# hvkwak/my-raytracer

Measured on AMD Instinct MI355X. Metric: Mrays/sec (primary+shadow+reflect), Office 1920x1080 1spp, higher is better.
Workload: dtype f64; 1 GPU; office_proxy 1920x1080 spp=1 depth=5 lights=2; triangles=59670, rays_per_frame=7073857, parallelism=single GPU, animation=camera orbit, 0.12 rad over each launch's 128 frames (distinct views), launches_in_flight=1, analytic_prims=False, production_frames_rendered=2595

## Files before the change

include/rt_hip.h:

```cpp
#ifndef RT_HIP_H
#define RT_HIP_H

#include <stddef.h>
#include "rt_scene.h"

#ifdef __cplusplus
extern "C" {
#endif

#define RT_OK 0
#define RT_ERR_INVALID (-1)
#define RT_ERR_HIP (-2)
#define RT_ERR_UNSUPPORTED (-3)

#define RT_MAX_LIGHTS 16
#define RT_LIGHTS_LIMIT (1 << 20)

typedef struct rt_scene_soa {
  int n_meshes;
  int n_vertices;
  int n_vertex_idx;
  int n_tex_coords;
  long long n_texels;
  const int* vertex_mesh_id;
// ... 23 lines not shown
  const double* bb_max;
  const int* left_child;
  const int* first_tri;
  const int* tri_count;
} rt_bvh_soa;

enum {
  RT_OUT_RGB_F32 = 0,
  RT_OUT_RGB_F64 = 1
};

enum {
  RT_FLAG_TRAVERSAL_STATS = 1,
  RT_FLAG_WIDE_STATS = 2,
  RT_FLAG_TIMELINE = 4,
  RT_FLAG_TILE_COST = 8,
  RT_FLAG_TILE_COST_TIME = 16,
  RT_FLAG_COST_ORDER = 32,
  RT_FLAG_NATURAL_ORDER = 64,
  RT_FLAG_GLOBAL_ROWS = 128
};

typedef struct rt_render_params {
  rt_camera camera;
  int n_lights;
  int max_depth;
  rt_light lights[RT_MAX_LIGHTS];
  double background[3];
  double ambience[3];
  int spp_n;
  int row_begin;
  int row_end;
  int stripe_height;
  int stripe_count;
  int stripe_index;
  int out_format;
  int flags;
  const rt_light* lights_ext;
} rt_render_params;

static inline const rt_light* rt_params_light(const rt_render_params* p, int i) {
  return p->lights_ext ? &p->lights_ext[i] : &p->lights[i];
}

typedef struct rt_stats {
  long long primary_rays;
  long long shadow_rays;
  long long reflection_rays;
  long long node_visits;
  long long tri_tests;
  long long closest_hits;
  long long pixels;
  long long reserved_;
} rt_stats;

typedef struct rt_scene rt_scene;

#define RT_MAX_COORDINATE 2305843009213693952.0

int rt_scene_upload(const rt_scene_soa* soa, const rt_bvh_soa* bvh, int device, rt_scene** out);

enum { RT_TREE_SAH = 0, RT_TREE_REFERENCE = 1, RT_TREE_SBVH = 2 };
enum { RT_COLLAPSE_GREEDY = 0, RT_COLLAPSE_SAH = 1, RT_COLLAPSE_BY_SIZE = 2 };

typedef struct rt_upload_options {
  int device_tree;
  int build_threads;
  int stack_ring;
  int lds_treelet;
  int collapse;
  int sbvh_leaf_max;
  int sbvh_bins;
  int blocks_per_cu;
  int grid_spare;
  int verbose;
  double sbvh_alpha;
  double sbvh_budget;
  double sbvh_c_trav;
  double collapse_c_tri;
  int reserve_cus;
  int order_window;
  int spp_lanes;
  int tree_opt;
  int reserved_[4];
} rt_upload_options;

enum { RT_TREE_OPT_PASSES = 3, RT_TREE_OPT_MAX = 64 };

void rt_upload_options_init(rt_upload_options* opt);

int rt_scene_upload_ex(const rt_scene_soa* soa, const rt_bvh_soa* bvh, int device, const rt_upload_options* opt,
                       rt_scene** out);

int rt_scene_upload_multi(const rt_scene_soa* soa, const rt_bvh_soa* bvh, const int* devices, int n_devices,
                          const rt_upload_options* opt, rt_scene** outs);

long long rt_scene_device_bytes(const rt_scene* scene);

int rt_scene_upload_seconds(const rt_scene* scene, double* build_s, double* copy_s);

int rt_scene_set_analytic(rt_scene* scene, const rt_sphere* spheres, int n_spheres, const rt_plane* planes,
                          int n_planes);

int rt_rows_in_shard(const rt_render_params* p);

int rt_launch_compute_image(rt_scene* scene, const rt_render_params* p, void* d_out,
                            rt_stats* stats, void* stream);

#define RT_MAX_FRAMES 128
int rt_launch_frames(rt_scene* scene, const rt_render_params* p, int n_frames, void* const* d_outs,
                     rt_stats* stats, void* stream);

int rt_launch_adaptive(rt_scene* scene, const rt_render_params* p, const double* d_primary, void* d_out, int subp,
                       double threshold, rt_stats* stats, long long* n_selected, void* stream);

int rt_launch_adaptive_frames(rt_scene* scene, const rt_render_params* p, int n_frames, const double* const* d_primary,
                              void* const* d_out, int subp, double threshold, rt_stats* stats, long long* n_selected,
                              void* stream);

int rt_launch_adaptive_shard(rt_scene* scene, const rt_render_params* p, const double* d_primary,
                             const double* d_halo, void* d_out, int subp, double threshold, rt_stats* stats,
                             long long* n_selected, void* stream);

int rt_adaptive_halo_rows(const rt_render_params* p, int* rows_out, int cap);

int rt_render_adaptive_to_host(rt_scene* scene, const rt_render_params* p, int subp, double threshold, void* host_out,
                               rt_stats* st_primary, rt_stats* st_adaptive, long long* n_selected);

int rt_render_to_host(rt_scene* scene, const rt_render_params* p, void* host_out, rt_stats* stats);

typedef struct rt_ray {
  double o[3];
  double d[3];
  double tmax;
  double reserved_;
} rt_ray;

typedef struct rt_hit {
  double t;
  double alpha;
  double beta;
  double normal[3];
  int slot;
  int mesh;
  int prim;
  int reserved_;
} rt_hit;

typedef struct rt_query_stats {
  long long rays, hits, stack_spills, watchdog, reserved_[4];
} rt_query_stats;

int rt_trace_closest(rt_scene* scene, const rt_ray* d_rays, long long n, rt_hit* d_hits, rt_query_stats* stats,
                     void* stream);

int rt_trace_occluded(rt_scene* scene, const rt_ray* d_rays, long long n, unsigned char* d_occluded,
                      rt_query_stats* stats, void* stream);

#define RT_RADIANCE_MAX_RAYS (1LL << 31)
int rt_trace_radiance(rt_scene* scene, const rt_render_params* p, const rt_ray* d_rays, long long n,
                      void* d_rgb, rt_stats* stats, void* stream);

#define RT_ORDER_MAX_RAYS (1LL << 31)
#define RT_ORDER_KEY_DEGENERATE 0x80000000u
#define RT_ORDER_TILE 1024

int rt_scene_bounds(const rt_scene* scene, double lo[3], double hi[3]);

size_t rt_ray_order_workspace_bytes(long long n);

// ... 52 lines not shown
int rt_trace_hits(rt_scene* scene, const rt_ray* d_rays, long long n, int k,
                  const rt_hit_key* d_after,
                  rt_hit* d_hits,
                  unsigned int* d_count,
                  rt_query_stats* stats, void* stream);

typedef struct rt_scene_update {
  long long n_vertices;
  long long n_triangles;
  const double* vertex_pos;
  const double* vertex_normals;
  const double* face_normals;
  long long reserved_[3];
} rt_scene_update;

int rt_scene_update_vertices(rt_scene* scene, const rt_scene_update* u, void* stream);

enum { RT_UPDATE_RECLIP = 1 };
int rt_scene_update_vertices_ex(rt_scene* scene, const rt_scene_update* u, unsigned flags, void* stream);

long long rt_debug_clip_regions(const rt_scene_soa* soa, const rt_bvh_soa* bvh, const rt_upload_options* opt,
                                double* clip_out, int* slot_out, long long cap);

int rt_reclip_box_host(const double p0[3], const double p1[3], const double p2[3], const double clip[6],
                       double lo[3], double hi[3]);

int rt_scene_set_triangle_order(rt_scene* scene, const int* slot_triangle, long long n_triangles);

typedef struct rt_scene_positions {
  long long n_vertices;
  const double* vertex_pos;
  int on_device;
  int reserved_;
  long long reserved2_[3];
} rt_scene_positions;

int rt_scene_update_positions(rt_scene* scene, const rt_scene_positions* positions, unsigned flags, void* stream);

int rt_normals_host(const int* vertex_idx, const int* slot_triangle, long long n_vertices, long long n_triangles,
                    const double* vertex_pos, double* vertex_normals_out, double* face_normals_out);

enum { RT_IMAGE_NODES4 = 0, RT_IMAGE_TRIS = 1, RT_IMAGE_TNORM = 2 };
long long rt_debug_scene_image(rt_scene* scene, int what, void* out, long long bytes);

#define RT_IPC_HANDLE_BYTES 64
int rt_ipc_get_handle(const void* d_ptr, unsigned char* handle, unsigned long long* offset);
int rt_ipc_open(const unsigned char* handle, unsigned long long offset, int device, int owner_device, void** d_ptr);
int rt_ipc_close(void* d_ptr, unsigned long long offset);

int rt_last_kernel_ms(rt_scene* scene, float* ms);

int rt_scene_status(const rt_scene* scene);

int rt_debug_counters(rt_scene* scene, unsigned long long* out, int n);

long long rt_debug_wave_log(rt_scene* scene, unsigned long long* out, long long n);

int rt_debug_blocks_per_cu(rt_scene* scene, int variant);

int rt_debug_last_grid(rt_scene* scene, long long* blocks, long long* full_blocks);

int rt_debug_corrupt_hierarchy(rt_scene* scene);

enum {
  RT_TREE_BAD_UNION = 1,
  RT_TREE_BAD_LEAF = 2,
  RT_TREE_BAD_RECORDS = 4,
  RT_TREE_BAD_IDS = 8,
  RT_TREE_BAD_FIXPOINT = 16
};
typedef struct rt_tree_report {
  long long binary_nodes, wide_nodes, records;
  long long moved;
  double sah_before, sah_after, dp_before, dp_after;
  double seconds;
  int passes;
  int stack4;
  unsigned int invalid;
  int converged;
} rt_tree_report;
int rt_debug_tree_report(const rt_scene_soa* soa, const rt_bvh_soa* bvh, const rt_upload_options* opt,
                         rt_tree_report* out);

long long rt_debug_timeline(rt_scene* scene, unsigned long long* out, long long n);

int rt_tile_shape(int* tile_w, int* tile_h);

long long rt_debug_tile_cost(rt_scene* scene, unsigned int* out, long long n);
int rt_debug_set_tile_order(rt_scene* scene, const unsigned int* order, long long n);
long long rt_debug_last_tile_order(rt_scene* scene, unsigned int* out, long long n);

void rt_scene_free(rt_scene* scene);

const char* rt_last_error(void);

const char* rt_build_info(void);

#ifdef __cplusplus
}
#endif
#endif
```

my-raytracer_amd/csrc/device/rt_render.hip:

```cpp
#ifndef RT_RAY_LIST_PASS
#include <hip/hip_runtime.h>
#include <hip/hip_ext.h>

#include <algorithm>
#include <array>
#include <chrono>
#include <cfloat>
#include <cmath>
#include <cstdio>
#include <cstdlib>
#include <cstring>
#include <memory>
#include <string>
#include <thread>
#include <vector>

#include <rocprim/block/block_radix_sort.hpp>

#include "../../../include/rt_hip.h"
#include "../host/device_image.hpp"
#include "rt_layout.hpp"

#pragma clang fp contract(off)

#include "rt_ao_fan.hpp"
#include "rt_refit.hpp"
#include "rt_reclip.hpp"
#include "rt_normals.hpp"

using namespace rtk;

namespace {

constexpr int kBlock = 256;
constexpr int kGroups = 8;
#ifndef RT_REFILL
#define RT_REFILL 16
#endif
constexpr int kRefill = RT_REFILL;
#ifndef RT_REFILL_GATE
#define RT_REFILL_GATE 0
#endif
constexpr bool kRefillGate = RT_REFILL_GATE != 0;
#ifndef RT_LEAF_PIN
#define RT_LEAF_PIN 1
#endif
#ifndef RT_MAT_BATCH
#define RT_MAT_BATCH 1
#endif
#ifndef RT_STACK_FAST
#define RT_STACK_FAST 41
#endif
constexpr bool kFastSort = (RT_STACK_FAST & 1) != 0, kFastAny = (RT_STACK_FAST & 2) != 0, kFastPop = (RT_STACK_FAST & 4) != 0;
constexpr bool kOneHit = (RT_STACK_FAST & 8) != 0, kMaskCnt = (RT_STACK_FAST & 32) != 0;
static_assert((RT_STACK_FAST & ~47) == 0, "RT_STACK_FAST: bits 1, 2, 4, 8 and 32");
constexpr bool kRoomTest = kFastSort || kFastAny;
constexpr int kCtrWords = 42;
constexpr int kShortStack = 8;
constexpr int kSlotDoubles = 10;
constexpr int kTopNodes = (40960 - kBlock * (kSlotDoubles * 8 + (2 + kShortStack) * 4) - RT_MAX_LIGHTS * 48 - 64) / 128;
constexpr int kStackMask = kShortStack - 1;
#ifndef RT_DONATE_MAX
#define RT_DONATE_MAX 24
#endif
constexpr int kDonateMax = RT_DONATE_MAX;
constexpr int kMigWords = 8;
static_assert(kMigWords <= kShortStack, "migration words travel in the stack ring entries");
constexpr int kPoolBytes = 64;
static_assert(8 + 8 * (kBlock / 64) + 4 <= kPoolBytes, "compaction pool does not fit");
static_assert((kShortStack & kStackMask) == 0, "the stack ring must be a power of two");

#ifdef RT_TILE_ROW_ORDER
constexpr bool kTileMorton = false;
#else
constexpr bool kTileMorton = true;
#endif
enum : int { ST_FETCH = 0, ST_CLOSEST = 1, ST_SHADOW = 2, ST_DONE = 3, ST_PARKED = 4, ST_HSHADOW = 5, ST_HCLOSEST = 6 };
constexpr uint32_t kTaskNone = 0xffffffffu;
constexpr uint32_t kTaskRefl = 0x80000000u;
static_assert(RT_LIGHTS_LIMIT <= (1 << 20), "light index must fit the task word");
constexpr int kBatchExtra = 31;
constexpr int kHelpShift = 24;
constexpr int kEndMask = (1 << kHelpShift) - 1;
static_assert(RT_LIGHTS_LIMIT < (1 << kHelpShift), "light index must fit the batch word");

__device__ __forceinline__ void wave_lds_sync() {
  __builtin_amdgcn_wave_barrier();
  asm volatile("s_waitcnt lgkmcnt(0)" ::: "memory");
  __builtin_amdgcn_wave_barrier();
}

constexpr int kBufWord3 = 0x00020000;
typedef unsigned int u32x2_t __attribute__((ext_vector_type(2)));
__device__ __forceinline__ double buf_ld(__amdgpu_buffer_rsrc_t r, uint32_t voff, uint32_t soff) {
  return __builtin_bit_cast(double, __builtin_amdgcn_raw_buffer_load_b64(r, voff, soff, 0));
}
__device__ __forceinline__ void buf_st(__amdgpu_buffer_rsrc_t r, uint32_t voff, uint32_t soff, double x) {
  __builtin_amdgcn_raw_buffer_store_b64(__builtin_bit_cast(u32x2_t, x), r, voff, soff, 0);
}
typedef unsigned int u32x4_t __attribute__((ext_vector_type(4)));
struct D2 {
  double a, b;
};
__device__ __forceinline__ D2 buf_ld2(__amdgpu_buffer_rsrc_t r, uint32_t voff, uint32_t soff) {
  const u32x4_t v = __builtin_amdgcn_raw_buffer_load_b128(r, voff, soff, 0);
  return D2{__builtin_bit_cast(double, u32x2_t{v.x, v.y}), __builtin_bit_cast(double, u32x2_t{v.z, v.w})};
}


__device__ __forceinline__ int wave_incl_scan(int x) {
  int incl = x;
#pragma unroll
  for (int o = 1; o < 64; o <<= 1) {
    const int v = __shfl_up(incl, o);
    if ((int)(threadIdx.x & 63) >= o) incl += v;
  }
  return incl;
}

__device__ __forceinline__ int kth_set_bit(unsigned long long m, int k) {
  int base = 0;
#pragma unroll
  for (int w = 32; w >= 1; w >>= 1) {
    const int c = __popcll(m & ((1ull << w) - 1ull));
    if (k >= c) { k -= c; m >>= w; base += w; }
  }
  return base;
}
enum : int { CS_PRIMARY = 8, CS_SHADOW, CS_REFLECT, CS_NODES, CS_TRIS, CS_HITS, CS_PIXELS };
enum : int {
  CD_NODE_ITERS = 16, CD_NODE_LANES, CD_LEAF_ITERS, CD_LEAF_LANES, CD_TRAV_CYCLES, CD_SHADE_CYCLES,
  CD_FETCH_CYCLES, CD_OUTER_ITERS, CD_TRAV_ROUNDS, CD_TRAV_ROUND_LANES, CD_SPILLS, CD_NODE_LINES,
  CD_LEAF_LINES, CD_BIG_LEAF_TESTS, CD_NODE_LDS_ITERS, CD_GUARD = 31,
  CD_GNODE_UNIFORM = 32, CD_GNODE_DISTINCT, CD_LEAF_UNIFORM, CD_ANYHIT_TRIS, CD_OWN_TRIS,
  CD_ZERO_TERM,
  CT_ORDER_JOBS = 39,
  CD_SLOW_PUSH = 40, CD_SLOW_POP
};
static_assert(kCtrWords * sizeof(unsigned long long) <= 512, "the counter words end where the work heads begin");
constexpr unsigned kGuardIters = 1u << 24;
constexpr unsigned kTravGuard = 1u << 24;
__device__ __forceinline__ void trip_watchdog(unsigned long long* ctr, unsigned int* host_word) {
  atomicOr(&ctr[CD_GUARD], 1ull);
  __builtin_nontemporal_store(1u, host_word);
  __threadfence_system();
  asm volatile("s_waitcnt vmcnt(0)" ::: "memory");
}
constexpr int kTlCap = 256;
constexpr int kTlWords = 8;

struct DivMagic {
  uint32_t m, s;
  __host__ __device__ uint32_t div(uint32_t n) const {
#ifdef __HIP_DEVICE_COMPILE__
    return m ? __umulhi(n, m) >> s : n;
#else
    return m ? (uint32_t)(((unsigned long long)n * m) >> 32) >> s : n;
#endif
  }
};
inline DivMagic div_magic(uint32_t d) {
  for (uint32_t s = 0; s < 32; ++s) {
    const unsigned __int128 p = (unsigned __int128)1 << (32 + s);
    const unsigned __int128 m = (p + d - 1) / d;
    if (m >> 32) continue;
    const unsigned __int128 e = m * d - p;
    if ((e << 31) < p) return DivMagic{(uint32_t)m, s};
  }
  return DivMagic{0u, 0u};
}
constexpr int kMaxFrames = RT_MAX_FRAMES;
constexpr int kListFrameShift = 25;
constexpr uint32_t kListPixMask = (1u << kListFrameShift) - 1u;
static_assert(kMaxFrames <= (1 << (32 - kListFrameShift)), "frame index must fit a list entry");
struct FrameDesc {
  double eye[3], ll[3], xd[3], yd[3];
  void* out;
  long long pad;
};
static_assert(sizeof(FrameDesc) == 112, "FrameDesc must be 112 bytes");
constexpr size_t kHeadsOff = 512;
constexpr int kHeadStride = 32;
constexpr size_t kCtrBytes = kHeadsOff + kGroups * 256;
constexpr size_t kCtlBytes = kCtrBytes + kMaxFrames * sizeof(FrameDesc);
struct KParams {
  const GNode* nodes;
  const GNode4* nodes4;
  const GTri* tris;
  const uint32_t* slot2dev;
  const TriShade* shade;
  const double* tnorm;
  const double* tu;
  const double* tv;
  const unsigned char* texels;
  const GMat* mats;
  unsigned long long* ctr;
  unsigned long long* heads;
  unsigned long long* wctr;
  double* pstate;
  uint32_t* spill;
  unsigned long long* wavelog;
  unsigned long long* tl;
  const double* lights;
  unsigned int* guard_host;
  size_t nslots;
  int n_gnodes;
  int out_fmt;
  int n_top;
  int top_off;
  double root_lo[3], root_hi[3];
  int W, H;
  int n_lights, max_depth;
  int zero_term_lights;
  double bg[3], amb[3];
  int spp_n;
  int group_log, chunks;
  int row_begin, stripe_h, stripe_count, stripe_index;
  int rows;
  int tiles_x;
  int out_global;
  union {
    int order_dilate;
    uint32_t fan_seed;
  };
  long long n_tiles;
  union {
    const uint32_t* list;
    const double* fan_dirs;
  };
  const unsigned long long* list_count;
  union {
    double* sample_out;
    double fan_bias;
  };
  union {
    int nsamp;
    int fan_k;
  };
  int n_prims;
  const GPrim* prims;
  int n_frames;
  int lights_off;
  int pool_off;
  long long frame_tiles;
  const FrameDesc* frames;
  union {
    const uint32_t* tile_order;
    const rt_ray* rays;
  };
  uint32_t* tile_cost;
  union {
    int cost_time;
    int fan_sets;
  };
  DivMagic div_row_tiles, div_tiles_x, div_stripe_h;
  const uint32_t* order_src;
  uint32_t* next_order;
  uint32_t* zero_map;
  union {
    long long n_pos;
    long long n_rays;
  };
};

struct D3 {
  double x, y, z;
};
__device__ __forceinline__ D3 d3(double x, double y, double z) { return D3{x, y, z}; }
__device__ __forceinline__ D3 add(D3 a, D3 b) { return D3{a.x + b.x, a.y + b.y, a.z + b.z}; }
__device__ __forceinline__ D3 sub(D3 a, D3 b) { return D3{a.x - b.x, a.y - b.y, a.z - b.z}; }
__device__ __forceinline__ D3 scl(double s, D3 a) { return D3{s * a.x, s * a.y, s * a.z}; }
__device__ __forceinline__ D3 mul(D3 a, D3 b) { return D3{a.x * b.x, a.y * b.y, a.z * b.z}; }
__device__ __forceinline__ double dot(D3 a, D3 b) { return a.x * b.x + a.y * b.y + a.z * b.z; }
__device__ __forceinline__ D3 normalize(D3 v) {
  const double n = sqrt(dot(v, v));
  if (n > 0.0) return D3{v.x / n, v.y / n, v.z / n};
  return v;
}
__device__ __forceinline__ double sqrt_normal(double q) {
  const double y = __builtin_amdgcn_rsq(q);
  double g = q * y, h = y * 0.5;
  const double r = __builtin_fma(-h, g, 0.5);
  g = __builtin_fma(g, r, g);
  double d = __builtin_fma(-g, g, q);
  h = __builtin_fma(h, r, h);
  g = __builtin_fma(d, h, g);
  d = __builtin_fma(-g, g, q);
  return __builtin_fma(d, h, g);
}
__device__ __forceinline__ double rcp_refined(double n) {
  double r = __builtin_amdgcn_rcp(n);
  r = __builtin_fma(r, __builtin_fma(-n, r, 1.0), r);
  return __builtin_fma(r, __builtin_fma(-n, r, 1.0), r);
}
__device__ __forceinline__ double div_by(double x, double n, double r) {
  const double q = x * r;
  return __builtin_fma(__builtin_fma(-n, q, x), r, q);
}
__device__ __forceinline__ D3 normalize_rcp(D3 v, double& n) {
  const double q = dot(v, v);
  const bool ok = fabs(v.x) >= 0x1p-200 && fabs(v.y) >= 0x1p-200 && fabs(v.z) >= 0x1p-200 &&
                  q <= 0x1p400;
  if (!ok) {
    n = sqrt(q);
    return normalize(v);
  }
  n = sqrt_normal(q);
  const double r = rcp_refined(n);
  return D3{div_by(v.x, n, r), div_by(v.y, n, r), div_by(v.z, n, r)};
}
__device__ __forceinline__ D3 normalize_shade(D3 v) {
  const double q = dot(v, v);
  if (!(q > 1e-200 && q < 1e200)) return normalize(v);
  const double r0 = __builtin_amdgcn_rsq(q);
  const double e = __builtin_fma(-(q * r0), r0, 1.0);
  const double r = __builtin_fma(0.5 * r0, e, r0);
  return D3{v.x * r, v.y * r, v.z * r};
}
__device__ __forceinline__ double pow_shade(double x, double y) {
  if (y >= 1.0 && y <= 256.0 && y == __builtin_floor(y)) {
    uint32_t n = (uint32_t)y;
    double r = 1.0, b = x;
    for (;;) {
      if (n & 1u) r *= b;
      n >>= 1;
      if (n == 0u) break;
      b *= b;
    }
    return r;
  }
  return pow(x, y);
}
__device__ __forceinline__ double stdmax(double a, double b) { return (a < b) ? b : a; }
__device__ __forceinline__ double stdmin(double a, double b) { return (b < a) ? b : a; }

__device__ __forceinline__ double det3(D3 v1, D3 v2, D3 v3) {
  return v1.x * (v2.y * v3.z - v3.y * v2.z) - v2.x * (v1.y * v3.z - v3.y * v1.z) +
         v3.x * (v1.y * v2.z - v2.y * v1.z);
}


__device__ __forceinline__ double prim_hit(const GPrim& G, D3 o, D3 d) {
  const D3 c = d3(G.c[0], G.c[1], G.c[2]);
  if (G.type == kPrimPlane) {
    const D3 n = d3(G.n[0], G.n[1], G.n[2]);
// ... 132 lines not shown
  __device__ __forceinline__ D3 kd() const { return d3(q1.y, q2.x, q2.y); }
  __device__ __forceinline__ D3 ks() const { return d3(q3.x, q3.y, q4.x); }
  __device__ __forceinline__ double shininess() const { return q4.y; }
  __device__ __forceinline__ double mirror() const { return q5.x; }
  __device__ __forceinline__ int shadowable() const { return __double2loint(q5.y); }
  __device__ __forceinline__ int draw_mode() const { return __double2hiint(q5.y); }
  __device__ __forceinline__ int tex_w() const { return __double2loint(q6); }
  __device__ __forceinline__ int tex_h() const { return __double2hiint(q6); }
  __device__ __forceinline__ uint32_t flags() const { return (uint32_t)__double2loint(q7); }
};
static_assert(offsetof(GMat, kd) == 24 && offsetof(GMat, ks) == 48 && offsetof(GMat, shininess) == 72 &&
              offsetof(GMat, mirror) == 80 && offsetof(GMat, shadowable) == 88 && offsetof(GMat, draw_mode) == 92 &&
              offsetof(GMat, tex_w) == 96 && offsetof(GMat, tex_h) == 100 && offsetof(GMat, flags) == 112,
              "Mat<true> unpacks GMat by its 16-byte groups");

#ifndef RT_TILE_W
#define RT_TILE_W 8
#endif
constexpr int kTileW = RT_TILE_W, kTileH = 64 / RT_TILE_W;
constexpr int kTileWLog = kTileW == 8 ? 3 : kTileW == 16 ? 4 : kTileW == 32 ? 5 : -1;
constexpr int kTileHLog = 6 - kTileWLog;
static_assert(kTileWLog > 0 && kTileW * kTileH == 64, "a tile is one wave's 64 pixels (8, 16 or 32 wide)");

enum : int { R_SCOLW = 0, R_PCOL = 1, R_HD = 2, R_LACC = 3, kRegions = 4 };
constexpr uint32_t kLaneRec = 32;
constexpr uint32_t kRegionBytes = 64 * kLaneRec;

struct RaySlots {
  double* o[3];
  double* d[3];
  double* tlim;
  double* a[3];
};

__device__ __forceinline__ float f4c(const float4& v, int c) {
  return c == 0 ? v.x : (c == 1 ? v.y : (c == 2 ? v.z : v.w));
}
__device__ __forceinline__ uint32_t u4c(const uint4& v, int c) {
  return c == 0 ? v.x : (c == 1 ? v.y : (c == 2 ? v.z : v.w));
}


#ifndef RT_WAVES_PER_EU
#define RT_WAVES_PER_EU 4
#endif
constexpr int kWavesPerEU = RT_WAVES_PER_EU;

constexpr int kOrderItems = 16;
constexpr int kOrderDilate = 4;
constexpr long long kOrderMaxRange = (long long)kBlock * kOrderItems;
constexpr int kOrderShift = 21;
__device__ __forceinline__ uint32_t order_class(uint32_t cost) {
  const int q = (int)(__float_as_uint((float)cost) >> kOrderShift) - ((127 + 8) << (23 - kOrderShift));
  return 255u - (uint32_t)min(255, max(0, q));
}
__device__ void order_range(const uint32_t* cost, uint32_t* order, long long n_tiles, int h, unsigned char* lds,
                            int tiles_x, int dilate) {
  using Sort = rocprim::block_radix_sort<unsigned int, kBlock, kOrderItems>;
  static_assert(sizeof(typename Sort::storage_type) <= 30720, "sort storage must fit the block's LDS (at least 30 KB)");
  auto& storage = *reinterpret_cast<typename Sort::storage_type*>(lds);
  const long long t0 = n_tiles * h / kGroups, t1 = n_tiles * (h + 1) / kGroups;
  unsigned int keys[kOrderItems];
#pragma unroll
  for (int j = 0; j < kOrderItems; ++j) {
    const long long li = (long long)threadIdx.x * kOrderItems + j;
    uint32_t c = 0u;
    if (t0 + li < t1) {
      const long long t = t0 + li, row = t / tiles_x, col = t - row * tiles_x;
      const long long x0 = max(0LL, col - dilate), x1 = min((long long)tiles_x - 1, col + dilate);
      for (long long x = x0; x <= x1; ++x) c = max(c, cost[row * tiles_x + x]);
    }
    keys[j] = t0 + li < t1 ? (order_class(c) << 12) | (uint32_t)li : 0xffffffffu;
  }
  Sort().sort(keys, storage, 12, 20);
#pragma unroll
  for (int j = 0; j < kOrderItems; ++j) {
    const long long pos = (long long)threadIdx.x * kOrderItems + j;
    if (t0 + pos < t1) order[t0 + pos] = (uint32_t)(t0 + (keys[j] & 0xfffu));
  }
}

#endif

#ifndef RT_RAY_LIST_PASS
template <int WIDTH, bool STATS, bool TL = false, int RING = kShortStack, bool GRP = false>
__global__ void __launch_bounds__(kBlock, kWavesPerEU * 256 / kBlock) render_kernel(KParams P) {
  constexpr bool RAYS = false, FAN = false;
#define RT_GROUPS_ON group_log
#elif !defined(RT_FAN_PASS)
template <int RING>
__global__ void __launch_bounds__(kBlock, kWavesPerEU * 256 / kBlock) radiance_kernel(KParams P) {
  constexpr int WIDTH = 4;
  constexpr bool STATS = false, TL = false, GRP = false, RAYS = true, FAN = false;
#define RT_GROUPS_ON group_log
#else
template <int RING>
__global__ void __launch_bounds__(kBlock, kWavesPerEU * 256 / kBlock) gather_kernel(KParams P) {
  constexpr int WIDTH = 4;
  constexpr bool STATS = false, TL = false, GRP = true, RAYS = true, FAN = true;
#define RT_GROUPS_ON true
#endif
  static_assert(RING >= kMigWords && (RING & (RING - 1)) == 0, "ring: a power of two holding the migration words");
  constexpr int kRingMask = RING - 1;
  constexpr bool kPinMat = RT_MAT_BATCH != 0 && !GRP;
  extern __shared__ __attribute__((aligned(16))) unsigned char lds_raw[];
  constexpr uint32_t kRingRegion = (uint32_t)RING * kBlock * sizeof(uint32_t);
  unsigned char* const lds_s = lds_raw + kRingRegion;
  double* lds_d = reinterpret_cast<double*>(lds_s);
  RaySlots R;
#pragma unroll
  for (int k = 0; k < 3; ++k) {
    R.o[k] = lds_d + k * kBlock + threadIdx.x;
    R.d[k] = lds_d + (3 + k) * kBlock + threadIdx.x;
  }
  R.tlim = lds_d + 6 * kBlock + threadIdx.x;
#pragma unroll
  for (int k = 0; k < 3; ++k) R.a[k] = lds_d + (7 + k) * kBlock + threadIdx.x;
  uint32_t* ltask = reinterpret_cast<uint32_t*>(lds_s + kSlotDoubles * kBlock * sizeof(double));
  uint32_t* lvis = ltask + kBlock;
  uint32_t* stk = reinterpret_cast<uint32_t*>(lds_raw) + threadIdx.x;
  const uint32_t lane_b = threadIdx.x * 4u;
  lvis[threadIdx.x] = 0u;
  uint32_t* pool_live = reinterpret_cast<uint32_t*>(lds_raw + P.pool_off);
  unsigned long long* pool_mask = reinterpret_cast<unsigned long long*>(lds_raw + P.pool_off + 8);
  uint32_t* pool_exh = reinterpret_cast<uint32_t*>(lds_raw + P.pool_off + 8 + 8 * (kBlock / 64));
  if (threadIdx.x == 0) {
    *pool_live = kBlock / 64;
    for (int w = 0; w < kBlock / 64; ++w) pool_mask[w] = 0ull;
    *pool_exh = 0u;
  }
  if (WIDTH == 4 && P.n_top > 0) {
    float4* dst = reinterpret_cast<float4*>(lds_raw + P.top_off);
    const float4* src = reinterpret_cast<const float4*>(P.nodes4);
    for (int i = threadIdx.x; i < P.n_top * (int)(sizeof(GNode4) / sizeof(float4)); i += kBlock) dst[i] = src[i];
  }
  double* lds_lights = reinterpret_cast<double*>(lds_raw + P.lights_off);
  const bool lights_lds = P.n_lights <= RT_MAX_LIGHTS;
  if (lights_lds)
    for (int i = threadIdx.x; i < P.n_lights * 6; i += kBlock) lds_lights[i] = P.lights[i];
  __syncthreads();
  const int wbase = threadIdx.x & ~63;
  uint32_t* spill = P.spill + (size_t)blockIdx.x * kBlock + threadIdx.x;

  const int lane = threadIdx.x & 63;
  auto lane_bit = [&](unsigned long long m) -> bool {
    int l = lane;
    asm volatile("" : "+v"(l));
    return ((m >> l) & 1ull) != 0ull;
  };
  auto below = [](unsigned long long m) -> int {
    return (int)__builtin_amdgcn_mbcnt_hi((uint32_t)(m >> 32), __builtin_amdgcn_mbcnt_lo((uint32_t)m, 0u));
  };
  const int group_log = GRP ? P.group_log : 0;
  auto full_groups = [&](unsigned long long m) -> unsigned long long {
    const int gl = group_log;
    for (int sh = 1; sh < (1 << gl); sh <<= 1) m &= m >> sh;
    unsigned long long first = 0ull;
    for (int b = 0; b < 64; b += 1 << gl) first |= 1ull << b;
    return m & first;
  };
  const __amdgpu_buffer_rsrc_t prs =
      __builtin_amdgcn_make_buffer_rsrc(P.pstate, 0, (int)(P.nslots * kRegions * kLaneRec), kBufWord3);
  uint32_t pvo = (blockIdx.x * (kBlock / 64) + (threadIdx.x >> 6)) * (uint32_t)kRegions * kRegionBytes +
                 (uint32_t)lane * kLaneRec;
  auto LD4 = [&](int r, D3& v, double& w) {
    const D2 a = buf_ld2(prs, pvo, (uint32_t)r * kRegionBytes), b = buf_ld2(prs, pvo, (uint32_t)r * kRegionBytes + 16u);
    v = d3(a.a, a.b, b.a);
    w = b.b;
  };
  auto ST4 = [&](int r, D3 v, double w) {
#ifdef RT_MEAS_NO_PSTATE
    return;
#endif
    const uint32_t o = (uint32_t)r * kRegionBytes;
    buf_st(prs, pvo, o, v.x); buf_st(prs, pvo, o + 8u, v.y); buf_st(prs, pvo, o + 16u, v.z); buf_st(prs, pvo, o + 24u, w);
  };
  auto LDV = [&](int r) { D3 v; double w; LD4(r, v, w); return v; };
  auto STV = [&](int r, D3 v) { ST4(r, v, 0.0); };
  auto LD_HN = [&]() { return d3(*R.a[0], *R.a[1], *R.a[2]); };
  auto ST_HN = [&](D3 v) { *R.a[0] = v.x; *R.a[1] = v.y; *R.a[2] = v.z; };
  auto LD_SCOL_W = [&](D3& scol, double& w) {
    LD4(R_SCOLW, scol, w);
  };
  auto ST_SCOL_W = [&](D3 scol, double w) { ST4(R_SCOLW, scol, w); };

  const long long n_list = !RAYS && P.list ? (long long)*P.list_count * (group_log ? 1 : P.nsamp) : 0;
  const long long n_tiles = !RAYS && P.list ? (n_list + 63) / 64 : P.n_tiles;
  int head = blockIdx.x % kGroups;
  int heads_left = kGroups;

  int state = ST_FETCH;
  int px = 0, lrow = 0, py = 0, sample = 0, depth = 0, light = 0, mesh = 0, frame = 0;
  long long item = 0;
  uint32_t pix_t0 = 0;
  int best = kNoHit;
  int own_rec = -1;
  int best_slot = kNoHit;
  double thit = DBL_MAX;
  bool shadow_hit = false;
  int batch_end = 0;
  int refl_h = -1;
  int want = 0;
  uint32_t htask = kTaskNone;
  unsigned c_primary = 0, c_shadow = 0, c_refl = 0, c_hits = 0;
  unsigned n_zero_term = 0;
  unsigned long long c_nodes = 0, c_tris = 0;
  unsigned long long d_node_it = 0, d_node_ln = 0, d_leaf_it = 0, d_leaf_ln = 0;
  unsigned long long d_trav = 0, d_shade = 0, d_fetch = 0, d_outer = 0, d_round_it = 0, d_round_ln = 0;
  unsigned long long d_spills = 0, d_node_lines = 0, d_leaf_lines = 0, d_big_leaf = 0, d_node_lds = 0, d_dummy = 0, d_gn_uni = 0, d_gn_dist = 0, d_leaf_uni = 0;
  unsigned long long d_slow_push = 0, d_slow_pop = 0;
  unsigned long long d_any_tris = 0, d_own_tris = 0;
  unsigned long long w_start = STATS ? __builtin_amdgcn_s_memrealtime() : 0ull, w_refill = 0, w_pixels = 0;
  unsigned long long t_stamp = 0;
  unsigned tl_n = 0;
  unsigned long long tl_t0 = 0;
  unsigned tl_it = 0, tl_leaf = 0, tl_spill = 0, tl_gnode = 0;
  unsigned long long tl_wn = 0, tl_wl = 0, tl_wr = 0, tl_dummy = 0;
  unsigned long long tl_gsum[4] = {0, 0, 0, 0}, tl_gcnt[4] = {0, 0, 0, 0}, tl_gap = 0;
  auto tl_wave_gap = [&](uint32_t kind) {
    const unsigned long long m = wballot(1);
    if (lane == __ffsll((long long)m) - 1) {
      const uint32_t now = (uint32_t)__builtin_amdgcn_s_memrealtime();
      const uint32_t prev = ltask[wbase + 63], pk = ltask[wbase + 62];
      ltask[wbase + 63] = now;
      ltask[wbase + 62] = kind;
      const unsigned long long g = now - prev;
#pragma unroll
      for (uint32_t k = 0; k < 4; ++k)
        if (pk == k) { tl_gsum[k] += g; tl_gcnt[k]++; }
      if (g > tl_gap) tl_gap = g;
    }
  };
  auto stamp = [&]() -> unsigned long long { return STATS ? __builtin_amdgcn_s_memtime() : 0ull; };

  struct Light6 { D3 pos, col; };
  typedef __attribute__((address_space(3))) double lds_double;
  typedef __attribute__((address_space(1))) const double glb_double;
  auto light_of = [&](int j) -> Light6 {
    if (lights_lds) {
      const lds_double* L = (const lds_double*)(lds_double*)(lds_lights) + 6 * j;
      return Light6{d3(L[0], L[1], L[2]), d3(L[3], L[4], L[5])};
    }
    const glb_double* L = (const glb_double*)(P.lights) + 6 * (size_t)j;
    return Light6{d3(L[0], L[1], L[2]), d3(L[3], L[4], L[5])};
  };

  auto nrm_n = [](D3 v, double& n) -> D3 {
    if constexpr (STATS || TL) {
      n = sqrt(dot(v, v));
      return normalize(v);
    } else {
      return normalize_rcp(v, n);
    }
  };
  auto nrm = [&](D3 v) -> D3 {
    double n;
    return nrm_n(v, n);
  };
  auto emit_ray = [&](D3 o, D3 dir, double t_limit) {
    const D3 d = nrm(dir);
    *R.o[0] = o.x; *R.o[1] = o.y; *R.o[2] = o.z;
    *R.d[0] = d.x; *R.d[1] = d.y; *R.d[2] = d.z;
    *R.tlim = t_limit;
  };

  auto start_sample = [&]() {
    int n = P.spp_n;
    asm volatile("" : "+s"(n));
    double X, Y;
    if (n == 1) {
      X = (double)px;
      Y = (double)py;
    } else {
      const int si = sample / n, sj = sample - si * n;
      const double xo = (si) / (double)n - 0.5 + 1.0 / (2.0 * n);
      const double yo = (sj) / (double)n - 0.5 + 1.0 / (2.0 * n);
      X = (double)px + xo;
      Y = (double)py + yo;
    }
    const FrameDesc& K = P.frames[frame];
    const D3 dir = d3(K.ll[0] + X * K.xd[0] + Y * K.yd[0] - K.eye[0],
                      K.ll[1] + X * K.xd[1] + Y * K.yd[1] - K.eye[1],
                      K.ll[2] + X * K.xd[2] + Y * K.yd[2] - K.eye[2]);
    depth = 0;
    c_primary++;
    if (sample == 0) pix_t0 = (uint32_t)__builtin_amdgcn_s_memrealtime();
    emit_ray(d3(K.eye[0], K.eye[1], K.eye[2]), dir, DBL_MAX);
    state = ST_CLOSEST;
// ... 152 lines not shown
            item = wk;
          } else {
            const uint32_t tile = P.tile_order ? P.tile_order[wk >> 6] : (uint32_t)(wk >> 6);
            const int j = (int)(wk & 63);
            const uint32_t row_tiles = (uint32_t)P.n_frames * (uint32_t)P.tiles_x;
            const uint32_t ty = P.div_row_tiles.div(tile);
            const uint32_t rem = tile - ty * row_tiles;
            frame = P.n_frames > 1 ? (int)P.div_tiles_x.div(rem) : 0;
            const int tx = (int)(rem - (uint32_t)frame * (uint32_t)P.tiles_x);
            int jx = j & (kTileW - 1), jy = j >> kTileWLog;
            if (kTileMorton && kTileW == 8) {
              jx = (j & 1) | ((j >> 1) & 2) | ((j >> 2) & 4);
              jy = ((j >> 1) & 1) | ((j >> 2) & 2) | ((j >> 3) & 4);
            }
            px = tx * kTileW + jx;
            lrow = (int)ty * kTileH + jy;
          }
          if (!RAYS && px < P.W && lrow < P.rows) {
            py = (P.stripe_count == 1)
                     ? P.row_begin + lrow
                     : stripe_row(P, lrow);
            if (P.list && !group_log) {
              long long ns = P.nsamp;
              asm volatile("" : "+s"(ns));
              sample = (int)(item % ns);
            } else {
              sample = lane - gbase;
            }
            start_sample();
          }
        }
      }
      m_fetch = wballot(state == ST_FETCH);
      m_busy = wballot(state == ST_CLOSEST || state == ST_SHADOW || state >= ST_HSHADOW);
      m_claim = RT_GROUPS_ON ? full_groups(m_fetch) : m_fetch;
      if (!RT_GROUPS_ON && __popcll(m_fetch) < kRefill && m_busy != 0) break;
    }
    if (heads_left == 0 && state == ST_FETCH) state = ST_DONE;
    const bool busy = (state == ST_CLOSEST || state == ST_SHADOW || state >= ST_HSHADOW);
    if (wballot(busy) == 0) {
      if (wballot(state != ST_DONE) != 0) continue;
      bool leave = true;
      if (lane == 0) {
        uint32_t v = *pool_live;
        for (;;) {
          if (v >= 2u) {
            const uint32_t seen = atomicCAS(pool_live, v, v - 1u);
            if (seen == v) break;
            v = seen;
            continue;
          }
          bool pooled = false;
          for (int w = 0; w < kBlock / 64; ++w) pooled |= pool_mask[w] != 0ull;
          if (pooled) leave = false;
          else *pool_live = 0u;
          break;
        }
      }
      if (__shfl(leave ? 1 : 0, 0)) break;
    }

    if (STATS) { const unsigned long long t = stamp(); d_fetch += t - t_stamp; t_stamp = t; }
    if constexpr (TL) {
      tl_t0 = __builtin_amdgcn_s_memrealtime();
      tl_it = tl_leaf = tl_spill = tl_gnode = 0;
      tl_wn = tl_wl = tl_wr = 0;
      tl_gap = 0;
#pragma unroll
      for (int k = 0; k < 4; ++k) tl_gsum[k] = tl_gcnt[k] = 0;
      if (lane == 0) { ltask[wbase + 63] = (uint32_t)tl_t0; ltask[wbase + 62] = 0u; }
      wave_lds_sync();
    }
    unsigned long long sh0 = 0ull;
    int kp = 0;
    for (;; ++kp) {
      const bool act = kp == 0 ? busy
                               : (state == ST_SHADOW && light + (batch_end >> kHelpShift) + kp < (batch_end & kEndMask));
      const bool anyhit = act && (state == ST_SHADOW || state == ST_HSHADOW);
      const int src = (act && state >= ST_HSHADOW) ? wbase + (int)(htask & 63u) : (int)threadIdx.x;
      D3 ro = d3(lds_d[0 * kBlock + src], lds_d[1 * kBlock + src], lds_d[2 * kBlock + src]);
      D3 rd = d3(lds_d[3 * kBlock + src], lds_d[4 * kBlock + src], lds_d[5 * kBlock + src]);
      double tlim = lds_d[6 * kBlock + src];
      bool zero_term = false;
      if (anyhit) {
        const int j = (state == ST_SHADOW) ? light + (kp > 0 ? (batch_end >> kHelpShift) + kp : 0)
                                           : (int)((htask >> 11) & 0xFFFFFu);
        const D3 hp = add(ro, scl(tlim, rd));
        const D3 to_l = sub(light_of(j).pos, hp);
        double nl;
        const D3 l = nrm_n(to_l, nl);
        if (lvis[src] & 1u) {
          const D3 hn = d3(lds_d[7 * kBlock + src], lds_d[8 * kBlock + src], lds_d[9 * kBlock + src]);
          zero_term = !(dot(hn, l) > 0.0);
        }
        ro = add(hp, scl(1e-4, l));
        rd = nrm(l);
        tlim = nl;
      } else if (act && state == ST_HCLOSEST) {
        const D3 hp = add(ro, scl(tlim, rd));
        const D3 hn = d3(lds_d[7 * kBlock + src], lds_d[8 * kBlock + src], lds_d[9 * kBlock + src]);
        const double s2 = 2.0 * dot(hn, rd);
        const D3 v = sub(rd, scl(s2, hn));
        ro = add(hp, scl(1e-4, v));
        rd = nrm(v);
        tlim = DBL_MAX;
        *R.o[0] = ro.x; *R.o[1] = ro.y; *R.o[2] = ro.z;
        *R.d[0] = rd.x; *R.d[1] = rd.y; *R.d[2] = rd.z;
      }
      int own = -1;
      if (anyhit) own = (state == ST_SHADOW) ? own_rec : __shfl(own_rec, (int)(htask & 63u));
      best = kNoHit;
      best_slot = kNoHit;
      n_zero_term += (unsigned)__popcll(wballot(zero_term));
      shadow_hit = !STATS && !TL && zero_term;
      uint32_t cur = kDone;
      double t_off = 0.0;
      for (int k = 0; k < P.n_prims; ++k) {
        if (!act || shadow_hit) break;
        const double t = prim_hit(P.prims[k], ro, rd);
        if (t < tlim) {
          if (anyhit) { shadow_hit = true; break; }
          tlim = t;
          best = kPrimHit | k;
          best_slot = -1;
        }
      }
      if (act && P.n_gnodes > 0 && !shadow_hit) {
        bool miss = false;
        int pz = 0;
        asm volatile("" : "+s"(pz));
        const double* const root_lo = P.root_lo + pz;
        const double* const root_hi = P.root_hi + pz;
        const double o3[3] = {ro.x, ro.y, ro.z}, d3v[3] = {rd.x, rd.y, rd.z};
        bool inside = true;
#pragma unroll
        for (int k = 0; k < 3; ++k)
          if (!(o3[k] >= root_lo[k] && o3[k] <= root_hi[k])) inside = false;
        if (!inside) {
          double tn = -DBL_MAX, tf = DBL_MAX;
#pragma unroll
          for (int k = 0; k < 3; ++k) {
            if (d3v[k] == 0.0) {
              if (o3[k] < root_lo[k] || o3[k] > root_hi[k]) miss = true;
              continue;
            }
            double t0 = (root_lo[k] - o3[k]) / d3v[k];
            double t1 = (root_hi[k] - o3[k]) / d3v[k];
            if (t0 > t1) { const double t = t0; t0 = t1; t1 = t; }
            if (t0 > tn) tn = t0;
            if (t1 < tf) tf = t1;
          }
          if (tn > tf || tf < 0.0) miss = true;
          t_off = tn > 0.0 ? tn : 0.0;
        }
        if (miss) t_off = 0.0;
        else cur = 0;
      }
      float inv[3];
      {
        const double d3v[3] = {rd.x, rd.y, rd.z};
#pragma unroll
        for (int k = 0; k < 3; ++k) {
          float df = (float)d3v[k];
          if (fabsf(df) < 1e-20f) df = signbit(d3v[k]) ? -1e-20f : 1e-20f;
          if constexpr (WIDTH == 4) {
            const float r0 = __builtin_amdgcn_rcpf(df);
            inv[k] = __builtin_fmaf(__builtin_fmaf(-df, r0, 1.0f), r0, r0);
          } else {
            inv[k] = 1.0f / df;
          }
        }
      }
      const float ofx = (float)(ro.x + t_off * rd.x);
      const float ofy = (float)(ro.y + t_off * rd.y);
      const float ofz = (float)(ro.z + t_off * rd.z);
      const float ivx = inv[0], ivy = inv[1], ivz = inv[2];
      const uint32_t nxo = ivx >= 0.f ? 0u : 16u, nyo = ivy >= 0.f ? 32u : 48u, nzo = ivz >= 0.f ? 64u : 80u;
      const float oix = ofx * ivx, oiy = ofy * ivy, oiz = ofz * ivz;
      const float lo_c = round_down_f(-t_off);
      float hi_c = round_up_f(tlim - t_off);
      float pinf = INFINITY;
      asm volatile("" : "+s"(pinf));
      constexpr uint32_t kSW = kBlock * 4u, kRingB = (uint32_t)RING * kSW, kRingBMask = (uint32_t)kRingMask * kSW;
      uint32_t sq = 0, sqlim = kRingB;
      auto ring = [&](uint32_t q) -> __attribute__((address_space(3))) uint32_t& {
        return *reinterpret_cast<__attribute__((address_space(3))) uint32_t*>((size_t)((q & kRingBMask) | lane_b));
      };
      auto push = [&](uint32_t x) {
        if (sq == sqlim) {
          const uint32_t qlo = sqlim - kRingB;
          spill[(size_t)(qlo / kSW) * P.nslots] = ring(qlo);
          sqlim += kSW;
          if (STATS) d_spills++;
          if constexpr (TL) tl_spill++;
        }
        ring(sq) = x;
        sq += kSW;
      };
      auto pop = [&]() -> uint32_t {
        if (sq == 0) return kDone;
        sq -= kSW;
        if (sq + kRingB >= sqlim) return ring(sq);
        sqlim = sq + kRingB;
        return spill[(size_t)(sq / kSW) * P.nslots];
      };
      auto pop_fast = [&]() -> uint32_t {
        const uint32_t x = ring(sq - kSW);
        const bool empty = sq == 0;
        sq -= empty ? 0u : kSW;
        return empty ? kDone : x;
// ... 706 lines not shown
        if (group_done && lane == gbase) {
          D3 pc = sample == 0 ? d3(0, 0, 0) : LDV(R_PCOL);
          if constexpr (FAN) {
            for (int k = 0; k < (1 << gl) && sample + k < P.fan_k; ++k) {
              const int t = wbase + gbase + k;
              pc = add(pc, d3(lds_d[0 * kBlock + t], lds_d[1 * kBlock + t], lds_d[2 * kBlock + t]));
            }
            if (sample + (1 << gl) < P.fan_k) STV(R_PCOL, pc);
            else store_pixel(pc);
          } else {
            for (int k = 0; k < (1 << gl); ++k) {
              const int t = wbase + gbase + k;
              pc = add(pc, d3(lds_d[0 * kBlock + t], lds_d[1 * kBlock + t], lds_d[2 * kBlock + t]));
            }
            if (sample + (1 << gl) < P.spp_n * P.spp_n) STV(R_PCOL, pc);
            else store_pixel(pc);
          }
        }
        wave_lds_sync();
        if (group_done) {
          sample += 1 << gl;
          if constexpr (FAN) {
            if (sample - (lane - gbase) < P.fan_k) start_fan();
            else state = heads_left > 0 ? ST_FETCH : ST_DONE;
          } else {
            if (sample < P.spp_n * P.spp_n) start_sample();
            else state = heads_left > 0 ? ST_FETCH : ST_DONE;
          }
        }
      }
    }

    {
      const bool idle = (state == ST_FETCH || state == ST_DONE);
      const unsigned long long I = wballot(idle);
      if (I != 0ull && wballot(want > 0) != 0ull) {
        if (idle) ltask[threadIdx.x] = kTaskNone;
        const int incl = wave_incl_scan(want);
        wave_lds_sync();
        const int off = incl - want;
        const int avail = (int)__popcll(I);
        const int got = min(want, max(0, avail - off));
        if (got > 0) {
          const int n_extra_lights = min(P.n_lights - light - 1, kBatchExtra);
          for (int t = 0; t < got; ++t) {
            const int ht = wbase + kth_set_bit(I, off + t);
            uint32_t tw;
            if (t < n_extra_lights) {
              tw = (uint32_t)lane | ((uint32_t)(t + 1) << 6) | ((uint32_t)(light + 1 + t) << 11);
            } else {
              tw = (uint32_t)lane | kTaskRefl;
              c_refl++;
              refl_h = ht;
            }
            ltask[ht] = tw;
          }
          batch_end |= min(got, n_extra_lights) << kHelpShift;
        }
        wave_lds_sync();
        if (idle) {
          htask = ltask[threadIdx.x];
          if (htask != kTaskNone) state = (htask & kTaskRefl) ? ST_HCLOSEST : ST_HSHADOW;
        }
      }
    }
    if (STATS) { const unsigned long long t = stamp(); d_shade += t - t_stamp; t_stamp = t; }
  }

  if (STATS && lane == 0) {
    unsigned long long* wl = P.wavelog + 4 * ((size_t)blockIdx.x * (kBlock / 64) + (threadIdx.x >> 6));
    wl[0] = w_start;
    wl[1] = w_refill;
    wl[2] = __builtin_amdgcn_s_memrealtime();
    wl[3] = w_pixels;
  }
  if (P.out_global) {
    __threadfence_system();
    asm volatile("s_waitcnt vmcnt(0)" ::: "memory");
  }
  const unsigned long long s0 = wave_sum(c_primary), s1 = wave_sum(c_shadow), s2 = wave_sum(c_refl);
  unsigned long long s3 = 0, s4 = 0, s5 = 0;
  if (STATS) { s3 = wave_sum(c_nodes); s4 = wave_sum(c_tris); s5 = wave_sum(c_hits); }
  if (lane == 0) {
    unsigned long long* wc = P.wctr + 4 * ((size_t)blockIdx.x * (kBlock / 64) + (threadIdx.x >> 6));
    wc[0] = s0; wc[1] = s1; wc[2] = s2; wc[3] = n_zero_term;
    if (STATS) {
      atomicAdd(&P.ctr[CS_NODES], s3);
      atomicAdd(&P.ctr[CS_TRIS], s4);
      atomicAdd(&P.ctr[CS_HITS], s5);
      atomicAdd(&P.ctr[CD_TRAV_CYCLES], d_trav);
      atomicAdd(&P.ctr[CD_SHADE_CYCLES], d_shade);
      atomicAdd(&P.ctr[CD_FETCH_CYCLES], d_fetch);
      atomicAdd(&P.ctr[CD_OUTER_ITERS], d_outer);
    }
  }
  if (STATS) {
    const unsigned long long a = wave_sum(d_node_it), b = wave_sum(d_node_ln), c = wave_sum(d_leaf_it);
    const unsigned long long d = wave_sum(d_leaf_ln), e = wave_sum(d_round_it), f = wave_sum(d_round_ln);
    const unsigned long long g = wave_sum(d_spills), h = wave_sum(d_node_lines), q = wave_sum(d_leaf_lines);
    const unsigned long long r = wave_sum(d_big_leaf), t = wave_sum(d_node_lds);
    const unsigned long long gu = wave_sum(d_gn_uni), gd = wave_sum(d_gn_dist), lu = wave_sum(d_leaf_uni);
    const unsigned long long at = wave_sum(d_any_tris), ot = wave_sum(d_own_tris);
    const unsigned long long pu = wave_sum(d_slow_push), po = wave_sum(d_slow_pop);
    if (lane == 0) {
      atomicAdd(&P.ctr[CD_SLOW_PUSH], pu);
      atomicAdd(&P.ctr[CD_SLOW_POP], po);
      atomicAdd(&P.ctr[CD_ANYHIT_TRIS], at);
      atomicAdd(&P.ctr[CD_OWN_TRIS], ot);
      atomicAdd(&P.ctr[CD_NODE_LDS_ITERS], t);
      atomicAdd(&P.ctr[CD_GNODE_UNIFORM], gu);
      atomicAdd(&P.ctr[CD_GNODE_DISTINCT], gd);
      atomicAdd(&P.ctr[CD_LEAF_UNIFORM], lu);
      atomicAdd(&P.ctr[CD_NODE_ITERS], a);
      atomicAdd(&P.ctr[CD_NODE_LANES], b);
      atomicAdd(&P.ctr[CD_LEAF_ITERS], c);
      atomicAdd(&P.ctr[CD_LEAF_LANES], d);
      atomicAdd(&P.ctr[CD_TRAV_ROUNDS], e);
      atomicAdd(&P.ctr[CD_TRAV_ROUND_LANES], f);
      atomicAdd(&P.ctr[CD_SPILLS], g);
      atomicAdd(&P.ctr[CD_NODE_LINES], h);
      atomicAdd(&P.ctr[CD_LEAF_LINES], q);
      atomicAdd(&P.ctr[CD_BIG_LEAF_TESTS], r);
    }
  }
  if (!RAYS && P.zero_map) {
    uint32_t* job = reinterpret_cast<uint32_t*>(lds_raw);
    for (;;) {
      __syncthreads();
      if (threadIdx.x == 0) *job = (uint32_t)atomicAdd(&P.ctr[CT_ORDER_JOBS], 1ull);
      __syncthreads();
      const uint32_t j = *job;
      __syncthreads();
      if (j >= 2u * kGroups) break;
      if (j < (uint32_t)kGroups) {
        if (P.order_src) order_range(P.order_src, P.next_order, P.n_pos, (int)j, lds_raw, P.tiles_x, P.order_dilate);
      } else {
        for (long long i = P.n_pos * (j - kGroups) / kGroups + threadIdx.x; i < P.n_pos * (j - kGroups + 1) / kGroups;
             i += kBlock)
          P.zero_map[i] = 0u;
      }
    }
  }
}
#undef RT_GROUPS_ON

#ifndef RT_RAY_LIST_PASS
#define RT_RAY_LIST_PASS 1
#include __FILE_NAME__
#define RT_FAN_PASS 1
#include __FILE_NAME__
#undef RT_FAN_PASS
#undef RT_RAY_LIST_PASS

__device__ __forceinline__ double nsq3(const double* a, const double* b) {
  const double dx = a[0] - b[0], dy = a[1] - b[1], dz = a[2] - b[2];
  return dx * dx + dy * dy + dz * dz;
}

struct ShardRows {
  int rows, W, H;
  int row_begin, stripe_h, stripe_count, stripe_index;
  __host__ __device__ int global_row(int lrow) const {
    return stripe_count == 1 ? row_begin + lrow
                             : ((lrow / stripe_h) * stripe_count + stripe_index) * stripe_h + (lrow % stripe_h);
  }
  __host__ __device__ int seg_first(int lrow) const { return stripe_count == 1 ? 0 : lrow - lrow % stripe_h; }
  __host__ __device__ int seg_last(int lrow) const {
    return stripe_count == 1 ? rows - 1 : min(seg_first(lrow) + stripe_h, rows) - 1;
  }
  __host__ __device__ int segment(int lrow) const { return stripe_count == 1 ? 0 : lrow / stripe_h; }
  __host__ __device__ int segments() const { return stripe_count == 1 ? (rows > 0) : (rows + stripe_h - 1) / stripe_h; }
};

constexpr int kSelThreads = 1024;
constexpr int kSelTilesPerWave = 8;
constexpr int kSelTilesPerBlock = (kSelThreads / 64) * kSelTilesPerWave;
__global__ void __launch_bounds__(kSelThreads) adaptive_select_kernel(const double* prim, const double* halo, void* out,
                                                                      int out_fmt, ShardRows G, double threshold,
                                                                      int tiles_x, long long n_tiles, uint32_t* list,
                                                                      unsigned long long* count, uint32_t frame_tag,
                                                                      const double* const* prims, void* const* outs) {
  if (prims) {
    prim = prims[blockIdx.y];
    out = outs[blockIdx.y];
    frame_tag = (uint32_t)blockIdx.y << kListFrameShift;
  }
  __shared__ uint32_t s_list[kSelThreads * kSelTilesPerWave];
  __shared__ uint32_t s_n;
  __shared__ unsigned long long s_base;
  if (threadIdx.x == 0) s_n = 0u;
  __syncthreads();
  const int j = threadIdx.x & 63;
  const int W = G.W;
  for (int it = 0; it < kSelTilesPerWave; ++it) {
    const long long tile = (long long)blockIdx.x * kSelTilesPerBlock + it * (kSelThreads / 64) + (threadIdx.x >> 6);
    bool sel = false;
    int x = 0, lrow = 0;
    if (tile < n_tiles) {
      const long long ty = tile / tiles_x;
      x = (int)(tile - ty * tiles_x) * 8 + (j & 7);
      lrow = (int)ty * 8 + (j >> 3);
      if (x < W && lrow < G.rows) {
        const size_t o = 3 * ((size_t)lrow * W + x);
        const double* c = prim + o;
        const int y = G.global_row(lrow);
        if (x >= 1 && y >= 1 && x < W - 1 && y < G.H - 1) {
          const int seg = G.segment(lrow);
          const double* up = lrow < G.seg_last(lrow) ? c + 3 * (size_t)W : halo + 3 * ((size_t)(2 * seg + 1) * W + x);
          const double* dn = lrow > G.seg_first(lrow) ? c - 3 * (size_t)W : halo + 3 * ((size_t)(2 * seg) * W + x);
          const double n = nsq3(c, c + 3) + nsq3(c, up) + nsq3(c, c - 3) + nsq3(c, dn);
          sel = n > threshold;
        }
        if (!sel) {
          if (out_fmt == RT_OUT_RGB_F64) {
            double* d = reinterpret_cast<double*>(out) + o;
            d[0] = c[0]; d[1] = c[1]; d[2] = c[2];
          } else {
            float* d = reinterpret_cast<float*>(out) + o;
            d[0] = (float)c[0]; d[1] = (float)c[1]; d[2] = (float)c[2];
          }
        }
      }
    }
    const unsigned long long m = wballot(sel);
    if (m != 0ull) {
      const int leader = __ffsll((long long)m) - 1;
      uint32_t base = 0u;
      if (j == leader) base = atomicAdd(&s_n, (uint32_t)__popcll(m));
      base = __shfl(base, leader);
      if (sel) {
        const unsigned long long below = j == 0 ? 0ull : (m & (~0ull >> (64 - j)));
        s_list[base + __popcll(below)] = frame_tag | (uint32_t)((size_t)lrow * W + x);
      }
    }
  }
  __syncthreads();
  const uint32_t n = s_n;
  if (n == 0u) return;
  if (threadIdx.x == 0) s_base = atomicAdd(count, (unsigned long long)n);
  __syncthreads();
  const unsigned long long b = s_base;
  for (uint32_t k = threadIdx.x; k < n; k += kSelThreads) list[b + k] = s_list[k];
}

__global__ void __launch_bounds__(256) adaptive_reduce_kernel(const uint32_t* list, const unsigned long long* count,
                                                              const double* samples, int nsamp, void* out,
                                                              int out_fmt, void* const* outs) {
  const long long i = (long long)blockIdx.x * blockDim.x + threadIdx.x;
  if (i >= (long long)*count) return;
  const double* s = samples + 3 * (size_t)i * nsamp;
  double r = 0.0, g = 0.0, b = 0.0;
  for (int k = 0; k < nsamp; ++k) {
    r = r + s[3 * k];
    g = g + s[3 * k + 1];
    b = b + s[3 * k + 2];
  }
  const double nn = (double)nsamp;
  r = stdmin(r / nn, 1.0);
  g = stdmin(g / nn, 1.0);
  b = stdmin(b / nn, 1.0);
  const uint32_t id = list[i];
  const size_t o = 3 * (size_t)(id & kListPixMask);
  if (outs) out = outs[id >> kListFrameShift];
  if (out_fmt == RT_OUT_RGB_F64) {
    double* d = reinterpret_cast<double*>(out) + o;
    d[0] = r; d[1] = g; d[2] = b;
  } else {
    float* d = reinterpret_cast<float*>(out) + o;
    d[0] = (float)r; d[1] = (float)g; d[2] = (float)b;
  }
}

thread_local std::string g_error;

int fail(int code, const std::string& msg) {
  g_error = msg;
  return code;
}

#define HIP_TRY(call)                                                                          \
  do {                                                                                         \
    const hipError_t e_ = (call);                                                              \
    if (e_ != hipSuccess)                                                                      \
      return fail(RT_ERR_HIP, std::string(#call) + ": " + hipGetErrorString(e_));              \
  } while (0)


using KernelFn = void (*)(KParams);

struct Variant {
  KernelFn fn;
  bool stats;
};

const Variant kVariants[] = {
    {render_kernel<4, false>, false},
    {render_kernel<4, true>, true},
    {render_kernel<2, true>, true},
    {render_kernel<4, false, true>, false},
    {render_kernel<4, false, false, 16>, false},
    {render_kernel<4, false, false, kShortStack, true>, false},
    {render_kernel<4, false, false, 16, true>, false},
    {radiance_kernel<kShortStack>, false},
    {radiance_kernel<16>, false},
    {gather_kernel<kShortStack>, false},
    {gather_kernel<16>, false},
};
constexpr int kNumVariants = 11;
constexpr int kRayVariant = 7;
constexpr int kFanVariant = 9;
constexpr bool kSppLanesDefault = true;
constexpr int kGroupLanes = 32;
constexpr int kRingDeep = 16;
inline int variant_ring(int v) {
  return (v == 4 || v == 6 || v == kRayVariant + 1 || v == kFanVariant + 1) ? kRingDeep : kShortStack;
}
size_t lds_bytes(int , int ring = kShortStack) {
  return (size_t)kBlock * (kSlotDoubles * sizeof(double) + (2 + (size_t)ring) * sizeof(uint32_t));
}
size_t lds_bytes_total(int stack_words, int n_top, int ring = kShortStack) {
  return lds_bytes(stack_words, ring) + (size_t)n_top * sizeof(GNode4) + RT_MAX_LIGHTS * 6 * sizeof(double) + kPoolBytes;
}
int top_nodes_for(int stack_words, int ring, int n_gnodes4) {
  const long long room = 40960 - (long long)lds_bytes_total(stack_words, 0, ring);
  return (int)std::max(0LL, std::min<long long>({room / (long long)sizeof(GNode4), (long long)kTopNodes, (long long)n_gnodes4}));
}

}

constexpr int kContexts = 8;
struct LaunchCtx {
  unsigned long long* d_ctr = nullptr;
  unsigned char* h_ctl = nullptr;
  size_t ctl_cap = 0;
  long long blocks = 0;
  long long full_blocks = 0;
  double* d_pstate = nullptr;
  uint32_t* d_spill = nullptr;
  unsigned long long* d_wavelog = nullptr;
  unsigned long long* d_wctr = nullptr;
  unsigned long long* d_tl = nullptr;
  hipEvent_t ev0 = nullptr, ev1 = nullptr;
  hipEvent_t ev_in = nullptr;
  long long waves = 0;
  int variant = -1;
  bool used = false;
};

struct QueryRing;
struct UpdateState;
struct NormalState;

struct rt_scene {
  int device = 0;
  GNode* d_nodes = nullptr;
  GTri* d_tris = nullptr;
  uint32_t* d_slot2dev = nullptr;
  TriShade* d_shade = nullptr;
  double* d_tnorm = nullptr;
  double* d_tu = nullptr;
  double* d_tv = nullptr;
  unsigned char* d_texels = nullptr;
  GMat* d_mats = nullptr;
  int n_gnodes = 0;
  long long n_tris = 0;
  int n_meshes = 0;
  int depth = 0;
  int stack_words = 1;
  LaunchCtx ctx[kContexts];
  int next_ctx = 0;
  int last_ctx = -1;
  hipStream_t last_stream = nullptr;
  size_t nslots = 0;
  unsigned int* h_guard = nullptr;
  unsigned int* d_guard = nullptr;
  double delta = 0.0;
  double root_lo[3] = {0, 0, 0}, root_hi[3] = {0, 0, 0};
  long long bytes = 0;
  int n_cu = 0;
  int blocks_per_cu[kNumVariants] = {};
  bool deep = false;
  bool big = false;
  int n_top_v[kNumVariants] = {};
  GNode4* d_nodes4 = nullptr;
  int n_gnodes4 = 0;
  int bpc_cap = 0;
  int grid_spare = 0;
  std::vector<GMat> mesh_mats;
  GPrim* d_prims = nullptr;
  int n_prims = 0;
  long long table_bytes = 0;
  uint32_t* d_cost[3] = {nullptr, nullptr, nullptr};
  uint32_t* d_order[2] = {nullptr, nullptr};
  long long cost_cap = 0, cost_n = 0;
  int cost_tiles_x = 0;
  long long cost_seq = 0;
  long long order_for = -1;
  long long last_order_n = 0;
  int last_order_buf = 0;
  uint32_t* d_tile_order = nullptr;
  void* d_host_stage = nullptr;
  size_t host_stage_bytes = 0;
  long long tile_order_n = 0;
  bool maps_used = false;
  hipStream_t maps_stream = nullptr;
  hipEvent_t maps_ev = nullptr;
  double build_s = 0.0, copy_s = 0.0;
  int reserve_cus = 0;
  int order_window = 0;
  int spp_lanes = 0;
  static constexpr int kMaskedStreams = 4;
  hipStream_t masked[kMaskedStreams] = {};
  hipStream_t masked_for[kMaskedStreams] = {};
  int n_masked = 0;
  QueryRing* query = nullptr;
  int order_grid = 0;
  long long n_vertices = 0;
  long long n_rec = 0;
  UpdateState* update = nullptr;
  NormalState* normals = nullptr;
  bool updated = false;
  std::shared_ptr<const ClipTable> clip;
};

namespace {

template <typename T>
int upload(T** dst, const std::vector<T>& src, long long& bytes) {
  const size_t n = std::max<size_t>(src.size(), 1);
  HIP_TRY(hipMalloc(reinterpret_cast<void**>(dst), n * sizeof(T)));
  if (!src.empty()) HIP_TRY(hipMemcpy(*dst, src.data(), src.size() * sizeof(T), hipMemcpyHostToDevice));
  bytes += (long long)(n * sizeof(T));
  return RT_OK;
}

}

extern "C" {

const char* rt_last_error(void) { return g_error.c_str(); }

const char* rt_build_info(void) {
  return "librt_hip: gfx950 persistent flattened render kernel; variants {4-wide 8-entry stack ring, 4-wide 16-entry ring (>= 2^18 triangle records), "
         "4-wide+stats, 2-wide canonical stats, 4-wide+round timeline, sample groups (spp > 1) on both rings, ray lists (rt_trace_radiance) on both rings, "
         "fans over surface points (rt_trace_gather) on both rings}; "
         "fp32 4-wide nodes (128 B) with an LDS treelet, "
         "fp64 triangles/shading, LDS ray slots + stack ring (global spill), global path state, 8 XCD work heads";
}

int rt_scene_upload(const rt_scene_soa* s, const rt_bvh_soa* b, int device, rt_scene** out) {
  return rt_scene_upload_ex(s, b, device, nullptr, out);
}

}

namespace {
int upload_image(const SceneImage& I, const rt_upload_options& opt, int device, rt_scene** out) {
  HIP_TRY(hipSetDevice(device));
  {
    hipMemPool_t pool;
    if (hipDeviceGetDefaultMemPool(&pool, device) == hipSuccess) {
      uint64_t keep = UINT64_MAX;
      (void)hipMemPoolSetAttribute(pool, hipMemPoolAttrReleaseThreshold, &keep);
    }
  }
  auto* sc = new rt_scene();
  sc->device = device;
  long long bytes = 0;
  int rc = RT_OK;
  if (rc == RT_OK) rc = upload(&sc->d_nodes, I.nodes, bytes);
  if (rc == RT_OK) rc = upload(&sc->d_nodes4, I.nodes4, bytes);
  if (rc == RT_OK) rc = upload(&sc->d_tris, I.tris, bytes);
  if (rc == RT_OK) rc = upload(&sc->d_slot2dev, I.slot2dev, bytes);
  if (rc == RT_OK) rc = upload(&sc->d_shade, I.shade, bytes);
  if (rc == RT_OK) rc = upload(&sc->d_tnorm, I.tnorm, bytes);
  if (rc == RT_OK) rc = upload(&sc->d_tu, I.tu, bytes);
  if (rc == RT_OK) rc = upload(&sc->d_tv, I.tv, bytes);
  if (rc == RT_OK) rc = upload(&sc->d_texels, I.texels, bytes);
  if (rc == RT_OK) rc = upload(&sc->d_mats, I.mats, bytes);
  if (rc != RT_OK) {
    rt_scene_free(sc);
    return rc;
  }
  sc->n_gnodes = (int)I.nodes.size();
  sc->n_tris = I.n_tris;
  sc->n_vertices = I.n_vertices;
  sc->n_rec = (long long)I.tris.size();
  sc->clip = I.clip;
  sc->n_meshes = I.n_meshes;
  sc->mesh_mats = I.mats;
  sc->table_bytes = (long long)(std::max<size_t>(I.mats.size(), 1) * sizeof(GMat));
  sc->depth = I.depth;
  sc->stack_words = std::max(std::max(1, I.depth), I.stack4);
  sc->n_gnodes4 = (int)I.nodes4.size();
  if ((unsigned long long)I.nodes4.size() * sizeof(GNode4) >= (1ull << 32)) {
    rt_scene_free(sc);
    return fail(RT_ERR_UNSUPPORTED, "rt_scene_upload: more than 2^25 4-wide nodes");
  }
  sc->big = I.tris.size() >= (size_t)(1u << 18);
  sc->deep = sc->big;
  if (opt.stack_ring != 0) sc->deep = opt.stack_ring >= 16;
  for (int v = 0; v < kNumVariants; ++v) {
    int& nt = sc->n_top_v[v];
    nt = top_nodes_for(sc->stack_words, variant_ring(v), sc->n_gnodes4);
    if (opt.lds_treelet > 0) nt = std::min(nt, opt.lds_treelet);
    if (opt.lds_treelet < 0) nt = 0;
  }
  sc->bpc_cap = opt.blocks_per_cu;
  sc->grid_spare = opt.grid_spare;
  sc->reserve_cus = opt.reserve_cus;
  sc->order_window = opt.order_window;
  sc->spp_lanes = opt.spp_lanes;
  sc->delta = I.delta;
  for (int k = 0; k < 3; ++k) {
    sc->root_lo[k] = I.root_lo[k];
    sc->root_hi[k] = I.root_hi[k];
  }
  sc->bytes = bytes;
  hipDeviceProp_t prop;
  if (hipGetDeviceProperties(&prop, device) != hipSuccess) { rt_scene_free(sc); return fail(RT_ERR_HIP, "hipGetDeviceProperties failed"); }
  sc->n_cu = prop.multiProcessorCount;
  sc->reserve_cus = std::max(0, std::min(sc->reserve_cus, sc->n_cu - 1));
  int max_blocks = 1;
  for (int v = 0; v < kNumVariants; ++v) {
    const int ring = variant_ring(v);
    const size_t lds = lds_bytes_total(sc->stack_words, sc->n_top_v[v], ring);
    int nb = 0;
    if (hipOccupancyMaxActiveBlocksPerMultiprocessor(&nb, reinterpret_cast<const void*>(kVariants[v].fn), kBlock, lds) !=
            hipSuccess || nb < 1)
      nb = 1;
    hipFuncAttributes fa;
    if (hipFuncGetAttributes(&fa, reinterpret_cast<const void*>(kVariants[v].fn)) == hipSuccess && fa.numRegs > 0) {
      const int waves_per_simd = 512 / ((fa.numRegs + 7) / 8 * 8);
      nb = std::min(nb, std::max(1, waves_per_simd * 4 / (kBlock / 64)));
    }
    nb = std::min(nb, std::max(1, (int)(160 * 1024 / lds)));
    sc->blocks_per_cu[v] = nb;
    max_blocks = std::max(max_blocks, nb);
  }
  sc->nslots = (size_t)sc->n_cu * max_blocks * kBlock;
  if (hipHostMalloc(reinterpret_cast<void**>(&sc->h_guard), 64, hipHostMallocMapped) != hipSuccess ||
      hipHostGetDevicePointer(reinterpret_cast<void**>(&sc->d_guard), sc->h_guard, 0) != hipSuccess) {
    rt_scene_free(sc);
    return fail(RT_ERR_HIP, "allocation of the watchdog word failed");
  }
  *reinterpret_cast<volatile unsigned int*>(sc->h_guard) = 0u;
  for (LaunchCtx& c : sc->ctx) {
    const size_t pb = sc->nslots * kRegions * kLaneRec;
    const size_t wb = sc->nslots / 64 * 4 * sizeof(unsigned long long);
    const size_t sb = sc->stack_words > kShortStack ? sc->nslots * (size_t)sc->stack_words * sizeof(uint32_t) : 0;
    c.ctl_cap = kCtlBytes + RT_MAX_LIGHTS * 6 * sizeof(double);
    if (hipMalloc(reinterpret_cast<void**>(&c.d_ctr), c.ctl_cap) != hipSuccess ||
        hipHostMalloc(reinterpret_cast<void**>(&c.h_ctl), c.ctl_cap, hipHostMallocDefault) != hipSuccess ||
        hipMalloc(reinterpret_cast<void**>(&c.d_pstate), pb) != hipSuccess ||
        hipMalloc(reinterpret_cast<void**>(&c.d_wavelog), wb) != hipSuccess ||
        hipMalloc(reinterpret_cast<void**>(&c.d_wctr), wb) != hipSuccess ||
        (sb > 0 && hipMalloc(reinterpret_cast<void**>(&c.d_spill), sb) != hipSuccess) ||
        hipMemset(c.d_ctr, 0, kCtrBytes) != hipSuccess ||
        hipEventCreate(&c.ev0) != hipSuccess || hipEventCreate(&c.ev1) != hipSuccess) {
      rt_scene_free(sc);
      return fail(RT_ERR_HIP, "allocation of launch contexts failed");
    }
    sc->bytes += (long long)(c.ctl_cap + pb + 2 * wb + sb);
  }
  *out = sc;
  return RT_OK;
}
int resolve_options(const rt_upload_options* opt, rt_upload_options& o) {
  upload_options_defaults(&o);
  if (!opt) return RT_OK;
  o = *opt;
  rt_upload_options d;
  upload_options_defaults(&d);
  if (o.sbvh_bins == 0) o.sbvh_bins = d.sbvh_bins;
  if (o.sbvh_c_trav == 0.0) o.sbvh_c_trav = d.sbvh_c_trav;
  if (o.collapse_c_tri == 0.0) o.collapse_c_tri = d.collapse_c_tri;
  if (o.lds_treelet < -1) return fail(RT_ERR_INVALID, "rt_scene_upload: lds_treelet must be >= -1");
  if (o.reserve_cus < -1) return fail(RT_ERR_INVALID, "rt_scene_upload: reserve_cus must be >= -1");
  if (o.order_window < -1 || o.order_window > 64)
    return fail(RT_ERR_INVALID, "rt_scene_upload: order_window must be in [-1, 64]");
  if (o.spp_lanes < -1 || o.spp_lanes > 64 || (o.spp_lanes > 1 && (o.spp_lanes & (o.spp_lanes - 1)) != 0))
    return fail(RT_ERR_INVALID, "rt_scene_upload: spp_lanes must be -1, 0, 1 or a power of two <= 64");
  if (o.stack_ring != 0 && o.stack_ring != 8 && o.stack_ring != 16)
    return fail(RT_ERR_INVALID, "rt_scene_upload: stack_ring must be 0, 8 or 16");
  if (o.blocks_per_cu < 0 || o.grid_spare < 0 || o.build_threads < 0)
    return fail(RT_ERR_INVALID, "rt_scene_upload: negative blocks_per_cu / grid_spare / build_threads");
  if (o.sbvh_leaf_max < 0 || o.sbvh_leaf_max > 8 || o.sbvh_bins < 2 || o.sbvh_bins > 128 ||
      o.sbvh_alpha != o.sbvh_alpha || o.sbvh_budget != o.sbvh_budget ||
       !(o.sbvh_c_trav >= 0.0) || !(o.collapse_c_tri >= 0.0))
    return fail(RT_ERR_INVALID, "rt_scene_upload: SBVH / collapse parameter out of range");
  return RT_OK;
}
}

extern "C" {

void rt_upload_options_init(rt_upload_options* opt) {
  if (opt) upload_options_defaults(opt);
}

int rt_scene_upload_ex(const rt_scene_soa* s, const rt_bvh_soa* b, int device, const rt_upload_options* opt,
                       rt_scene** out) {
  if (!out) return fail(RT_ERR_INVALID, "rt_scene_upload: null out");
  *out = nullptr;
  rt_upload_options o;
  int rc = resolve_options(opt, o);
  if (rc != RT_OK) return rc;
  SceneImage I;
  const auto t0 = std::chrono::steady_clock::now();
  rc = build_image(s, b, o, kTopNodes, I);
  if (rc != RT_OK) return fail(rc, build_image_error());
  const auto t1 = std::chrono::steady_clock::now();
  rc = upload_image(I, o, device, out);
  if (rc == RT_OK) {
    (*out)->build_s = std::chrono::duration<double>(t1 - t0).count();
    (*out)->copy_s = std::chrono::duration<double>(std::chrono::steady_clock::now() - t1).count();
  }
  return rc;
}

int rt_scene_upload_multi(const rt_scene_soa* s, const rt_bvh_soa* b, const int* devices, int n_devices,
                          const rt_upload_options* opt, rt_scene** outs) {
  if (!outs || !devices || n_devices < 1) return fail(RT_ERR_INVALID, "rt_scene_upload_multi: bad argument");
  for (int g = 0; g < n_devices; ++g) outs[g] = nullptr;
  rt_upload_options o;
  int rc = resolve_options(opt, o);
  if (rc != RT_OK) return rc;
  SceneImage I;
  const auto t0 = std::chrono::steady_clock::now();
  rc = build_image(s, b, o, kTopNodes, I);
  if (rc != RT_OK) return fail(rc, build_image_error());
  const double build_s = std::chrono::duration<double>(std::chrono::steady_clock::now() - t0).count();
  std::vector<int> rcs(n_devices, RT_OK);
  std::vector<std::string> errs(n_devices);
  std::vector<std::thread> th;
  for (int g = 0; g < n_devices; ++g)
    th.emplace_back([&, g]() {
      const auto t1 = std::chrono::steady_clock::now();
      rcs[g] = upload_image(I, o, devices[g], &outs[g]);
      if (rcs[g] != RT_OK) {
        errs[g] = g_error;
      } else {
        outs[g]->build_s = build_s;
        outs[g]->copy_s = std::chrono::duration<double>(std::chrono::steady_clock::now() - t1).count();
      }
    });
  for (auto& t : th) t.join();
  for (int g = 0; g < n_devices; ++g)
    if (rcs[g] != RT_OK) {
      for (int k = 0; k < n_devices; ++k) {
        rt_scene_free(outs[k]);
        outs[k] = nullptr;
      }
      return fail(rcs[g], "rt_scene_upload_multi: device " + std::to_string(devices[g]) + ": " + errs[g]);
    }
  return RT_OK;
}

long long rt_scene_device_bytes(const rt_scene* s) { return s ? s->bytes : 0; }

int rt_scene_upload_seconds(const rt_scene* s, double* build_s, double* copy_s) {
  if (!s) return fail(RT_ERR_INVALID, "rt_scene_upload_seconds: null scene");
  if (build_s) *build_s = s->build_s;
  if (copy_s) *copy_s = s->copy_s;
  return RT_OK;
}

int rt_rows_in_shard(const rt_render_params* p) {
  if (!p) return 0;
  const int H = p->camera.height;
  const int sc = p->stripe_count > 0 ? p->stripe_count : 1;
  const int sh = p->stripe_height > 0 ? p->stripe_height : 1;
  if (sc == 1) {
    const int rb = std::max(0, p->row_begin);
    const int re = (p->row_end <= 0 || p->row_end > H) ? H : p->row_end;
    return std::max(0, re - rb);
  }
  int rows = 0;
  for (int y = 0; y < H; ++y)
    if ((y / sh) % sc == p->stripe_index) rows++;
  return rows;
}

}

namespace {
int read_counters(const LaunchCtx& C, unsigned long long* c) {
  HIP_TRY(hipMemcpy(c, C.d_ctr, kCtrWords * sizeof(unsigned long long), hipMemcpyDeviceToHost));
  if (C.waves > 0) {
    std::vector<unsigned long long> w((size_t)C.waves * 4);
    HIP_TRY(hipMemcpy(w.data(), C.d_wctr, w.size() * sizeof(unsigned long long), hipMemcpyDeviceToHost));
    for (size_t i = 0; i < w.size(); i += 4) {
      c[CS_PRIMARY] += w[i];
      c[CS_SHADOW] += w[i + 1];
      c[CS_REFLECT] += w[i + 2];
      c[CD_ZERO_TERM] += w[i + 3];
    }
  }
  return RT_OK;
}

int masked_stream(rt_scene* sc, hipStream_t caller, hipStream_t* out) {
  for (int i = 0; i < sc->n_masked; ++i)
    if (sc->masked_for[i] == caller) { *out = sc->masked[i]; return RT_OK; }
  if (sc->n_masked >= rt_scene::kMaskedStreams) {
    const uintptr_t h = reinterpret_cast<uintptr_t>(caller);
    *out = sc->masked[(size_t)((h >> 4) ^ (h >> 12)) % rt_scene::kMaskedStreams];
    return RT_OK;
  }
  std::vector<uint32_t> mask((size_t)(sc->n_cu + 31) / 32, 0u);
  for (int c = sc->reserve_cus; c < sc->n_cu; ++c) mask[(size_t)c / 32] |= 1u << (c % 32);
  hipStream_t s = nullptr;
  HIP_TRY(hipExtStreamCreateWithCUMask(&s, (uint32_t)mask.size(), mask.data()));
  {
    std::vector<uint32_t> got(mask.size(), 0u);
    const hipError_t e = hipExtStreamGetCUMask(s, (uint32_t)got.size(), got.data());
    if (e != hipSuccess || got != mask) {
      (void)hipStreamDestroy(s);
      return fail(RT_ERR_HIP, e != hipSuccess ? "hipExtStreamGetCUMask failed"
                                              : "reserve_cus: the CU-masked stream did not take the requested mask");
    }
  }
  sc->masked[sc->n_masked] = s;
  sc->masked_for[sc->n_masked] = caller;
  sc->n_masked++;
  *out = s;
  return RT_OK;
}

static bool event_done(hipEvent_t e) {
  const hipError_t q = hipEventQuery(e);
  if (q == hipErrorNotReady && hipPeekAtLastError() == hipErrorNotReady) (void)hipGetLastError();
  return q == hipSuccess;
}

const char* const kGuardMsg =
    "a launch on this scene tripped the kernel watchdog (cyclic or corrupt hierarchy, or a kernel bug): "
    "its pixels and every later result of this scene are void";
static bool guard_tripped(const rt_scene* sc) {
  return sc->h_guard && *reinterpret_cast<const volatile unsigned int*>(sc->h_guard) != 0u;
}

bool use_groups(const rt_scene* sc, const rt_render_params* p) {
  const int nsamp = p->spp_n * p->spp_n;
  return nsamp > 1 && (nsamp & (nsamp - 1)) == 0 && (sc->spp_lanes > 0 || (sc->spp_lanes == 0 && kSppLanesDefault)) &&
         !(p->flags & (RT_FLAG_COST_ORDER | RT_FLAG_TRAVERSAL_STATS | RT_FLAG_WIDE_STATS | RT_FLAG_TIMELINE |
                       RT_FLAG_TILE_COST | RT_FLAG_TILE_COST_TIME));
}

int launch_render(rt_scene* sc, const rt_render_params* p, int n_frames, void* const* outs, rt_stats* stats,
                  void* stream, const uint32_t* list, const unsigned long long* count, long long list_cap,
                  double* sample_out = nullptr, const rt_ray* rays = nullptr, long long n_rays = 0,
                  const rt_ao_params* fan = nullptr) {
  if (!sc || !p || !outs) return fail(RT_ERR_INVALID, "rt_launch_compute_image: null argument");
  if (n_frames < 1 || n_frames > kMaxFrames) return fail(RT_ERR_INVALID, "rt_launch_frames: n_frames out of range");
  for (int f = 0; f < n_frames; ++f) {
    if (!outs[f]) return fail(RT_ERR_INVALID, "rt_launch_compute_image: null output buffer");
    if (f == 0) continue;
    rt_render_params q = p[f];
    for (int k = 0; k < 3; ++k) {
      q.camera.eye[k] = p[0].camera.eye[k]; q.camera.lower_left[k] = p[0].camera.lower_left[k];
      q.camera.x_dir[k] = p[0].camera.x_dir[k]; q.camera.y_dir[k] = p[0].camera.y_dir[k];
    }
    if (std::memcmp(&q, &p[0], sizeof q) != 0)
      return fail(RT_ERR_INVALID, "rt_launch_frames: frames may differ only in camera position and direction");
  }
  if (p->camera.width <= 0 || p->camera.height <= 0 || p->camera.width > 65535 || p->camera.height > 65535)
    return fail(RT_ERR_INVALID, "bad image size (1..65535 per side)");
  if (p->n_lights < 0 || p->n_lights > (p->lights_ext ? RT_LIGHTS_LIMIT : RT_MAX_LIGHTS))
    return fail(RT_ERR_INVALID, "n_lights out of range (more than RT_MAX_LIGHTS lights need lights_ext)");
  if (p->spp_n < 1 || p->spp_n > 64) return fail(RT_ERR_INVALID, "spp_n must be in [1, 64]");
  if (p->max_depth < 0) return fail(RT_ERR_INVALID, "max_depth must be >= 0");
  if (p->out_format != RT_OUT_RGB_F32 && p->out_format != RT_OUT_RGB_F64) return fail(RT_ERR_INVALID, "bad out_format");
  const int scount = p->stripe_count > 0 ? p->stripe_count : 1;
  if (p->stripe_index < 0 || p->stripe_index >= scount) return fail(RT_ERR_INVALID, "stripe_index out of range");
  if (scount > 1 && (p->row_begin != 0 || (p->row_end > 0 && p->row_end != p->camera.height)))
    return fail(RT_ERR_INVALID, "row ranges cannot be combined with stripe_count > 1");
  const int rows = rt_rows_in_shard(p);
  hipStream_t st = reinterpret_cast<hipStream_t>(stream);
  HIP_TRY(hipSetDevice(sc->device));
  if (guard_tripped(sc)) return fail(RT_ERR_HIP, kGuardMsg);
  if ((p->flags & RT_FLAG_TRAVERSAL_STATS) && sc->updated)
    return fail(RT_ERR_UNSUPPORTED, "RT_FLAG_TRAVERSAL_STATS is not supported after rt_scene_update_vertices");

  KParams P;
  std::memset(&P, 0, sizeof P);
  P.nodes = sc->d_nodes; P.nodes4 = sc->d_nodes4; P.tris = sc->d_tris; P.slot2dev = sc->d_slot2dev; P.shade = sc->d_shade; P.tnorm = sc->d_tnorm;
  P.tu = sc->d_tu; P.tv = sc->d_tv; P.texels = sc->d_texels; P.mats = sc->d_mats;
  P.prims = sc->d_prims; P.n_prims = sc->n_prims;
  LaunchCtx& C = sc->ctx[sc->next_ctx];
  const int ci = sc->next_ctx;
  const hipStream_t caller = st;
  if (sc->reserve_cus > 0) {
    hipStream_t ks = nullptr;
    const int mrc = masked_stream(sc, caller, &ks);
    if (mrc != RT_OK) return mrc;
    if (!C.ev_in) HIP_TRY(hipEventCreateWithFlags(&C.ev_in, hipEventDisableTiming));
    HIP_TRY(hipEventRecord(C.ev_in, caller));
    HIP_TRY(hipStreamWaitEvent(ks, C.ev_in, 0));
    st = ks;
  }
  if (C.used && !event_done(C.ev1)) {
    HIP_TRY(hipStreamWaitEvent(st, C.ev1, 0));
    HIP_TRY(hipEventSynchronize(C.ev1));
  }
  const size_t lights_at = kCtrBytes + (size_t)n_frames * sizeof(FrameDesc);
  const size_t ctl_bytes = lights_at + (size_t)p->n_lights * 6 * sizeof(double);
  if (ctl_bytes > C.ctl_cap) {
    HIP_TRY(hipFree(C.d_ctr));
    C.d_ctr = nullptr;
    HIP_TRY(hipHostFree(C.h_ctl));
    C.h_ctl = nullptr;
    sc->bytes -= (long long)C.ctl_cap;
    C.ctl_cap = 0;
    HIP_TRY(hipMalloc(reinterpret_cast<void**>(&C.d_ctr), ctl_bytes));
    HIP_TRY(hipHostMalloc(reinterpret_cast<void**>(&C.h_ctl), ctl_bytes, hipHostMallocDefault));
    C.ctl_cap = ctl_bytes;
    sc->bytes += (long long)ctl_bytes;
  }
  P.ctr = C.d_ctr;
  P.heads = reinterpret_cast<unsigned long long*>(reinterpret_cast<unsigned char*>(C.d_ctr) + kHeadsOff);
  P.wctr = C.d_wctr;
  P.n_frames = n_frames;
  P.frames = reinterpret_cast<const FrameDesc*>(reinterpret_cast<unsigned char*>(C.d_ctr) + kCtrBytes);
  P.n_gnodes = sc->n_gnodes;
  P.out_fmt = p->out_format;
  for (int k = 0; k < 3; ++k) {
    P.root_lo[k] = sc->root_lo[k]; P.root_hi[k] = sc->root_hi[k];
    P.bg[k] = p->background[k]; P.amb[k] = p->ambience[k];
  }
  P.W = p->camera.width;
  P.H = p->camera.height;
  P.n_lights = p->n_lights;
  P.max_depth = p->max_depth;
  P.lights = reinterpret_cast<const double*>(reinterpret_cast<unsigned char*>(C.d_ctr) + lights_at);
  P.guard_host = sc->d_guard;
  P.pstate = C.d_pstate;
  P.spill = C.d_spill;
  P.wavelog = C.d_wavelog;
  P.nslots = sc->nslots;
  P.spp_n = p->spp_n;
  P.row_begin = scount == 1 ? std::max(0, p->row_begin) : 0;
  P.stripe_h = p->stripe_height > 0 ? p->stripe_height : 1;
  P.stripe_count = scount;
  P.stripe_index = p->stripe_index;
  P.rows = rows;
  P.out_global = (p->flags & RT_FLAG_GLOBAL_ROWS) ? 1 : 0;
  if (P.out_global && list) return fail(RT_ERR_INVALID, "RT_FLAG_GLOBAL_ROWS is not supported by the adaptive pass");
  P.tiles_x = (P.W + kTileW - 1) / kTileW;
  P.nsamp = p->spp_n * p->spp_n;
  const bool group = list ? sample_out == nullptr : use_groups(sc, p);
  if (group) {
    P.group_log = 0;
    const int gmax = sc->spp_lanes >= 2 ? sc->spp_lanes : kGroupLanes;
    while ((1 << (P.group_log + 1)) <= std::min(P.nsamp, gmax)) P.group_log++;
    P.chunks = P.nsamp >> P.group_log;
  }
  if (fan) {
    P.group_log = 0;
    while ((1 << (P.group_log + 1)) <= std::min(fan->k, kGroupLanes)) P.group_log++;
    P.chunks = (fan->k + (1 << P.group_log) - 1) >> P.group_log;
  }
  P.frame_tiles = list ? (list_cap * (group ? 1 : P.nsamp) + 63) / 64
                       : (long long)P.tiles_x * ((rows + kTileH - 1) / kTileH);
  P.n_tiles = list ? P.frame_tiles : P.frame_tiles * n_frames;
  if (rays) P.n_tiles = P.frame_tiles = (n_rays + 63) / 64;
  if (P.n_tiles >= (1LL << 31)) return fail(RT_ERR_INVALID, "rt_launch: more than 2^31 tiles in one launch");
  P.div_row_tiles = div_magic((uint32_t)P.tiles_x * (uint32_t)n_frames);
  P.div_tiles_x = div_magic((uint32_t)P.tiles_x);
  P.div_stripe_h = div_magic((uint32_t)P.stripe_h);
  P.list = list;
  P.list_count = count;
  P.sample_out = sample_out;
  if (!list && !rays && sc->d_tile_order && sc->tile_order_n == P.n_tiles) P.tile_order = sc->d_tile_order;
  const bool debug_order = !rays && sc->d_tile_order && sc->tile_order_n == P.n_tiles;
  const bool implicit_order =
      !(p->flags & (RT_FLAG_TRAVERSAL_STATS | RT_FLAG_WIDE_STATS | RT_FLAG_TIMELINE | RT_FLAG_TILE_COST |
                    RT_FLAG_TILE_COST_TIME | RT_FLAG_NATURAL_ORDER)) &&
      !debug_order && (!sc->maps_used || sc->maps_stream == st);
  const bool cost_debug = !list && !rays && (p->flags & (RT_FLAG_TILE_COST | RT_FLAG_TILE_COST_TIME));
  const bool cost_order = !list && !rays && !group && n_frames == 1 && ((p->flags & RT_FLAG_COST_ORDER) || implicit_order);
  if (cost_order || cost_debug) {
    const long long n_pos = (long long)P.tiles_x * ((rows + kTileH - 1) / kTileH);
    if (sc->cost_cap < n_pos) {
      HIP_TRY(hipDeviceSynchronize());
      for (uint32_t*& q : sc->d_cost) { if (q) HIP_TRY(hipFree(q)); q = nullptr; }
      for (uint32_t*& q : sc->d_order) { if (q) HIP_TRY(hipFree(q)); q = nullptr; }
      sc->cost_cap = 0;
      for (uint32_t*& q : sc->d_cost) HIP_TRY(hipMalloc(reinterpret_cast<void**>(&q), (size_t)n_pos * sizeof(uint32_t)));
      for (uint32_t*& q : sc->d_order) HIP_TRY(hipMalloc(reinterpret_cast<void**>(&q), (size_t)n_pos * sizeof(uint32_t)));
      sc->cost_cap = n_pos;
      sc->cost_seq = 0;
      sc->order_for = -1;
    }
    if (sc->cost_n != n_pos || sc->cost_tiles_x != P.tiles_x) {
      sc->cost_seq = 0;
      sc->order_for = -1;
    }
    sc->cost_n = n_pos;
    sc->cost_tiles_x = P.tiles_x;
    if (sc->maps_used && sc->maps_stream != st)
      HIP_TRY(hipStreamWaitEvent(st, sc->maps_ev, 0));
    P.cost_time = (p->flags & RT_FLAG_TILE_COST) ? 0 : 1;
    if (!cost_order) {
      sc->cost_seq = 0;
      HIP_TRY(hipMemsetAsync(sc->d_cost[0], 0, (size_t)n_pos * sizeof(uint32_t), st));
      P.tile_cost = sc->d_cost[0];
      sc->cost_seq = 1;
      sc->order_for = -1;
    } else {
      const long long q = sc->cost_seq;
      if (q == 0)
        for (uint32_t* m : sc->d_cost) HIP_TRY(hipMemsetAsync(m, 0, (size_t)n_pos * sizeof(uint32_t), st));
      P.tile_cost = sc->d_cost[q % 3];
      if (sc->order_for == q && n_pos == P.n_tiles) {
        P.tile_order = sc->d_order[q % 2];
        sc->last_order_n = P.n_tiles;
        sc->last_order_buf = (int)(q % 2);
      }
      if ((n_pos + kGroups - 1) / kGroups <= kOrderMaxRange) {
        P.order_src = q >= 1 ? sc->d_cost[(q + 2) % 3] : nullptr;
        P.order_dilate = sc->order_window > 0 ? sc->order_window : sc->order_window < 0 ? 0
                         : sc->big ? 0 : kOrderDilate;
        P.next_order = sc->d_order[(q + 1) % 2];
        P.zero_map = sc->d_cost[(q + 1) % 3];
        P.n_pos = n_pos;
        if (q >= 1) sc->order_for = q + 1;
      } else {
        HIP_TRY(hipMemsetAsync(sc->d_cost[(q + 1) % 3], 0, (size_t)n_pos * sizeof(uint32_t), st));
      }
      sc->cost_seq = q + 1;
    }
  }

  const int v = fan ? kFanVariant + (sc->deep ? 1 : 0)
                : rays ? kRayVariant + (sc->deep ? 1 : 0)
                : (p->flags & RT_FLAG_TRAVERSAL_STATS) ? 2
                : (p->flags & RT_FLAG_WIDE_STATS) ? 1
                : (p->flags & RT_FLAG_TIMELINE) ? 3
                : sc->deep ? (group ? 6 : 4)
                : group ? 5 : 0;
  const int ring = variant_ring(v);
  const int n_top = sc->n_top_v[v];
  const size_t lds = lds_bytes_total(sc->stack_words, n_top, ring);
  P.n_top = n_top;
  P.top_off = (int)lds_bytes(sc->stack_words, ring);
  P.lights_off = P.top_off + n_top * (int)sizeof(GNode4);
  P.pool_off = P.lights_off + RT_MAX_LIGHTS * 6 * (int)sizeof(double);
  const long long waves_needed = fan ? ((n_rays << P.group_log) + 63) / 64 : (P.n_tiles * 64 + 63) / 64;
  int bpc = sc->blocks_per_cu[v];
  if (sc->bpc_cap > 0) bpc = std::min(bpc, sc->bpc_cap);
  auto grid_of = [&](int bpc_) {
    long long b = (long long)(sc->n_cu - sc->reserve_cus) * bpc_;
    b = std::max<long long>(1, std::min<long long>(b, (waves_needed + kBlock / 64 - 1) / (kBlock / 64)));
    b = std::min<long long>(b, (long long)(sc->nslots / kBlock));
    if (sc->grid_spare > 0)
      b = std::max<long long>(1, b - sc->grid_spare);
    return b;
  };
  const long long full_blocks = grid_of(bpc);
  if (n_frames == 1 && sc->last_ctx >= 0 && sc->last_stream != st &&
      !event_done(sc->ctx[sc->last_ctx].ev1))
    bpc = std::max(1, bpc / 2);
  const long long blocks = grid_of(bpc);

  std::memset(C.h_ctl, 0, kCtrBytes);
  FrameDesc* fd = reinterpret_cast<FrameDesc*>(C.h_ctl + kCtrBytes);
  for (int f = 0; f < n_frames; ++f) {
    std::memset(&fd[f], 0, sizeof(FrameDesc));
    for (int k = 0; k < 3; ++k) {
      fd[f].eye[k] = p[f].camera.eye[k]; fd[f].ll[k] = p[f].camera.lower_left[k];
      fd[f].xd[k] = p[f].camera.x_dir[k]; fd[f].yd[k] = p[f].camera.y_dir[k];
    }
    fd[f].out = outs[f];
  }
  double* ld = reinterpret_cast<double*>(C.h_ctl + lights_at);
  bool finite_lights = true;
  for (int i = 0; i < p->n_lights; ++i) {
    const rt_light* L = rt_params_light(p, i);
    for (int k = 0; k < 3; ++k) {
      ld[6 * i + k] = L->position[k]; ld[6 * i + 3 + k] = L->color[k];
      finite_lights = finite_lights && std::isfinite(L->color[k]);
    }
  }
  P.zero_term_lights = finite_lights ? (int)kMatZeroTerm : 0;
  HIP_TRY(hipMemcpyAsync(C.d_ctr, C.h_ctl, ctl_bytes, hipMemcpyHostToDevice, st));
  if (v == 3) {
    const size_t tb = sc->nslots / 64 * kTlCap * kTlWords * sizeof(unsigned long long);
    if (!C.d_tl) {
      HIP_TRY(hipMalloc(reinterpret_cast<void**>(&C.d_tl), tb));
      sc->bytes += (long long)tb;
    }
    HIP_TRY(hipMemsetAsync(C.d_tl, 0, tb, st));
  }
  P.tl = C.d_tl;
  if (rays) {
    P.rays = rays;
    P.n_rays = n_rays;
  }
  if (fan) {
    P.fan_dirs = fan->d_dirs;
    P.fan_bias = fan->bias;
    P.fan_k = fan->k;
    P.fan_sets = fan->n_sets;
    P.fan_seed = fan->seed;
  }
  if (rows > 0) {
    void* args[] = {&P};
    HIP_TRY(hipExtLaunchKernel(reinterpret_cast<const void*>(kVariants[v].fn), dim3((unsigned)blocks), dim3(kBlock),
                               args, lds, st, C.ev0, C.ev1, 0));
  } else {
    HIP_TRY(hipEventRecord(C.ev0, st));
    HIP_TRY(hipEventRecord(C.ev1, st));
  }
  if (st != caller) HIP_TRY(hipStreamWaitEvent(caller, C.ev1, 0));
  if (cost_order || cost_debug) {
    if (!sc->maps_ev) HIP_TRY(hipEventCreateWithFlags(&sc->maps_ev, hipEventDisableTiming));
    HIP_TRY(hipEventRecord(sc->maps_ev, st));
    sc->maps_used = true;
    sc->maps_stream = st;
  }
  C.used = true;
  C.variant = v;
  C.waves = rows > 0 ? blocks * (kBlock / 64) : 0;
// ... 297 lines not shown
  hipPointerAttribute_t at;
  void* direct = nullptr;
  if (hipPointerGetAttributes(&at, host_out) == hipSuccess && at.type == hipMemoryTypeHost) {
    if (hipHostGetDevicePointer(&direct, host_out, 0) != hipSuccess) direct = nullptr;
  }
  (void)hipGetLastError();
  if (direct) return rt_launch_compute_image(sc, p, direct, stats ? stats : &local, nullptr);
  if (sc->host_stage_bytes < bytes) {
    if (sc->d_host_stage) HIP_TRY(hipFree(sc->d_host_stage));
    sc->d_host_stage = nullptr;
    sc->host_stage_bytes = 0;
    HIP_TRY(hipMalloc(&sc->d_host_stage, bytes));
    sc->host_stage_bytes = bytes;
  }
  int rc = rt_launch_compute_image(sc, p, sc->d_host_stage, stats ? stats : &local, nullptr);
  if (rc == RT_OK) {
    const hipError_t e = hipMemcpy(host_out, sc->d_host_stage, (size_t)rows * p->camera.width * 3 * elem,
                                   hipMemcpyDeviceToHost);
    if (e != hipSuccess) rc = fail(RT_ERR_HIP, std::string("hipMemcpy D2H: ") + hipGetErrorString(e));
  }
  return rc;
}

int rt_render_adaptive_to_host(rt_scene* sc, const rt_render_params* p, int subp, double threshold, void* host_out,
                               rt_stats* st_primary, rt_stats* st_adaptive, long long* n_selected) {
  if (!sc || !p || !host_out) return fail(RT_ERR_INVALID, "rt_render_adaptive_to_host: null argument");
  if (p->flags & RT_FLAG_GLOBAL_ROWS)
    return fail(RT_ERR_INVALID, "rt_render_adaptive_to_host: RT_FLAG_GLOBAL_ROWS is not supported");
  const int W = p->camera.width, H = p->camera.height;
  if (W <= 0 || H <= 0) return fail(RT_ERR_INVALID, "bad image size");
  if (p->stripe_count > 1 || p->row_begin != 0 || (p->row_end > 0 && p->row_end != H))
    return fail(RT_ERR_INVALID, "rt_render_adaptive_to_host: needs the full frame (neighbour test), no stripes/row range");
  if (p->out_format != RT_OUT_RGB_F32 && p->out_format != RT_OUT_RGB_F64) return fail(RT_ERR_INVALID, "bad out_format");
  HIP_TRY(hipSetDevice(sc->device));
  const size_t elem = p->out_format == RT_OUT_RGB_F64 ? sizeof(double) : sizeof(float);
  const size_t bytes = (size_t)H * W * 3 * elem;
  StreamScratch scratch{nullptr, {}};
  double* prim = nullptr;
  HIP_TRY(scratch.alloc(&prim, (size_t)H * W * 3 * sizeof(double)));
  rt_render_params q = *p;
  q.out_format = RT_OUT_RGB_F64;
  int rc = rt_launch_compute_image(sc, &q, prim, st_primary, nullptr);
  if (rc != RT_OK) return rc;
  hipPointerAttribute_t at;
  void* direct = nullptr;
  if (hipPointerGetAttributes(&at, host_out) == hipSuccess && at.type == hipMemoryTypeHost) {
    if (hipHostGetDevicePointer(&direct, host_out, 0) != hipSuccess) direct = nullptr;
  }
  (void)hipGetLastError();
  if (!direct && sc->host_stage_bytes < bytes) {
    HIP_TRY(hipDeviceSynchronize());
    if (sc->d_host_stage) HIP_TRY(hipFree(sc->d_host_stage));
    sc->d_host_stage = nullptr;
    sc->host_stage_bytes = 0;
    HIP_TRY(hipMalloc(&sc->d_host_stage, bytes));
    sc->host_stage_bytes = bytes;
  }
  rc = rt_launch_adaptive(sc, p, prim, direct ? direct : sc->d_host_stage, subp, threshold, st_adaptive, n_selected,
                          nullptr);
  if (rc != RT_OK) return rc;
  if (!direct) {
    const hipError_t e = hipMemcpy(host_out, sc->d_host_stage, bytes, hipMemcpyDeviceToHost);
    if (e != hipSuccess) return fail(RT_ERR_HIP, std::string("hipMemcpy D2H: ") + hipGetErrorString(e));
  } else {
    HIP_TRY(hipStreamSynchronize(nullptr));
  }
  if (guard_tripped(sc)) return fail(RT_ERR_HIP, kGuardMsg);
  return RT_OK;
}

int rt_debug_counters(rt_scene* sc, unsigned long long* out, int n) {
  if (!sc || !out || n <= 0) return fail(RT_ERR_INVALID, "rt_debug_counters: bad argument");
  HIP_TRY(hipSetDevice(sc->device));
  HIP_TRY(hipDeviceSynchronize());
  unsigned long long c[kCtrWords];
  if (sc->last_ctx < 0) return fail(RT_ERR_INVALID, "rt_debug_counters: no launch recorded");
  const int rc = read_counters(sc->ctx[sc->last_ctx], c);
  if (rc != RT_OK) return rc;
  for (int i = 0; i < n && i < kCtrWords; ++i) out[i] = c[i];
  return std::min(n, kCtrWords);
}

int rt_debug_blocks_per_cu(rt_scene* sc, int variant) {
  if (!sc || variant < 0 || variant >= kNumVariants) return fail(RT_ERR_INVALID, "rt_debug_blocks_per_cu: bad argument");
  return sc->blocks_per_cu[variant];
}

long long rt_debug_tile_cost(rt_scene* sc, unsigned int* out, long long n) {
  if (!sc) return fail(RT_ERR_INVALID, "rt_debug_tile_cost: null scene");
  if (sc->cost_seq < 1) return 0;
  if (hipSetDevice(sc->device) != hipSuccess || hipDeviceSynchronize() != hipSuccess)
    return fail(RT_ERR_HIP, "rt_debug_tile_cost: synchronize failed");
  const long long m = std::min(n, sc->cost_n);
  if (out && m > 0 &&
      hipMemcpy(out, sc->d_cost[(sc->cost_seq - 1) % 3], (size_t)m * sizeof(uint32_t), hipMemcpyDeviceToHost) != hipSuccess)
    return fail(RT_ERR_HIP, "rt_debug_tile_cost: copy failed");
  return sc->cost_n;
}

long long rt_debug_last_tile_order(rt_scene* sc, unsigned int* out, long long n) {
  if (!sc) return fail(RT_ERR_INVALID, "rt_debug_last_tile_order: null scene");
  if (!sc->d_order[0] || sc->last_order_n <= 0) return 0;
  if (hipSetDevice(sc->device) != hipSuccess || hipDeviceSynchronize() != hipSuccess)
    return fail(RT_ERR_HIP, "rt_debug_last_tile_order: synchronize failed");
  const long long m = std::min(n, sc->last_order_n);
  if (out && m > 0 &&
      hipMemcpy(out, sc->d_order[sc->last_order_buf], (size_t)m * sizeof(uint32_t), hipMemcpyDeviceToHost) != hipSuccess)
    return fail(RT_ERR_HIP, "rt_debug_last_tile_order: copy failed");
  return sc->last_order_n;
}

int rt_debug_set_tile_order(rt_scene* sc, const unsigned int* order, long long n) {
  if (!sc || n < 0 || (n > 0 && !order)) return fail(RT_ERR_INVALID, "rt_debug_set_tile_order: bad argument");
  if (hipSetDevice(sc->device) != hipSuccess || hipDeviceSynchronize() != hipSuccess)
    return fail(RT_ERR_HIP, "rt_debug_set_tile_order: synchronize failed");
  {
    std::vector<bool> seen((size_t)n, false);
    for (long long i = 0; i < n; ++i) {
      if ((long long)order[i] >= n || seen[order[i]])
        return fail(RT_ERR_INVALID, "rt_debug_set_tile_order: not a permutation");
      seen[order[i]] = true;
    }
  }
  if (sc->d_tile_order) (void)hipFree(sc->d_tile_order);
  sc->d_tile_order = nullptr;
  sc->tile_order_n = 0;
  if (n == 0) return RT_OK;
  if (hipMalloc(reinterpret_cast<void**>(&sc->d_tile_order), (size_t)n * sizeof(uint32_t)) != hipSuccess ||
      hipMemcpy(sc->d_tile_order, order, (size_t)n * sizeof(uint32_t), hipMemcpyHostToDevice) != hipSuccess)
    return fail(RT_ERR_HIP, "rt_debug_set_tile_order: upload failed");
  sc->tile_order_n = n;
  return RT_OK;
}

long long rt_debug_timeline(rt_scene* sc, unsigned long long* out, long long n) {
  if (!sc || !out || n <= 0) return fail(RT_ERR_INVALID, "rt_debug_timeline: bad argument");
  HIP_TRY(hipSetDevice(sc->device));
  HIP_TRY(hipDeviceSynchronize());
  if (sc->last_ctx < 0 || !sc->ctx[sc->last_ctx].d_tl || sc->ctx[sc->last_ctx].variant != 3)
    return fail(RT_ERR_INVALID, "rt_debug_timeline: the last launch was not an RT_FLAG_TIMELINE launch");
  const long long words = std::min<long long>(n, (long long)(sc->nslots / 64 * kTlCap * kTlWords));
  HIP_TRY(hipMemcpy(out, sc->ctx[sc->last_ctx].d_tl, (size_t)words * sizeof(unsigned long long), hipMemcpyDeviceToHost));
  return words;
}

long long rt_debug_wave_log(rt_scene* sc, unsigned long long* out, long long n) {
  if (!sc || !out || n <= 0) return fail(RT_ERR_INVALID, "rt_debug_wave_log: bad argument");
  HIP_TRY(hipSetDevice(sc->device));
  HIP_TRY(hipDeviceSynchronize());
  const long long words = std::min<long long>(n, (long long)(sc->nslots / 64 * 4));
  if (sc->last_ctx < 0) return fail(RT_ERR_INVALID, "rt_debug_wave_log: no launch recorded");
  HIP_TRY(hipMemcpy(out, sc->ctx[sc->last_ctx].d_wavelog, (size_t)words * sizeof(unsigned long long),
                    hipMemcpyDeviceToHost));
  return words;
}

int rt_tile_shape(int* tile_w, int* tile_h) {
  if (!tile_w || !tile_h) return fail(RT_ERR_INVALID, "rt_tile_shape: null argument");
  *tile_w = kTileW;
  *tile_h = kTileH;
  return RT_OK;
}

int rt_ipc_get_handle(const void* d_ptr, unsigned char* handle, unsigned long long* offset) {
  if (!d_ptr || !handle || !offset) return fail(RT_ERR_INVALID, "rt_ipc_get_handle: null argument");
  static_assert(sizeof(hipIpcMemHandle_t) == RT_IPC_HANDLE_BYTES, "IPC handle size");
  hipDeviceptr_t base = nullptr;
// ... 63 lines not shown
  GNode4 n;
  std::memset(&n, 0, sizeof n);
  for (int c = 0; c < 4; ++c) {
    const float lo = c == 0 ? -1e30f : INFINITY, hi = c == 0 ? 1e30f : -INFINITY;
    n.lox[c] = n.loy[c] = n.loz[c] = lo;
    n.hix[c] = n.hiy[c] = n.hiz[c] = hi;
    n.ref[c] = c == 0 ? 0u : kEmpty;
  }
  HIP_TRY(hipMemcpy(sc->d_nodes4, &n, sizeof n, hipMemcpyHostToDevice));
  return RT_OK;
}

int rt_scene_set_analytic(rt_scene* sc, const rt_sphere* spheres, int n_spheres, const rt_plane* planes,
                          int n_planes) {
  if (!sc) return fail(RT_ERR_INVALID, "rt_scene_set_analytic: null scene");
  if (n_spheres < 0 || n_planes < 0 || (n_spheres > 0 && !spheres) || (n_planes > 0 && !planes))
    return fail(RT_ERR_INVALID, "rt_scene_set_analytic: bad primitive arrays");
  const long long n = (long long)n_spheres + n_planes;
  if (n > (1 << 20)) return fail(RT_ERR_INVALID, "rt_scene_set_analytic: more than 2^20 primitives");
  std::vector<GMat> mats = sc->mesh_mats;
  std::vector<GPrim> prims((size_t)n);
  auto add_mat = [&](const rt_material& m) {
    GMat G;
    std::memset(&G, 0, sizeof G);
    for (int k = 0; k < 3; ++k) {
      G.ka[k] = m.ambient[k];
      G.kd[k] = m.diffuse[k];
      G.ks[k] = m.specular[k];
    }
    G.shininess = m.shininess;
    G.mirror = m.mirror;
    G.shadowable = m.shadowable;
    G.draw_mode = RT_DRAW_FLAT;
    G.tex_w = -1;
    G.flags = mat_flags(G);
    mats.push_back(G);
    return (int)mats.size() - 1;
  };
  for (int i = 0; i < n_spheres; ++i) {
    GPrim& G = prims[i];
    std::memset(&G, 0, sizeof G);
    for (int k = 0; k < 3; ++k) G.c[k] = spheres[i].center[k];
    G.r = spheres[i].radius;
    G.type = kPrimSphere;
    G.mat = add_mat(spheres[i].material);
  }
  for (int i = 0; i < n_planes; ++i) {
    GPrim& G = prims[(size_t)n_spheres + i];
    std::memset(&G, 0, sizeof G);
    for (int k = 0; k < 3; ++k) {
      G.c[k] = planes[i].center[k];
      G.n[k] = planes[i].normal[k];
    }
    G.type = kPrimPlane;
    G.mat = add_mat(planes[i].material);
  }
  HIP_TRY(hipSetDevice(sc->device));
  HIP_TRY(hipDeviceSynchronize());
  long long bytes = 0;
  GMat* d_mats = nullptr;
  GPrim* d_prims = nullptr;
  int rc = upload(&d_mats, mats, bytes);
  if (rc == RT_OK) rc = upload(&d_prims, prims, bytes);
  if (rc != RT_OK) {
    if (d_mats) (void)hipFree(d_mats);
    if (d_prims) (void)hipFree(d_prims);
    return rc;
  }
  if (sc->d_mats) (void)hipFree(sc->d_mats);
  if (sc->d_prims) (void)hipFree(sc->d_prims);
  sc->d_mats = d_mats;
  sc->d_prims = d_prims;
  sc->n_prims = (int)n;
  sc->bytes += bytes - sc->table_bytes;
  sc->table_bytes = bytes;
  return RT_OK;
}

void rt_scene_free(rt_scene* sc) {
  if (!sc) return;
  (void)hipSetDevice(sc->device);
  (void)hipDeviceSynchronize();
  void* ptrs[] = {sc->d_cost[0], sc->d_cost[1], sc->d_cost[2], sc->d_order[0], sc->d_order[1], sc->d_tile_order, sc->d_host_stage, sc->d_nodes, sc->d_nodes4, sc->d_tris, sc->d_shade, sc->d_tnorm, sc->d_tu,
                  sc->d_tv, sc->d_texels, sc->d_mats, sc->d_slot2dev, sc->d_prims};
  for (void* q : ptrs)
    if (q) (void)hipFree(q);
  if (sc->h_guard) (void)hipHostFree(sc->h_guard);
  query_ring_free(sc);
  update_state_free(sc);
  normal_state_free(sc);
  for (LaunchCtx& c : sc->ctx) {
    void* cp[] = {c.d_ctr, c.d_pstate, c.d_spill, c.d_wavelog, c.d_tl, c.d_wctr};
    for (void* q : cp)
      if (q) (void)hipFree(q);
    if (c.h_ctl) (void)hipHostFree(c.h_ctl);
    if (c.ev0) (void)hipEventDestroy(c.ev0);
    if (c.ev1) (void)hipEventDestroy(c.ev1);
  }
  if (sc->maps_ev) (void)hipEventDestroy(sc->maps_ev);
  for (LaunchCtx& c : sc->ctx)
    if (c.ev_in) (void)hipEventDestroy(c.ev_in);
  for (int i = 0; i < rt_scene::kMaskedStreams; ++i)
    if (sc->masked[i]) (void)hipStreamDestroy(sc->masked[i]);
  delete sc;
}

}

#endif
```

my-raytracer_amd/rtamd/__init__.py:

```python
import ctypes as C
import os
from pathlib import Path

import numpy as np

from . import abi
from .abi import RT_OK, RT_OUT_RGB_F32, RT_OUT_RGB_F64, RT_FLAG_TRAVERSAL_STATS, RT_FLAG_WIDE_STATS, RT_FLAG_TIMELINE

PKG_ROOT = Path(__file__).resolve().parent.parent
LIB_DIR = PKG_ROOT / "lib"
HOST_LIB = LIB_DIR / "librt_host.so"
HIP_LIB = Path(os.environ.get("RTAMD_HIP_LIB", LIB_DIR / "librt_hip.so"))
MULTI_LIB = LIB_DIR / "librt_multi.so"

_host = None
_hip = None
_multi = None


class RtError(RuntimeError):
    pass


def host_lib():
# ... 714 lines not shown
            raise ValueError("dirs must be an [n_sets, k, 3] float64 array")
        for name, x, dims, last in (("points", points, 2, 8), ("dirs", dirs, 3, 3)):
            if isinstance(x, np.ndarray):
                continue
            if not (isinstance(x, torch.Tensor) and x.dtype == torch.float64 and x.dim() == dims
                    and x.shape[-1] == last and x.is_contiguous() and x.device == dev):
                shape = "[n, 8]" if dims == 2 else "[n_sets, k, 3]"
                raise ValueError(f"{name} must be a contiguous {shape} float64 tensor on {dev}")
        if host_in:
            points = torch.from_numpy(np.ascontiguousarray(points, dtype=np.float64)).to(dev)
        if dirs_uploaded:
            dirs = torch.from_numpy(np.ascontiguousarray(dirs, dtype=np.float64)).to(dev)
        n = points.shape[0]
        a = abi.AoParams(k=dirs.shape[1], n_sets=dirs.shape[0], seed=int(seed) & 0xffffffff, bias=float(bias),
                         d_dirs=dirs.data_ptr() if dirs.numel() else None)
        dtype = torch.float64 if params.out_format == RT_OUT_RGB_F64 else torch.float32
        out = torch.zeros((n, 3), dtype=dtype, device=dev)
        st = abi.Stats() if stats else None
        if stream:
            torch.cuda.current_stream(dev).synchronize()
        _check_hip(fn(self._h, C.byref(params), C.c_void_p(points.data_ptr() if n else None), n, C.byref(a),
                      C.c_void_p(out.data_ptr() if n else None), C.byref(st) if st is not None else None,
                      C.c_void_p(stream) if stream else None), "rt_trace_gather")
        if stream and (host_in or dirs_uploaded):
            torch.cuda.ExternalStream(stream, device=dev).synchronize()
        if host_in:
            torch.cuda.synchronize(dev)
            out = out.cpu().numpy()
        return (out, st) if stats else out

    def camera(self, params, hits=True, points=False, order="row", point_tmax=float("inf"), stats=False,
               stream=None):
        import torch

        fn = _camera_fn("rt_trace_camera")
        if order not in _CAMERA_ORDERS:
            raise ValueError(f"order must be one of {sorted(_CAMERA_ORDERS)}")
        if not (hits or points):
            raise ValueError("nothing requested: hits and points are both False")
        dev = torch.device(f"cuda:{self.device}")
        n = rows_in_shard(params) * params.camera.width
        if not 0 <= n <= abi.RT_CAMERA_MAX_PIXELS:
            raise ValueError("the shard holds more than RT_CAMERA_MAX_PIXELS pixels")
        ht = torch.zeros((n, 8), dtype=torch.float64, device=dev) if hits else None
        pt = torch.zeros((n, 8), dtype=torch.float64, device=dev) if points else None
        out = abi.CameraOut(d_hits=ht.data_ptr() if hits else None, d_points=pt.data_ptr() if points else None,
                            order=_CAMERA_ORDERS[order], point_tmax=float(point_tmax))
        st = abi.QueryStats() if stats else None
        if stream:
            torch.cuda.current_stream(dev).synchronize()
        if n:
            _check_hip(fn(self._h, C.byref(params), C.byref(out), C.byref(st) if st is not None else None,
                          C.c_void_p(stream) if stream else None), "rt_trace_camera")
        res = {}
        if hits:
            res["hits"] = _hit_views(ht)
        if points:
            res["points"] = pt
        return (res, st) if stats else res

    def _fan_image(self, params, radius, trace):
        import torch

        rows, W = rows_in_shard(params), params.camera.width
        pts = self.camera(params, hits=False, points=True, order="tile", point_tmax=radius)["points"]
        vals = trace(pts)
        perm = torch.from_numpy(tile_major(W, rows)).to(vals.device)
        img = torch.zeros_like(vals)
        img[perm] = vals
        return img

    def ao_image(self, params, dirs, seed=0, bias=0.0, radius=float("inf")):
        import torch

        k = dirs.shape[1]
        img = self._fan_image(params, radius, lambda pts: self.ao(pts, dirs, seed=seed, bias=bias))
        return (img.to(torch.float64) / float(k)).reshape(rows_in_shard(params), params.camera.width)

    def gather_image(self, params, dirs, seed=0, bias=0.0):
        img = self._fan_image(params, float("inf"), lambda pts: self.gather(pts, dirs, params, seed=seed, bias=bias))
        return img.reshape(rows_in_shard(params), params.camera.width, 3)

    def debug_counters(self):
        buf = (C.c_ulonglong * 40)()
        n = hip_lib().rt_debug_counters(self._h, buf, 40)
        if n < 0:
            _check_hip(n, "rt_debug_counters")
        names = {16: "node_iters", 17: "node_lanes", 18: "leaf_iters", 19: "leaf_lanes", 20: "trav_cycles",
                 21: "shade_cycles", 22: "fetch_cycles", 23: "outer_iters", 24: "trav_rounds", 25: "trav_round_lanes",
                 26: "stack_spills", 27: "node_lines", 28: "leaf_lines", 29: "big_leaf_tests",
                 30: "node_lds_iters", 32: "gnode_uniform_iters", 33: "gnode_distinct", 34: "leaf_uniform_iters",
                 35: "anyhit_tri_tests", 36: "anyhit_own_record_tests", 37: "shadow_rays_skipped"}
        return {v: int(buf[k]) for k, v in names.items()}

    def wave_log(self, max_waves=1 << 16):
        buf = np.zeros(4 * max_waves, dtype=np.uint64)
        n = hip_lib().rt_debug_wave_log(self._h, buf.ctypes.data_as(C.POINTER(C.c_ulonglong)), len(buf))
        if n < 0:
            _check_hip(int(n), "rt_debug_wave_log")
        return buf[:n].reshape(-1, 4)

    def timeline(self, max_waves=1 << 14):
        buf = np.zeros(8 * 256 * max_waves, dtype=np.uint64)
        n = hip_lib().rt_debug_timeline(self._h, buf.ctypes.data_as(C.POINTER(C.c_ulonglong)), len(buf))
        if n < 0:
            _check_hip(int(n), "rt_debug_timeline")
        return buf[:n].reshape(-1, 256, 8)

    def last_kernel_ms(self):
        ms = C.c_float(0.0)
        _check_hip(hip_lib().rt_last_kernel_ms(self._h, C.byref(ms)), "rt_last_kernel_ms")
        return ms.value

    def status(self):
        return int(hip_lib().rt_scene_status(self._h))

    def last_grid(self):
        b, f = C.c_longlong(0), C.c_longlong(0)
        _check_hip(hip_lib().rt_debug_last_grid(self._h, C.byref(b), C.byref(f)), "rt_debug_last_grid")
        return b.value, f.value

    def debug_corrupt_hierarchy(self):
        _check_hip(hip_lib().rt_debug_corrupt_hierarchy(self._h), "rt_debug_corrupt_hierarchy")


def _hit_views(out):
    import torch

    ints = out.view(torch.int32)
    return {"t": out[:, 0], "alpha": out[:, 1], "beta": out[:, 2], "normal": out[:, 3:6],
            "slot": ints[:, 12], "mesh": ints[:, 13], "prim": ints[:, 14]}


HIT_KEY_DTYPE = np.dtype([("t", "<f8"), ("slot", "<i4"), ("reserved_", "<i4")])


def _hit_keys(after, n, dev):
    import torch

    if isinstance(after, (tuple, list)):
        if len(after) != 2:
            raise ValueError("after must be a pair (t, slot), a HIT_KEY_DTYPE array or [n, 2] key rows")
        t, slot = after
        if isinstance(t, torch.Tensor) or isinstance(slot, torch.Tensor):
            t = torch.as_tensor(t, dtype=torch.float64, device=dev).reshape(-1).contiguous()
            slot = torch.as_tensor(slot, device=dev).reshape(-1).to(torch.int64)
            if t.shape[0] != n or slot.shape[0] != n:
                raise ValueError(f"after must hold {n} keys")
            return torch.stack([t.view(torch.int64), slot & 0xFFFFFFFF], dim=1).contiguous()
        rec = np.zeros(np.shape(t), dtype=HIT_KEY_DTYPE)
        rec["t"], rec["slot"] = t, slot
        after = rec
    if isinstance(after, np.ndarray):
        if after.dtype == HIT_KEY_DTYPE and after.shape == (n,):
            words = np.ascontiguousarray(after).view(np.int64).reshape(n, 2)
        elif after.dtype == np.float64 and after.shape == (n, 2):
            words = np.ascontiguousarray(after).view(np.int64)
        else:
            raise ValueError(f"after must be {n} keys: a HIT_KEY_DTYPE array [n] or float64 rows [n, 2]")
        return torch.from_numpy(words.copy()).to(dev)
    if (isinstance(after, torch.Tensor) and after.dtype in (torch.float64, torch.int64) and tuple(after.shape) == (n, 2)
            and after.is_contiguous() and after.device == dev):
        return after.view(torch.int64)
    raise ValueError(f"after must be {n} keys: a pair (t, slot), a HIT_KEY_DTYPE array or contiguous [n, 2] rows on {dev}")


def _hits_fn(name):
    try:
        return getattr(hip_lib(), name)
    except AttributeError:
        raise RtError(f"{name}: not exported by this librt_hip.so (RTAMD_HIP_LIB)") from None


def _update_fn(name):
    try:
# ... 358 lines not shown
```

my-raytracer_amd/rtamd/abi.py:

```python
import ctypes as C

c_double3 = C.c_double * 3

RT_OK = 0
RT_ERR_INVALID = -1
RT_ERR_HIP = -2
RT_ERR_UNSUPPORTED = -3
RT_MAX_COORDINATE = 2.0 ** 61
RT_MAX_LIGHTS = 16
RT_LIGHTS_LIMIT = 1 << 20
RT_MAX_FRAMES = 128
RT_DRAW_FLAT = 0
RT_DRAW_PHONG = 1
RT_OUT_RGB_F32 = 0
RT_OUT_RGB_F64 = 1
RT_FLAG_TRAVERSAL_STATS = 1
RT_FLAG_WIDE_STATS = 2
RT_FLAG_TIMELINE = 4
RT_FLAG_TILE_COST = 8
RT_FLAG_TILE_COST_TIME = 16
RT_FLAG_COST_ORDER = 32
RT_FLAG_NATURAL_ORDER = 64
RT_FLAG_GLOBAL_ROWS = 128
RT_IPC_HANDLE_BYTES = 64
# ... 94 lines not shown
        n = len(lights)
        self.n_lights = n
        if n <= RT_MAX_LIGHTS:
            self.lights_ext = None
            arr = self.lights
        else:
            arr = (Light * n)()
            self._lights_keep = arr
            self.lights_ext = C.cast(arr, C.POINTER(Light))
        for i, (pos, col) in enumerate(lights):
            for k in range(3):
                arr[i].position[k] = pos[k]
                arr[i].color[k] = col[k]


class Stats(C.Structure):
    _fields_ = [("primary_rays", C.c_longlong), ("shadow_rays", C.c_longlong),
                ("reflection_rays", C.c_longlong), ("node_visits", C.c_longlong),
                ("tri_tests", C.c_longlong), ("closest_hits", C.c_longlong),
                ("pixels", C.c_longlong), ("reserved_", C.c_longlong)]

    def as_dict(self):
        return {name: int(getattr(self, name)) for name, _ in self._fields_ if name != "reserved_"}


class Ray(C.Structure):
    _fields_ = [("o", c_double3), ("d", c_double3), ("tmax", C.c_double), ("reserved_", C.c_double)]


class Hit(C.Structure):
    _fields_ = [("t", C.c_double), ("alpha", C.c_double), ("beta", C.c_double), ("normal", c_double3),
                ("slot", C.c_int), ("mesh", C.c_int), ("prim", C.c_int), ("reserved_", C.c_int)]


class HitKey(C.Structure):
    _fields_ = [("t", C.c_double), ("slot", C.c_int), ("reserved_", C.c_int)]


class QueryStats(C.Structure):
    _fields_ = [("rays", C.c_longlong), ("hits", C.c_longlong), ("stack_spills", C.c_longlong),
                ("watchdog", C.c_longlong), ("reserved_", C.c_longlong * 4)]

    def as_dict(self):
        return {name: int(getattr(self, name)) for name, _ in self._fields_ if name != "reserved_"}


class AoParams(C.Structure):
    _fields_ = [("k", C.c_int), ("n_sets", C.c_int), ("seed", C.c_uint), ("reserved_", C.c_int),
                ("bias", C.c_double), ("d_dirs", C.c_void_p)]


class CameraOut(C.Structure):
    _fields_ = [("d_hits", C.c_void_p), ("d_points", C.c_void_p), ("order", C.c_int), ("reserved_", C.c_int),
                ("point_tmax", C.c_double)]


RT_IMAGE_NODES4, RT_IMAGE_TRIS, RT_IMAGE_TNORM = 0, 1, 2
RT_UPDATE_RECLIP = 1


class SceneUpdate(C.Structure):
    _fields_ = [("n_vertices", C.c_longlong), ("n_triangles", C.c_longlong), ("vertex_pos", C.POINTER(C.c_double)),
                ("vertex_normals", C.POINTER(C.c_double)), ("face_normals", C.POINTER(C.c_double)),
                ("reserved_", C.c_longlong * 3)]


class ScenePositions(C.Structure):
    _fields_ = [("n_vertices", C.c_longlong), ("vertex_pos", C.c_void_p), ("on_device", C.c_int),
                ("reserved_", C.c_int), ("reserved2_", C.c_longlong * 3)]


class GenParams(C.Structure):
    _fields_ = [("width", C.c_int), ("height", C.c_int), ("n_triangles", C.c_longlong),
                ("seed", C.c_ulonglong), ("max_depth", C.c_int), ("detail", C.c_int)]


class UploadOptions(C.Structure):
    _fields_ = [("device_tree", C.c_int), ("build_threads", C.c_int), ("stack_ring", C.c_int),
                ("lds_treelet", C.c_int), ("collapse", C.c_int), ("sbvh_leaf_max", C.c_int),
                ("sbvh_bins", C.c_int), ("blocks_per_cu", C.c_int), ("grid_spare", C.c_int),
                ("verbose", C.c_int), ("sbvh_alpha", C.c_double), ("sbvh_budget", C.c_double),
                ("sbvh_c_trav", C.c_double), ("collapse_c_tri", C.c_double), ("reserve_cus", C.c_int),
                ("order_window", C.c_int), ("spp_lanes", C.c_int), ("tree_opt", C.c_int),
                ("reserved_", C.c_int * 4)]


RT_TREE_OPT_PASSES, RT_TREE_OPT_MAX = 3, 64
RT_TREE_BAD_UNION, RT_TREE_BAD_LEAF, RT_TREE_BAD_RECORDS, RT_TREE_BAD_IDS, RT_TREE_BAD_FIXPOINT = 1, 2, 4, 8, 16


class TreeReport(C.Structure):
    _fields_ = [("binary_nodes", C.c_longlong), ("wide_nodes", C.c_longlong), ("records", C.c_longlong),
                ("moved", C.c_longlong), ("sah_before", C.c_double), ("sah_after", C.c_double),
                ("dp_before", C.c_double), ("dp_after", C.c_double), ("seconds", C.c_double),
                ("passes", C.c_int), ("stack4", C.c_int), ("invalid", C.c_uint), ("converged", C.c_int)]

    def as_dict(self):
        return {name: getattr(self, name) for name, _ in self._fields_}


RT_TREE_SAH, RT_TREE_REFERENCE, RT_TREE_SBVH = 0, 1, 2
RT_COLLAPSE_GREEDY, RT_COLLAPSE_SAH, RT_COLLAPSE_BY_SIZE = 0, 1, 2

HIP_SYMBOLS = {
    "rt_scene_upload": (C.c_int, [C.POINTER(SceneSoA), C.POINTER(BvhSoA), C.c_int, C.POINTER(C.c_void_p)]),
    "rt_upload_options_init": (None, [C.POINTER(UploadOptions)]),
    "rt_scene_upload_ex": (C.c_int, [C.POINTER(SceneSoA), C.POINTER(BvhSoA), C.c_int, C.POINTER(UploadOptions),
                                     C.POINTER(C.c_void_p)]),
    "rt_scene_upload_multi": (C.c_int, [C.POINTER(SceneSoA), C.POINTER(BvhSoA), C.POINTER(C.c_int), C.c_int,
                                        C.POINTER(UploadOptions), C.POINTER(C.c_void_p)]),
    "rt_scene_set_analytic": (C.c_int, [C.c_void_p, C.POINTER(Sphere), C.c_int, C.POINTER(Plane), C.c_int]),
    "rt_scene_device_bytes": (C.c_longlong, [C.c_void_p]),
    "rt_scene_upload_seconds": (C.c_int, [C.c_void_p, C.POINTER(C.c_double), C.POINTER(C.c_double)]),
    "rt_rows_in_shard": (C.c_int, [C.POINTER(RenderParams)]),
    "rt_launch_compute_image": (C.c_int, [C.c_void_p, C.POINTER(RenderParams), C.c_void_p,
                                          C.POINTER(Stats), C.c_void_p]),
    "rt_launch_frames": (C.c_int, [C.c_void_p, C.POINTER(RenderParams), C.c_int, C.POINTER(C.c_void_p),
                                   C.POINTER(Stats), C.c_void_p]),
    "rt_launch_adaptive": (C.c_int, [C.c_void_p, C.POINTER(RenderParams), C.c_void_p, C.c_void_p, C.c_int,
                                     C.c_double, C.POINTER(Stats), C.POINTER(C.c_longlong), C.c_void_p]),
    "rt_launch_adaptive_shard": (C.c_int, [C.c_void_p, C.POINTER(RenderParams), C.c_void_p, C.c_void_p,
                                           C.c_void_p, C.c_int, C.c_double, C.POINTER(Stats),
                                           C.POINTER(C.c_longlong), C.c_void_p]),
    "rt_launch_adaptive_frames": (C.c_int, [C.c_void_p, C.POINTER(RenderParams), C.c_int, C.POINTER(C.c_void_p),
                                            C.POINTER(C.c_void_p), C.c_int, C.c_double, C.POINTER(Stats),
                                            C.POINTER(C.c_longlong), C.c_void_p]),
    "rt_adaptive_halo_rows": (C.c_int, [C.POINTER(RenderParams), C.POINTER(C.c_int), C.c_int]),
    "rt_render_to_host": (C.c_int, [C.c_void_p, C.POINTER(RenderParams), C.c_void_p, C.POINTER(Stats)]),
    "rt_render_adaptive_to_host": (C.c_int, [C.c_void_p, C.POINTER(RenderParams), C.c_int, C.c_double, C.c_void_p,
                                             C.POINTER(Stats), C.POINTER(Stats), C.POINTER(C.c_longlong)]),
    "rt_trace_closest": (C.c_int, [C.c_void_p, C.c_void_p, C.c_longlong, C.c_void_p, C.POINTER(QueryStats),
                                   C.c_void_p]),
    "rt_trace_occluded": (C.c_int, [C.c_void_p, C.c_void_p, C.c_longlong, C.c_void_p, C.POINTER(QueryStats),
                                    C.c_void_p]),
    "rt_trace_hits": (C.c_int, [C.c_void_p, C.c_void_p, C.c_longlong, C.c_int, C.c_void_p, C.c_void_p, C.c_void_p,
                                C.POINTER(QueryStats), C.c_void_p]),
    "rt_trace_radiance": (C.c_int, [C.c_void_p, C.POINTER(RenderParams), C.c_void_p, C.c_longlong, C.c_void_p,
                                    C.POINTER(Stats), C.c_void_p]),
    "rt_scene_bounds": (C.c_int, [C.c_void_p, C.POINTER(C.c_double), C.POINTER(C.c_double)]),
    "rt_ray_order_workspace_bytes": (C.c_size_t, [C.c_longlong]),
    "rt_ray_keys_host": (C.c_int, [C.POINTER(C.c_double), C.POINTER(C.c_double), C.c_void_p, C.c_longlong, C.c_int,
                                   C.POINTER(C.c_uint)]),
    "rt_ray_order": (C.c_int, [C.c_void_p, C.c_void_p, C.c_longlong, C.c_int, C.c_void_p, C.c_void_p, C.c_void_p,
                               C.c_void_p]),
    "rt_permute_rows": (C.c_int, [C.c_void_p, C.c_void_p, C.c_void_p, C.c_longlong, C.c_int, C.c_int, C.c_int,
                                  C.c_void_p]),
    "rt_debug_set_order_grid": (C.c_int, [C.c_void_p, C.c_int]),
    "rt_trace_ao": (C.c_int, [C.c_void_p, C.c_void_p, C.c_longlong, C.POINTER(AoParams), C.c_void_p,
                              C.POINTER(QueryStats), C.c_void_p]),
    "rt_ao_rays_host": (C.c_int, [C.c_void_p, C.c_longlong, C.POINTER(AoParams), C.c_void_p]),
    "rt_trace_gather": (C.c_int, [C.c_void_p, C.POINTER(RenderParams), C.c_void_p, C.c_longlong, C.POINTER(AoParams),
                                  C.c_void_p, C.POINTER(Stats), C.c_void_p]),
    "rt_trace_camera": (C.c_int, [C.c_void_p, C.POINTER(RenderParams), C.POINTER(CameraOut), C.POINTER(QueryStats),
                                  C.c_void_p]),
    "rt_camera_rays_host": (C.c_int, [C.POINTER(RenderParams), C.c_int, C.c_void_p]),
    "rt_surface_points_host": (C.c_int, [C.c_void_p, C.c_void_p, C.c_longlong, C.c_double, C.c_void_p]),
    "rt_scene_update_vertices": (C.c_int, [C.c_void_p, C.POINTER(SceneUpdate), C.c_void_p]),
    "rt_debug_scene_image": (C.c_longlong, [C.c_void_p, C.c_int, C.c_void_p, C.c_longlong]),
    "rt_scene_update_vertices_ex": (C.c_int, [C.c_void_p, C.POINTER(SceneUpdate), C.c_uint, C.c_void_p]),
    "rt_debug_clip_regions": (C.c_longlong, [C.POINTER(SceneSoA), C.POINTER(BvhSoA), C.POINTER(UploadOptions),
                                             C.POINTER(C.c_double), C.POINTER(C.c_int), C.c_longlong]),
    "rt_reclip_box_host": (C.c_int, [C.POINTER(C.c_double)] * 6),
    "rt_scene_set_triangle_order": (C.c_int, [C.c_void_p, C.POINTER(C.c_int), C.c_longlong]),
    "rt_scene_update_positions": (C.c_int, [C.c_void_p, C.POINTER(ScenePositions), C.c_uint, C.c_void_p]),
    "rt_normals_host": (C.c_int, [C.POINTER(C.c_int), C.POINTER(C.c_int), C.c_longlong, C.c_longlong,
                                  C.POINTER(C.c_double), C.POINTER(C.c_double), C.POINTER(C.c_double)]),
    "rt_last_kernel_ms": (C.c_int, [C.c_void_p, C.POINTER(C.c_float)]),
    "rt_tile_shape": (C.c_int, [C.POINTER(C.c_int), C.POINTER(C.c_int)]),
    "rt_ipc_get_handle": (C.c_int, [C.c_void_p, C.c_char_p, C.POINTER(C.c_ulonglong)]),
    "rt_ipc_open": (C.c_int, [C.c_char_p, C.c_ulonglong, C.c_int, C.c_int, C.POINTER(C.c_void_p)]),
    "rt_ipc_close": (C.c_int, [C.c_void_p, C.c_ulonglong]),
    "rt_debug_counters": (C.c_int, [C.c_void_p, C.POINTER(C.c_ulonglong), C.c_int]),
    "rt_debug_wave_log": (C.c_longlong, [C.c_void_p, C.POINTER(C.c_ulonglong), C.c_longlong]),
    "rt_debug_timeline": (C.c_longlong, [C.c_void_p, C.POINTER(C.c_ulonglong), C.c_longlong]),
    "rt_debug_tile_cost": (C.c_longlong, [C.c_void_p, C.POINTER(C.c_uint), C.c_longlong]),
    "rt_debug_set_tile_order": (C.c_int, [C.c_void_p, C.POINTER(C.c_uint), C.c_longlong]),
    "rt_debug_last_tile_order": (C.c_longlong, [C.c_void_p, C.POINTER(C.c_uint), C.c_longlong]),
    "rt_debug_blocks_per_cu": (C.c_int, [C.c_void_p, C.c_int]),
    "rt_debug_last_grid": (C.c_int, [C.c_void_p, C.POINTER(C.c_longlong), C.POINTER(C.c_longlong)]),
    "rt_debug_corrupt_hierarchy": (C.c_int, [C.c_void_p]),
    "rt_debug_tree_report": (C.c_int, [C.POINTER(SceneSoA), C.POINTER(BvhSoA), C.POINTER(UploadOptions),
                                       C.POINTER(TreeReport)]),
    "rt_scene_status": (C.c_int, [C.c_void_p]),
    "rt_scene_free": (None, [C.c_void_p]),
    "rt_last_error": (C.c_char_p, []),
    "rt_build_info": (C.c_char_p, []),
}

HOST_SYMBOLS = {
    "rt_host_load": (C.c_int, [C.c_char_p, C.POINTER(C.c_void_p)]),
    "rt_host_generate": (C.c_int, [C.c_char_p, C.POINTER(GenParams), C.POINTER(C.c_void_p)]),
    "rt_host_raw": (C.POINTER(RawScene), [C.c_void_p]),
    "rt_host_prepare": (C.c_int, [C.c_void_p, C.POINTER(C.c_double)]),
    "rt_host_prepare_ex": (C.c_int, [C.c_void_p, C.c_int, C.POINTER(C.c_double)]),
    "rt_host_update_vertices": (C.c_int, [C.c_void_p, C.POINTER(C.c_double), C.c_longlong]),
    "rt_host_slot_triangles": (C.POINTER(C.c_int), [C.c_void_p]),
    "rt_host_soa": (C.POINTER(SceneSoA), [C.c_void_p]),
    "rt_host_bvh": (C.POINTER(BvhSoA), [C.c_void_p]),
    "rt_host_camera": (C.c_int, [C.c_void_p, C.c_int, C.c_int, C.POINTER(Camera)]),
    "rt_host_render_params": (C.c_int, [C.c_void_p, C.c_int, C.c_int, C.c_int, C.POINTER(RenderParams)]),
    "rt_host_save": (C.c_int, [C.c_void_p, C.c_char_p]),
    "rt_write_ppm": (C.c_int, [C.c_char_p, C.POINTER(C.c_float), C.c_int, C.c_int]),
    "rt_host_triangle_count": (C.c_longlong, [C.c_void_p]),
    "rt_host_bvh_depth": (C.c_int, [C.c_void_p]),
    "rt_host_free": (None, [C.c_void_p]),
    "rt_host_last_error": (C.c_char_p, []),
}


MULTI_SYMBOLS = {
    "rt_multi_create": (C.c_int, [C.POINTER(SceneSoA), C.POINTER(BvhSoA), C.POINTER(C.c_int), C.c_int,
                                  C.POINTER(UploadOptions), C.POINTER(C.c_void_p)]),
    "rt_multi_device_count": (C.c_int, [C.c_void_p]),
    "rt_multi_set_assembly": (C.c_int, [C.c_void_p, C.c_int]),
    "rt_multi_assembly": (C.c_int, [C.c_void_p]),
    "rt_multi_debug_inject": (C.c_int, [C.c_void_p, C.c_int]),
    "rt_multi_render": (C.c_int, [C.c_void_p, C.POINTER(RenderParams), C.c_int, C.c_void_p, C.POINTER(Stats),
                                  C.POINTER(C.c_double)]),
    "rt_multi_render_frames": (C.c_int, [C.c_void_p, C.POINTER(RenderParams), C.c_int, C.c_int,
                                         C.POINTER(C.c_void_p), C.POINTER(Stats), C.POINTER(C.c_double)]),
    "rt_multi_render_to_host": (C.c_int, [C.c_void_p, C.POINTER(RenderParams), C.c_int, C.c_void_p,
                                          C.POINTER(Stats), C.POINTER(C.c_double)]),
    "rt_multi_max_rows": (C.c_int, [C.c_int, C.c_int, C.c_int]),
    "rt_multi_interleave_host": (C.c_int, [C.c_void_p, C.c_void_p, C.c_int, C.c_int, C.c_int, C.c_int, C.c_int,
                                           C.c_int]),
    "rt_multi_interleave_frames_host": (C.c_int, [C.c_void_p, C.POINTER(C.c_void_p), C.c_int, C.c_int, C.c_int,
                                                  C.c_int, C.c_int, C.c_int, C.c_int]),
    "rt_multi_free": (None, [C.c_void_p]),
    "rt_multi_last_error": (C.c_char_p, []),
}


def bind(lib, table, partial=False):
    for name, (res, args) in table.items():
        if (partial or name.startswith("rt_debug_")) and not hasattr(lib, name):
            continue
        fn = getattr(lib, name)
        fn.restype = res
        fn.argtypes = args
    return lib
```

Baseline: 28310 Mrays/s.

## Certify shadow rays with per-light cube depth maps to skip BVH traversal

Adds a host-built cube-map per point light for static scenes. Each texel stores a conservative nearest-occluder bound and an occluded-distance bound. In the new render kernel variants, a shadow ray first looks up its texel: if it is certified lit or certified occluded, BVH any-hit traversal is skipped, otherwise it traces as before. Maps are built when a light position repeats between launches and are cached on the device in up to four slots. The cost is a host build pass, extra device memory, one 16-byte load per shadow ray and more kernel variants. Correctness depends on the float tolerances used in certification.

```diff
diff --git a/include/rt_hip.h b/include/rt_hip.h
--- a/include/rt_hip.h
+++ b/include/rt_hip.h
@@ -129,10 +129,12 @@
   int order_window;
   int spp_lanes;
   int tree_opt;
-  int reserved_[4];
+  int light_map;
+  int reserved_[3];
 } rt_upload_options;
 
 enum { RT_TREE_OPT_PASSES = 3, RT_TREE_OPT_MAX = 64 };
+enum { RT_LIGHT_MAP_MIN = 16, RT_LIGHT_MAP_MAX = 2048, RT_LIGHT_MAPS = 4 };
 
 void rt_upload_options_init(rt_upload_options* opt);
 
@@ -351,6 +353,11 @@
 int rt_debug_tree_report(const rt_scene_soa* soa, const rt_bvh_soa* bvh, const rt_upload_options* opt,
                          rt_tree_report* out);
 
+long long rt_debug_light_map(const rt_scene_soa* soa, const double* light, int R, int build_threads,
+                             void* out, long long bytes);
+int rt_debug_light_map_certify(const void* map, int R, const double* light, long long n,
+                               const double* points, const int* slots, unsigned char* out);
+
 long long rt_debug_timeline(rt_scene* scene, unsigned long long* out, long long n);
 
 int rt_tile_shape(int* tile_w, int* tile_h);
diff --git a/my-raytracer_amd/csrc/device/rt_render.hip b/my-raytracer_amd/csrc/device/rt_render.hip
--- a/my-raytracer_amd/csrc/device/rt_render.hip
+++ b/my-raytracer_amd/csrc/device/rt_render.hip
@@ -1,4 +1,4 @@
-#ifndef RT_RAY_LIST_PASS
+#if !defined(RT_RAY_LIST_PASS) && !defined(RT_LM_PASS)
 #include <hip/hip_runtime.h>
 #include <hip/hip_ext.h>
 
@@ -19,6 +19,7 @@
 
 #include "../../../include/rt_hip.h"
 #include "../host/device_image.hpp"
+#include "../host/light_map.hpp"
 #include "rt_layout.hpp"
 
 #pragma clang fp contract(off)
@@ -55,7 +56,7 @@
 constexpr bool kOneHit = (RT_STACK_FAST & 8) != 0, kMaskCnt = (RT_STACK_FAST & 32) != 0;
 static_assert((RT_STACK_FAST & ~47) == 0, "RT_STACK_FAST: bits 1, 2, 4, 8 and 32");
 constexpr bool kRoomTest = kFastSort || kFastAny;
-constexpr int kCtrWords = 42;
+constexpr int kCtrWords = 43;
 constexpr int kShortStack = 8;
 constexpr int kSlotDoubles = 10;
 constexpr int kTopNodes = (40960 - kBlock * (kSlotDoubles * 8 + (2 + kShortStack) * 4) - RT_MAX_LIGHTS * 48 - 64) / 128;
@@ -134,10 +135,17 @@
   CD_LEAF_LINES, CD_BIG_LEAF_TESTS, CD_NODE_LDS_ITERS, CD_GUARD = 31,
   CD_GNODE_UNIFORM = 32, CD_GNODE_DISTINCT, CD_LEAF_UNIFORM, CD_ANYHIT_TRIS, CD_OWN_TRIS,
   CD_ZERO_TERM,
+  CD_CERT_LIT,
   CT_ORDER_JOBS = 39,
-  CD_SLOW_PUSH = 40, CD_SLOW_POP
+  CD_SLOW_PUSH = 40, CD_SLOW_POP,
+  CD_CERT_OCC = 42
 };
 static_assert(kCtrWords * sizeof(unsigned long long) <= 512, "the counter words end where the work heads begin");
+constexpr int kWaveCtrs = 4;
+constexpr int kLightMaps = RT_LIGHT_MAPS;
+#ifndef RT_LIGHT_MAP
+#define RT_LIGHT_MAP 1
+#endif
 constexpr unsigned kGuardIters = 1u << 24;
 constexpr unsigned kTravGuard = 1u << 24;
 __device__ __forceinline__ void trip_watchdog(unsigned long long* ctr, unsigned int* host_word) {
@@ -261,6 +269,10 @@
     long long n_pos;
     long long n_rays;
   };
+  const uint4* lmap;
+  unsigned long long* lmctr;
+  uint32_t lmap_slots;
+  int lmap_R;
 };
 
 struct D3 {
@@ -559,23 +571,33 @@
 
 #endif
 
+#ifdef RT_LM_PASS
+#define RT_KN(a) a##_lm_kernel
+#else
+#define RT_KN(a) a##_kernel
+#endif
 #ifndef RT_RAY_LIST_PASS
 template <int WIDTH, bool STATS, bool TL = false, int RING = kShortStack, bool GRP = false>
-__global__ void __launch_bounds__(kBlock, kWavesPerEU * 256 / kBlock) render_kernel(KParams P) {
+__global__ void __launch_bounds__(kBlock, kWavesPerEU * 256 / kBlock) RT_KN(render)(KParams P) {
   constexpr bool RAYS = false, FAN = false;
 #define RT_GROUPS_ON group_log
 #elif !defined(RT_FAN_PASS)
 template <int RING>
-__global__ void __launch_bounds__(kBlock, kWavesPerEU * 256 / kBlock) radiance_kernel(KParams P) {
+__global__ void __launch_bounds__(kBlock, kWavesPerEU * 256 / kBlock) RT_KN(radiance)(KParams P) {
   constexpr int WIDTH = 4;
   constexpr bool STATS = false, TL = false, GRP = false, RAYS = true, FAN = false;
 #define RT_GROUPS_ON group_log
 #else
 template <int RING>
-__global__ void __launch_bounds__(kBlock, kWavesPerEU * 256 / kBlock) gather_kernel(KParams P) {
+__global__ void __launch_bounds__(kBlock, kWavesPerEU * 256 / kBlock) RT_KN(gather)(KParams P) {
   constexpr int WIDTH = 4;
   constexpr bool STATS = false, TL = false, GRP = true, RAYS = true, FAN = true;
 #define RT_GROUPS_ON true
+#endif
+#ifdef RT_LM_PASS
+  constexpr bool LM = true;
+#else
+  constexpr bool LM = STATS || TL;
 #endif
   static_assert(RING >= kMigWords && (RING & (RING - 1)) == 0, "ring: a power of two holding the migration words");
   constexpr int kRingMask = RING - 1;
@@ -681,6 +703,9 @@
   uint32_t htask = kTaskNone;
   unsigned c_primary = 0, c_shadow = 0, c_refl = 0, c_hits = 0;
   unsigned n_zero_term = 0;
+  if constexpr (RT_LIGHT_MAP != 0 && LM) {
+    if (lane == 0) P.lmctr[(size_t)blockIdx.x * (kBlock / 64) + (threadIdx.x >> 6)] = 0ull;
+  }
   unsigned long long c_nodes = 0, c_tris = 0;
   unsigned long long d_node_it = 0, d_node_ln = 0, d_leaf_it = 0, d_leaf_ln = 0;
   unsigned long long d_trav = 0, d_shade = 0, d_fetch = 0, d_outer = 0, d_round_it = 0, d_round_ln = 0;
@@ -999,6 +1024,7 @@
       D3 rd = d3(lds_d[3 * kBlock + src], lds_d[4 * kBlock + src], lds_d[5 * kBlock + src]);
       double tlim = lds_d[6 * kBlock + src];
       bool zero_term = false;
+      int cert = 0;
       if (anyhit) {
         const int j = (state == ST_SHADOW) ? light + (kp > 0 ? (batch_end >> kHelpShift) + kp : 0)
                                            : (int)((htask >> 11) & 0xFFFFFu);
@@ -1013,6 +1039,33 @@
         ro = add(hp, scl(1e-4, l));
         rd = nrm(l);
         tlim = nl;
+        if constexpr (RT_LIGHT_MAP != 0 && LM) {
+        if (P.lmap_slots != 0xffffffffu && j < kLightMaps && !zero_term) {
+          int mz = 0;
+          asm volatile("" : "+s"(mz));
+          const uint32_t mslots = P.lmap_slots;
+          const uint32_t ms = (mslots >> (8 * j)) & 0xffu;
+          const float dx = (float)-rd.x, dy = (float)-rd.y, dz = (float)-rd.z;
+          const float ax = fabsf(dx), ay = fabsf(dy), az = fabsf(dz);
+          const int axis = (ax >= ay && ax >= az) ? 0 : (ay >= az ? 1 : 2);
+          const float dm = axis == 0 ? dx : (axis == 1 ? dy : dz);
+          const float db = axis == 0 ? dy : (axis == 1 ? dz : dx);
+          const float dc = axis == 0 ? dz : (axis == 1 ? dx : dy);
+          const float am = fabsf(dm);
+          if (ms != 0xffu && am > 0.0f) {
+            const int R_ = *(&P.lmap_R + mz);
+            const float half = 0.5f * (float)R_;
+            int ti = (int)floorf((db / am + 1.0f) * half), tj = (int)floorf((dc / am + 1.0f) * half);
+            ti = min(max(ti, 0), R_ - 1);
+            tj = min(max(tj, 0), R_ - 1);
+            const uint32_t face = ms * 6u + 2u * (uint32_t)axis + (dm < 0.0f ? 1u : 0u);
+            const uint4 tx = (*(&P.lmap + mz))[((size_t)face * (size_t)R_ + (size_t)tj) * (size_t)R_ + (size_t)ti];
+            const float nlf = (float)tlim;
+            if (nlf * 1.00001f < __uint_as_float(tx.y)) cert = 1;
+            else if (nlf > __uint_as_float(tx.z) * 1.00001f + 1e-3f) cert = 2;
+          }
+        }
+        }
       } else if (act && state == ST_HCLOSEST) {
         const D3 hp = add(ro, scl(tlim, rd));
         const D3 hn = d3(lds_d[7 * kBlock + src], lds_d[8 * kBlock + src], lds_d[9 * kBlock + src]);
@@ -1029,7 +1082,17 @@
       best = kNoHit;
       best_slot = kNoHit;
       n_zero_term += (unsigned)__popcll(wballot(zero_term));
-      shadow_hit = !STATS && !TL && zero_term;
+      shadow_hit = !STATS && !TL && (zero_term || cert == 2);
+      if constexpr (RT_LIGHT_MAP != 0 && LM) {
+        const unsigned long long n_cert =
+            (unsigned long long)__popcll(wballot(cert == 1)) | ((unsigned long long)__popcll(wballot(cert == 2)) << 32);
+        int mz2 = 0;
+        asm volatile("" : "+s"(mz2));
+        if (n_cert != 0ull && lane == 0)
+          atomicAdd(*(&P.lmctr + mz2) + ((size_t)blockIdx.x * (kBlock / 64) +
+                               (size_t)__builtin_amdgcn_readfirstlane((int)(threadIdx.x >> 6))), n_cert);
+      }
+      const bool lit_skip = RT_LIGHT_MAP != 0 && LM && !STATS && !TL && cert == 1;
       uint32_t cur = kDone;
       double t_off = 0.0;
       for (int k = 0; k < P.n_prims; ++k) {
@@ -1042,7 +1105,7 @@
           best_slot = -1;
         }
       }
-      if (act && P.n_gnodes > 0 && !shadow_hit) {
+      if (act && P.n_gnodes > 0 && !shadow_hit && !lit_skip) {
         bool miss = false;
         int pz = 0;
         asm volatile("" : "+s"(pz));
@@ -1915,7 +1978,7 @@
   unsigned long long s3 = 0, s4 = 0, s5 = 0;
   if (STATS) { s3 = wave_sum(c_nodes); s4 = wave_sum(c_tris); s5 = wave_sum(c_hits); }
   if (lane == 0) {
-    unsigned long long* wc = P.wctr + 4 * ((size_t)blockIdx.x * (kBlock / 64) + (threadIdx.x >> 6));
+    unsigned long long* wc = P.wctr + kWaveCtrs * ((size_t)blockIdx.x * (kBlock / 64) + (threadIdx.x >> 6));
     wc[0] = s0; wc[1] = s1; wc[2] = s2; wc[3] = n_zero_term;
     if (STATS) {
       atomicAdd(&P.ctr[CS_NODES], s3);
@@ -1976,14 +2039,20 @@
   }
 }
 #undef RT_GROUPS_ON
-
-#ifndef RT_RAY_LIST_PASS
+#undef RT_KN
+
+#if !defined(RT_RAY_LIST_PASS) && !defined(RT_LM_PASS)
 #define RT_RAY_LIST_PASS 1
 #include __FILE_NAME__
 #define RT_FAN_PASS 1
 #include __FILE_NAME__
 #undef RT_FAN_PASS
 #undef RT_RAY_LIST_PASS
+#if RT_LIGHT_MAP
+#define RT_LM_PASS 1
+#include __FILE_NAME__
+#undef RT_LM_PASS
+#endif
 
 __device__ __forceinline__ double nsq3(const double* a, const double* b) {
   const double dx = a[0] - b[0], dy = a[1] - b[1], dz = a[2] - b[2];
@@ -2138,14 +2207,28 @@
     {radiance_kernel<16>, false},
     {gather_kernel<kShortStack>, false},
     {gather_kernel<16>, false},
+#if RT_LIGHT_MAP
+    {render_lm_kernel<4, false>, false},
+    {render_lm_kernel<4, false, false, 16>, false},
+    {render_lm_kernel<4, false, false, kShortStack, true>, false},
+    {render_lm_kernel<4, false, false, 16, true>, false},
+#endif
 };
-constexpr int kNumVariants = 11;
+constexpr int kNumVariants = RT_LIGHT_MAP ? 15 : 11;
+constexpr int kLmVariant = 11;
+constexpr int kLmBase[4] = {0, 4, 5, 6};
+inline int lm_variant(int v) {
+  for (int k = 0; k < kNumVariants - kLmVariant; ++k)
+    if (kLmBase[k] == v) return kLmVariant + k;
+  return v;
+}
 constexpr int kRayVariant = 7;
 constexpr int kFanVariant = 9;
 constexpr bool kSppLanesDefault = true;
 constexpr int kGroupLanes = 32;
 constexpr int kRingDeep = 16;
 inline int variant_ring(int v) {
+  if (v >= kLmVariant) v = kLmBase[v - kLmVariant];
   return (v == 4 || v == 6 || v == kRayVariant + 1 || v == kFanVariant + 1) ? kRingDeep : kShortStack;
 }
 size_t lds_bytes(int , int ring = kShortStack) {
@@ -2172,6 +2255,7 @@
   uint32_t* d_spill = nullptr;
   unsigned long long* d_wavelog = nullptr;
   unsigned long long* d_wctr = nullptr;
+  unsigned long long* d_lmctr = nullptr;
   unsigned long long* d_tl = nullptr;
   hipEvent_t ev0 = nullptr, ev1 = nullptr;
   hipEvent_t ev_in = nullptr;
@@ -2254,6 +2338,18 @@
   NormalState* normals = nullptr;
   bool updated = false;
   std::shared_ptr<const ClipTable> clip;
+  int lm_R = 0;
+  int lm_threads = 1;
+  std::vector<double> lm_pos;
+  std::vector<int> lm_idx;
+  uint4* d_lmap = nullptr;
+  bool lm_have[kLightMaps] = {};
+  double lm_key[kLightMaps][3] = {};
+  long long lm_used[kLightMaps] = {};
+  long long lm_seq = 0;
+  int lm_prev_n = 0;
+  double lm_prev[kLightMaps][3] = {};
+  double lm_build_s = 0.0;
 };
 
 namespace {
@@ -2288,6 +2384,92 @@
 }
 
 namespace {
+void keep_light_map_input(rt_scene* sc, const rt_scene_soa* s, const rt_upload_options& o) {
+  const long long nt = s->n_vertex_idx / 3;
+  if (!RT_LIGHT_MAP || o.light_map < 0 || nt == 0 || nt >= (1LL << 18)) return;
+  sc->lm_R = o.light_map > 0 ? o.light_map : kLightMapDefaultR;
+  sc->lm_threads = o.build_threads > 0 ? std::min(o.build_threads, 64)
+                                       : std::max(1, std::min((int)std::thread::hardware_concurrency(), 16));
+  sc->lm_pos.resize((size_t)nt * 9);
+  sc->lm_idx.resize((size_t)nt * 3);
+  for (long long i = 0; i < 3 * nt; ++i) {
+    const double* v = s->vertex_pos + 3 * (size_t)s->vertex_idx[i];
+    sc->lm_pos[3 * i] = v[0]; sc->lm_pos[3 * i + 1] = v[1]; sc->lm_pos[3 * i + 2] = v[2];
+    sc->lm_idx[i] = (int)i;
+  }
+}
+
+int light_maps_for_launch(rt_scene* sc, const rt_render_params* p, KParams& P) {
+  P.lmap = nullptr;
+  P.lmap_slots = 0xffffffffu;
+  P.lmap_R = 0;
+  const int n = std::min(p->n_lights, kLightMaps);
+  if (sc->updated && sc->lm_R > 0) {
+    if (sc->d_lmap) {
+      HIP_TRY(hipDeviceSynchronize());
+      HIP_TRY(hipFree(sc->d_lmap));
+      sc->d_lmap = nullptr;
+    }
+    std::vector<double>().swap(sc->lm_pos);
+    std::vector<int>().swap(sc->lm_idx);
+    for (bool& h : sc->lm_have) h = false;
+    sc->lm_R = 0;
+  }
+  const bool on = sc->lm_R > 0 && !sc->updated && sc->n_prims == 0 && !sc->lm_pos.empty();
+  if (on) {
+    sc->lm_seq++;
+    const size_t texels = (size_t)6 * sc->lm_R * sc->lm_R;
+    for (int j = 0; j < n; ++j) {
+      const double* pos = rt_params_light(p, j)->position;
+      int slot = -1;
+      for (int m = 0; m < kLightMaps; ++m)
+        if (sc->lm_have[m] && std::memcmp(sc->lm_key[m], pos, sizeof sc->lm_key[m]) == 0) slot = m;
+      if (slot < 0 && j < sc->lm_prev_n && std::memcmp(sc->lm_prev[j], pos, sizeof sc->lm_prev[j]) == 0) {
+        rt_scene_soa soa;
+        std::memset(&soa, 0, sizeof soa);
+        soa.n_vertices = (int)(sc->lm_pos.size() / 3);
+        soa.n_vertex_idx = (int)sc->lm_idx.size();
+        soa.vertex_pos = sc->lm_pos.data();
+        soa.vertex_idx = sc->lm_idx.data();
+        LightMap M;
+        const int rc = build_light_map(&soa, pos, sc->lm_R, sc->lm_threads, M);
+        sc->lm_build_s += M.seconds;
+        if (rc == RT_OK) {
+          if (!sc->d_lmap) {
+            HIP_TRY(hipMalloc(reinterpret_cast<void**>(&sc->d_lmap), kLightMaps * texels * sizeof(uint4)));
+          }
+          int m = 0;
+          for (int k = 0; k < kLightMaps; ++k) {
+            if (!sc->lm_have[k]) { m = k; break; }
+            if (sc->lm_used[k] < sc->lm_used[m]) m = k;
+          }
+          if (sc->lm_have[m]) {
+            if (sc->lm_used[m] == sc->lm_seq) m = -1;
+            else HIP_TRY(hipDeviceSynchronize());
+          }
+          if (m >= 0) {
+            HIP_TRY(hipMemcpy(sc->d_lmap + (size_t)m * texels, M.tex.data(), texels * sizeof(uint4), hipMemcpyHostToDevice));
+            sc->lm_have[m] = true;
+            std::memcpy(sc->lm_key[m], pos, sizeof sc->lm_key[m]);
+            slot = m;
+          }
+        }
+      }
+      if (slot >= 0) {
+        sc->lm_used[slot] = sc->lm_seq;
+        P.lmap_slots = (P.lmap_slots & ~(0xffu << (8 * j))) | ((uint32_t)slot << (8 * j));
+      }
+    }
+    if (P.lmap_slots != 0xffffffffu) {
+      P.lmap = sc->d_lmap;
+      P.lmap_R = sc->lm_R;
+    }
+  }
+  sc->lm_prev_n = n;
+  for (int j = 0; j < n; ++j) std::memcpy(sc->lm_prev[j], rt_params_light(p, j)->position, sizeof sc->lm_prev[j]);
+  return RT_OK;
+}
+
 int upload_image(const SceneImage& I, const rt_upload_options& opt, int device, rt_scene** out) {
   HIP_TRY(hipSetDevice(device));
   {
@@ -2381,20 +2563,23 @@
   for (LaunchCtx& c : sc->ctx) {
     const size_t pb = sc->nslots * kRegions * kLaneRec;
     const size_t wb = sc->nslots / 64 * 4 * sizeof(unsigned long long);
+    const size_t wcb = sc->nslots / 64 * kWaveCtrs * sizeof(unsigned long long);
+    const size_t lcb = sc->nslots / 64 * sizeof(unsigned long long);
     const size_t sb = sc->stack_words > kShortStack ? sc->nslots * (size_t)sc->stack_words * sizeof(uint32_t) : 0;
     c.ctl_cap = kCtlBytes + RT_MAX_LIGHTS * 6 * sizeof(double);
     if (hipMalloc(reinterpret_cast<void**>(&c.d_ctr), c.ctl_cap) != hipSuccess ||
         hipHostMalloc(reinterpret_cast<void**>(&c.h_ctl), c.ctl_cap, hipHostMallocDefault) != hipSuccess ||
         hipMalloc(reinterpret_cast<void**>(&c.d_pstate), pb) != hipSuccess ||
         hipMalloc(reinterpret_cast<void**>(&c.d_wavelog), wb) != hipSuccess ||
-        hipMalloc(reinterpret_cast<void**>(&c.d_wctr), wb) != hipSuccess ||
+        hipMalloc(reinterpret_cast<void**>(&c.d_wctr), wcb) != hipSuccess ||
+        hipMalloc(reinterpret_cast<void**>(&c.d_lmctr), lcb) != hipSuccess ||
         (sb > 0 && hipMalloc(reinterpret_cast<void**>(&c.d_spill), sb) != hipSuccess) ||
         hipMemset(c.d_ctr, 0, kCtrBytes) != hipSuccess ||
         hipEventCreate(&c.ev0) != hipSuccess || hipEventCreate(&c.ev1) != hipSuccess) {
       rt_scene_free(sc);
       return fail(RT_ERR_HIP, "allocation of launch contexts failed");
     }
-    sc->bytes += (long long)(c.ctl_cap + pb + 2 * wb + sb);
+    sc->bytes += (long long)(c.ctl_cap + pb + wb + wcb + lcb + sb);
   }
   *out = sc;
   return RT_OK;
@@ -2416,6 +2601,8 @@
     return fail(RT_ERR_INVALID, "rt_scene_upload: spp_lanes must be -1, 0, 1 or a power of two <= 64");
   if (o.stack_ring != 0 && o.stack_ring != 8 && o.stack_ring != 16)
     return fail(RT_ERR_INVALID, "rt_scene_upload: stack_ring must be 0, 8 or 16");
+  if (o.light_map < -1 || (o.light_map > 0 && (o.light_map < RT_LIGHT_MAP_MIN || o.light_map > RT_LIGHT_MAP_MAX)))
+    return fail(RT_ERR_INVALID, "rt_scene_upload: light_map must be -1, 0 or in [RT_LIGHT_MAP_MIN, RT_LIGHT_MAP_MAX]");
   if (o.blocks_per_cu < 0 || o.grid_spare < 0 || o.build_threads < 0)
     return fail(RT_ERR_INVALID, "rt_scene_upload: negative blocks_per_cu / grid_spare / build_threads");
   if (o.sbvh_leaf_max < 0 || o.sbvh_leaf_max > 8 || o.sbvh_bins < 2 || o.sbvh_bins > 128 ||
@@ -2446,6 +2633,7 @@
   const auto t1 = std::chrono::steady_clock::now();
   rc = upload_image(I, o, device, out);
   if (rc == RT_OK) {
+    keep_light_map_input(*out, s, o);
     (*out)->build_s = std::chrono::duration<double>(t1 - t0).count();
     (*out)->copy_s = std::chrono::duration<double>(std::chrono::steady_clock::now() - t1).count();
   }
@@ -2475,6 +2663,7 @@
         errs[g] = g_error;
       } else {
         outs[g]->build_s = build_s;
+        keep_light_map_input(outs[g], s, o);
         outs[g]->copy_s = std::chrono::duration<double>(std::chrono::steady_clock::now() - t1).count();
       }
     });
@@ -2521,13 +2710,21 @@
 int read_counters(const LaunchCtx& C, unsigned long long* c) {
   HIP_TRY(hipMemcpy(c, C.d_ctr, kCtrWords * sizeof(unsigned long long), hipMemcpyDeviceToHost));
   if (C.waves > 0) {
-    std::vector<unsigned long long> w((size_t)C.waves * 4);
+    std::vector<unsigned long long> w((size_t)C.waves * kWaveCtrs);
     HIP_TRY(hipMemcpy(w.data(), C.d_wctr, w.size() * sizeof(unsigned long long), hipMemcpyDeviceToHost));
-    for (size_t i = 0; i < w.size(); i += 4) {
+    for (size_t i = 0; i < w.size(); i += kWaveCtrs) {
       c[CS_PRIMARY] += w[i];
       c[CS_SHADOW] += w[i + 1];
       c[CS_REFLECT] += w[i + 2];
       c[CD_ZERO_TERM] += w[i + 3];
+    }
+    if (RT_LIGHT_MAP && (C.variant >= kLmVariant || (C.variant >= 1 && C.variant <= 3))) {
+      std::vector<unsigned long long> m((size_t)C.waves);
+      HIP_TRY(hipMemcpy(m.data(), C.d_lmctr, m.size() * sizeof(unsigned long long), hipMemcpyDeviceToHost));
+      for (unsigned long long x : m) {
+        c[CD_CERT_LIT] += x & 0xffffffffull;
+        c[CD_CERT_OCC] += x >> 32;
+      }
     }
   }
   return RT_OK;
@@ -2654,6 +2851,7 @@
   P.ctr = C.d_ctr;
   P.heads = reinterpret_cast<unsigned long long*>(reinterpret_cast<unsigned char*>(C.d_ctr) + kHeadsOff);
   P.wctr = C.d_wctr;
+  P.lmctr = C.d_lmctr;
   P.n_frames = n_frames;
   P.frames = reinterpret_cast<const FrameDesc*>(reinterpret_cast<unsigned char*>(C.d_ctr) + kCtrBytes);
   P.n_gnodes = sc->n_gnodes;
@@ -2766,13 +2964,19 @@
     }
   }
 
-  const int v = fan ? kFanVariant + (sc->deep ? 1 : 0)
+  {
+    P.lmap_slots = 0xffffffffu;
+    const int lrc = (rays || fan) ? RT_OK : light_maps_for_launch(sc, p, P);
+    if (lrc != RT_OK) return lrc;
+  }
+  const int v0 = fan ? kFanVariant + (sc->deep ? 1 : 0)
                 : rays ? kRayVariant + (sc->deep ? 1 : 0)
                 : (p->flags & RT_FLAG_TRAVERSAL_STATS) ? 2
                 : (p->flags & RT_FLAG_WIDE_STATS) ? 1
                 : (p->flags & RT_FLAG_TIMELINE) ? 3
                 : sc->deep ? (group ? 6 : 4)
                 : group ? 5 : 0;
+  const int v = P.lmap_slots != 0xffffffffu ? lm_variant(v0) : v0;
   const int ring = variant_ring(v);
   const int n_top = sc->n_top_v[v];
   const size_t lds = lds_bytes_total(sc->stack_words, n_top, ring);
@@ -3236,7 +3440,7 @@
 }
 
 int rt_debug_blocks_per_cu(rt_scene* sc, int variant) {
-  if (!sc || variant < 0 || variant >= kNumVariants) return fail(RT_ERR_INVALID, "rt_debug_blocks_per_cu: bad argument");
+  if (!sc || variant < 0 || variant >= kLmVariant) return fail(RT_ERR_INVALID, "rt_debug_blocks_per_cu: bad argument");
   return sc->blocks_per_cu[variant];
 }
 
@@ -3466,7 +3670,7 @@
   (void)hipSetDevice(sc->device);
   (void)hipDeviceSynchronize();
   void* ptrs[] = {sc->d_cost[0], sc->d_cost[1], sc->d_cost[2], sc->d_order[0], sc->d_order[1], sc->d_tile_order, sc->d_host_stage, sc->d_nodes, sc->d_nodes4, sc->d_tris, sc->d_shade, sc->d_tnorm, sc->d_tu,
-                  sc->d_tv, sc->d_texels, sc->d_mats, sc->d_slot2dev, sc->d_prims};
+                  sc->d_tv, sc->d_texels, sc->d_mats, sc->d_slot2dev, sc->d_prims, sc->d_lmap};
   for (void* q : ptrs)
     if (q) (void)hipFree(q);
   if (sc->h_guard) (void)hipHostFree(sc->h_guard);
@@ -3474,7 +3678,7 @@
   update_state_free(sc);
   normal_state_free(sc);
   for (LaunchCtx& c : sc->ctx) {
-    void* cp[] = {c.d_ctr, c.d_pstate, c.d_spill, c.d_wavelog, c.d_tl, c.d_wctr};
+    void* cp[] = {c.d_ctr, c.d_pstate, c.d_spill, c.d_wavelog, c.d_tl, c.d_wctr, c.d_lmctr};
     for (void* q : cp)
       if (q) (void)hipFree(q);
     if (c.h_ctl) (void)hipHostFree(c.h_ctl);
diff --git a/my-raytracer_amd/csrc/host/light_map.cpp b/my-raytracer_amd/csrc/host/light_map.cpp
--- /dev/null
+++ b/my-raytracer_amd/csrc/host/light_map.cpp
@@ -0,0 +1,325 @@
+#include "light_map.hpp"
+
+#include <algorithm>
+#include <atomic>
+#include <chrono>
+#include <limits>
+#include <thread>
+
+namespace rtk {
+namespace {
+
+constexpr double kInf = std::numeric_limits<double>::infinity();
+constexpr double kEps = 2.220446049250313e-16;
+
+struct V3 { double x, y, z; };
+inline V3 operator-(V3 a, V3 b) { return {a.x - b.x, a.y - b.y, a.z - b.z}; }
+inline V3 operator+(V3 a, V3 b) { return {a.x + b.x, a.y + b.y, a.z + b.z}; }
+inline V3 operator*(double s, V3 a) { return {s * a.x, s * a.y, s * a.z}; }
+inline double dot(V3 a, V3 b) { return a.x * b.x + a.y * b.y + a.z * b.z; }
+inline V3 cross(V3 a, V3 b) { return {a.y * b.z - a.z * b.y, a.z * b.x - a.x * b.z, a.x * b.y - a.y * b.x}; }
+inline double len(V3 a) { return std::sqrt(dot(a, a)); }
+inline double comp(V3 a, int k) { return k == 0 ? a.x : (k == 1 ? a.y : a.z); }
+
+double origin_distance(V3 a, V3 b, V3 c) {
+  const V3 ab = b - a, ac = c - a, ap = -1.0 * a;
+  const double d1 = dot(ab, ap), d2 = dot(ac, ap);
+  if (d1 <= 0.0 && d2 <= 0.0) return len(a);
+  const V3 bp = -1.0 * b;
+  const double d3 = dot(ab, bp), d4 = dot(ac, bp);
+  if (d3 >= 0.0 && d4 <= d3) return len(b);
+  const double vc = d1 * d4 - d3 * d2;
+  if (vc <= 0.0 && d1 >= 0.0 && d3 <= 0.0) return len(a + (d1 / (d1 - d3)) * ab);
+  const V3 cp = -1.0 * c;
+  const double d5 = dot(ab, cp), d6 = dot(ac, cp);
+  if (d6 >= 0.0 && d5 <= d6) return len(c);
+  const double vb = d5 * d2 - d1 * d6;
+  if (vb <= 0.0 && d2 >= 0.0 && d6 <= 0.0) return len(a + (d2 / (d2 - d6)) * ac);
+  const double va = d3 * d6 - d5 * d4;
+  if (va <= 0.0 && (d4 - d3) >= 0.0 && (d5 - d6) >= 0.0)
+    return len(b + ((d4 - d3) / ((d4 - d3) + (d5 - d6))) * (c - b));
+  const double den = 1.0 / (va + vb + vc);
+  return len(a + (vb * den) * ab + (vc * den) * ac);
+}
+
+struct TriPre {
+  V3 p[3];
+  V3 N[3];
+  V3 Nsum;
+  double tol[3];
+  double absD;
+  double area2;
+  double dist;
+  double lmax;
+  bool skip;
+  bool edge_on;
+  bool self_safe;
+  bool cover_ok;
+};
+
+struct Entry { int tri; int16_t i0, i1, j0, j1; };
+
+inline float round_down_f(double x) {
+  float f = (float)x;
+  if ((double)f > x) f = std::nextafterf(f, -std::numeric_limits<float>::infinity());
+  return f;
+}
+inline float round_up_f(double x) {
+  float f = (float)x;
+  if ((double)f < x) f = std::nextafterf(f, std::numeric_limits<float>::infinity());
+  return f;
+}
+
+void prepare_triangle(const rt_scene_soa* s, const double L[3], int t, TriPre& T) {
+  for (int k = 0; k < 3; ++k) {
+    const double* v = s->vertex_pos + 3 * (size_t)s->vertex_idx[3 * (size_t)t + k];
+    T.p[k] = {v[0] - L[0], v[1] - L[1], v[2] - L[2]};
+  }
+  T.skip = false;
+  for (int k = 0; k < 3; ++k)
+    if (!std::isfinite(T.p[k].x) || !std::isfinite(T.p[k].y) || !std::isfinite(T.p[k].z)) T.skip = true;
+  if (T.skip) return;
+  const V3 n0 = cross(T.p[1], T.p[2]), n1 = cross(T.p[2], T.p[0]), n2 = cross(T.p[0], T.p[1]);
+  const double D = dot(T.p[0], n0);
+  const double sg = D < 0.0 ? -1.0 : 1.0;
+  T.N[0] = sg * n0; T.N[1] = sg * n1; T.N[2] = sg * n2;
+  T.Nsum = sg * cross(T.p[1] - T.p[0], T.p[2] - T.p[0]);
+  const double l0 = len(T.p[0]), l1 = len(T.p[1]), l2 = len(T.p[2]);
+  T.tol[0] = 1e-10 * l1 * l2 * 1.7320508075688774;
+  T.tol[1] = 1e-10 * l2 * l0 * 1.7320508075688774;
+  T.tol[2] = 1e-10 * l0 * l1 * 1.7320508075688774;
+  T.absD = std::fabs(D);
+  T.area2 = len(T.Nsum);
+  T.dist = origin_distance(T.p[0], T.p[1], T.p[2]);
+  T.lmax = std::max(len(T.p[1] - T.p[0]), std::max(len(T.p[2] - T.p[1]), len(T.p[0] - T.p[2])));
+  T.edge_on = !(T.absD > 1e-12 * l0 * l1 * l2) || !(T.area2 > 0.0);
+  const double dmax = std::max(l0, std::max(l1, l2));
+  T.self_safe = !T.edge_on && T.absD >= 1e-3 * dmax * T.area2 && T.area2 >= 1e-6 * T.lmax * T.lmax;
+  T.cover_ok = !T.edge_on && T.area2 >= 1e-3 * T.lmax * T.lmax;
+}
+
+bool face_range(const TriPre& T, int f, int R, double delta, Entry& e) {
+  const int axis = f >> 1, b = (axis + 1) % 3, c = (axis + 2) % 3;
+  const double sa = (f & 1) ? -1.0 : 1.0;
+  struct P { double x, y, w; };
+  P poly[12], tmp[12];
+  int n = 3;
+  for (int k = 0; k < 3; ++k) poly[k] = {comp(T.p[k], b), comp(T.p[k], c), sa * comp(T.p[k], axis)};
+  const double kk = 1.0 + 2.0 * delta + 1e-6;
+  for (int pl = 0; pl < 4 && n > 0; ++pl) {
+    auto side = [&](const P& q) {
+      const double a = pl < 2 ? q.x : q.y;
+      return kk * q.w + ((pl & 1) ? a : -a);
+    };
+    int m = 0;
+    for (int k = 0; k < n; ++k) {
+      const P& q0 = poly[k];
+      const P& q1 = poly[(k + 1) % n];
+      const double s0 = side(q0), s1 = side(q1);
+      if (s0 >= 0.0) tmp[m++] = q0;
+      if ((s0 >= 0.0) != (s1 >= 0.0)) {
+        const double t = s0 / (s0 - s1);
+        tmp[m++] = {q0.x + t * (q1.x - q0.x), q0.y + t * (q1.y - q0.y), q0.w + t * (q1.w - q0.w)};
+      }
+    }
+    n = m;
+    for (int k = 0; k < n; ++k) poly[k] = tmp[k];
+  }
+  if (n == 0) return false;
+  double ulo = kInf, uhi = -kInf, vlo = kInf, vhi = -kInf;
+  for (int k = 0; k < n; ++k) {
+    if (!(poly[k].w > 1e-300)) { ulo = vlo = -2.0; uhi = vhi = 2.0; break; }
+    const double u = poly[k].x / poly[k].w, v = poly[k].y / poly[k].w;
+    ulo = std::min(ulo, u); uhi = std::max(uhi, u);
+    vlo = std::min(vlo, v); vhi = std::max(vhi, v);
+  }
+  auto lo_ix = [&](double x) {
+    const double g = std::floor((x - delta + 1.0) * 0.5 * R) - 1.0;
+    return (int)std::min(std::max(g, 0.0), (double)(R - 1));
+  };
+  auto hi_ix = [&](double x) {
+    const double g = std::floor((x + delta + 1.0) * 0.5 * R) + 1.0;
+    return (int)std::min(std::max(g, 0.0), (double)(R - 1));
+  };
+  e.i0 = (int16_t)lo_ix(ulo); e.i1 = (int16_t)hi_ix(uhi);
+  e.j0 = (int16_t)lo_ix(vlo); e.j1 = (int16_t)hi_ix(vhi);
+  return true;
+}
+
+struct TexelAcc { double lb1, d2, occ; int id1; };
+
+void raster_band(const std::vector<TriPre>& tris, const std::vector<Entry>& entries, int f, int j_begin, int j_end,
+                 int R, double delta, double rmax, bool lit_ok, LightTexel* out) {
+  const int axis = f >> 1, b = (axis + 1) % 3, c = (axis + 2) % 3;
+  const double sa = (f & 1) ? -1.0 : 1.0;
+  const double step = 2.0 / R;
+  std::vector<TexelAcc> acc((size_t)(j_end - j_begin) * R, TexelAcc{kInf, kInf, kInf, -1});
+  const double du = 0.5 * step + delta, r = std::sqrt(2.0) * du, spread = 1.01 * r;
+  for (const Entry& e : entries) {
+    const TriPre& T = tris[e.tri];
+    double A[3], B[3], C[3];
+    for (int k = 0; k < 3; ++k) { A[k] = sa * comp(T.N[k], axis); B[k] = comp(T.N[k], b); C[k] = comp(T.N[k], c); }
+    const double As = sa * comp(T.Nsum, axis), Bs = comp(T.Nsum, b), Cs = comp(T.Nsum, c);
+    const int ja = std::max((int)e.j0, j_begin), jb = std::min((int)e.j1, j_end - 1);
+    for (int j = ja; j <= jb; ++j) {
+      const double v0 = -1.0 + j * step - delta, v1 = -1.0 + (j + 1) * step + delta, vc = -1.0 + (j + 0.5) * step;
+      for (int i = e.i0; i <= e.i1; ++i) {
+        const double u0 = -1.0 + i * step - delta, u1 = -1.0 + (i + 1) * step + delta, uc = -1.0 + (i + 0.5) * step;
+        const double cu[4] = {u0, u1, u0, u1}, cv[4] = {v0, v0, v1, v1};
+        double E[3][4];
+        bool outside = false, inside = true;
+        for (int k = 0; k < 3; ++k) {
+          bool all_out = true;
+          for (int q = 0; q < 4; ++q) {
+            E[k][q] = A[k] + B[k] * cu[q] + C[k] * cv[q];
+            all_out = all_out && E[k][q] < -T.tol[k];
+            inside = inside && E[k][q] > T.tol[k];
+          }
+          outside = outside || all_out;
+        }
+        if (!T.edge_on && outside) continue;
+        double lb = T.dist;
+        double cos0 = 0.0;
+        if (!T.edge_on) {
+          cos0 = (As + Bs * uc + Cs * vc) / (T.area2 * std::sqrt(1.0 + uc * uc + vc * vc));
+          const double qv = std::min(1.0, std::fabs(cos0) + spread);
+          lb = std::max(lb, T.absD / (T.area2 * qv));
+        }
+        lb *= 1.0 - 1e-12;
+        TexelAcc& a = acc[(size_t)(j - j_begin) * R + i];
+        if (!T.self_safe) {
+          a.d2 = std::min(a.d2, lb);
+        } else if (lb < a.lb1 || (lb == a.lb1 && e.tri < a.id1)) {
+          a.d2 = std::min(a.d2, a.lb1);
+          a.lb1 = lb;
+          a.id1 = e.tri;
+        } else {
+          a.d2 = std::min(a.d2, lb);
+        }
+        if (!T.cover_ok || !inside) continue;
+        const double cos_lb = cos0 - spread, s_lb = T.area2 * cos_lb;
+        if (!(cos_lb >= 1e-2) || !(s_lb >= 1e-6)) continue;
+        const double margin = 1e-7 + 1e3 * 64.0 * kEps * (2.0 * rmax + T.lmax) * T.lmax / s_lb;
+        double ub = 0.0;
+        bool cover = true;
+        for (int q = 0; q < 4 && cover; ++q) {
+          const double sum = E[0][q] + E[1][q] + E[2][q];
+          if (!(sum > 0.0)) { cover = false; break; }
+          for (int k = 0; k < 3; ++k) cover = cover && E[k][q] >= margin * sum;
+          ub = std::max(ub, T.absD * std::sqrt(1.0 + cu[q] * cu[q] + cv[q] * cv[q]) / sum);
+        }
+        if (cover) a.occ = std::min(a.occ, ub * (1.0 + 1e-12));
+      }
+    }
+  }
+  for (int j = j_begin; j < j_end; ++j)
+    for (int i = 0; i < R; ++i) {
+      const TexelAcc& a = acc[(size_t)(j - j_begin) * R + i];
+      LightTexel& t = out[((size_t)f * R + j) * R + i];
+      t.id1 = a.id1;
+      t.d2 = lit_ok ? round_down_f(a.d2) : 0.0f;
+      t.occ = round_up_f(a.occ);
+      t.pad_ = 0;
+    }
+}
+
+template <class F>
+void run_threads(int threads, F&& fn) {
+  if (threads <= 1) { fn(0); return; }
+  std::vector<std::thread> th;
+  for (int t = 0; t < threads; ++t) th.emplace_back([&fn, t] { fn(t); });
+  for (auto& x : th) x.join();
+}
+
+}
+
+int build_light_map(const rt_scene_soa* s, const double light[3], int R, int threads, LightMap& out) {
+  out = LightMap();
+  if (!s || !light) return RT_ERR_INVALID;
+  if (R == 0) R = kLightMapDefaultR;
+  if (R < kLightMapMinR || R > kLightMapMaxR) return RT_ERR_INVALID;
+  if (!std::isfinite(light[0]) || !std::isfinite(light[1]) || !std::isfinite(light[2])) return RT_ERR_UNSUPPORTED;
+  const auto t0 = std::chrono::steady_clock::now();
+  threads = std::max(1, std::min(threads, 64));
+  const int nt = s->n_vertex_idx / 3;
+  const double delta = kLightMapDilation * 2.0 / R;
+  constexpr int kBandRows = 16;
+  const int bands = (R + kBandRows - 1) / kBandRows;
+
+  std::vector<TriPre> tris((size_t)nt);
+  std::vector<std::vector<std::vector<Entry>>> found(threads, std::vector<std::vector<Entry>>(6));
+  std::vector<double> far(threads, 0.0), near(threads, kInf);
+  run_threads(threads, [&](int w) {
+    const int lo = (int)((long long)nt * w / threads), hi = (int)((long long)nt * (w + 1) / threads);
+    for (int t = lo; t < hi; ++t) {
+      TriPre& T = tris[t];
+      prepare_triangle(s, light, t, T);
+      if (T.skip) continue;
+      for (int k = 0; k < 3; ++k) far[w] = std::max(far[w], len(T.p[k]));
+      near[w] = std::min(near[w], T.dist);
+      for (int f = 0; f < 6; ++f) {
+        Entry e;
+        e.tri = t;
+        if (face_range(T, f, R, delta, e)) found[w][f].push_back(e);
+      }
+    }
+  });
+  double rmax = 0.0, dmin = kInf;
+  for (int w = 0; w < threads; ++w) { rmax = std::max(rmax, far[w]); dmin = std::min(dmin, near[w]); }
+  if (rmax > kLightMapMaxExtent) return RT_ERR_UNSUPPORTED;
+  const bool lit_ok = dmin > 1e-3;
+
+  std::vector<std::vector<Entry>> by_band((size_t)6 * bands);
+  for (int f = 0; f < 6; ++f)
+    for (int w = 0; w < threads; ++w)
+      for (const Entry& e : found[w][f])
+        for (int bd = e.j0 / kBandRows; bd <= e.j1 / kBandRows; ++bd) by_band[(size_t)f * bands + bd].push_back(e);
+
+  out.tex.resize((size_t)6 * R * R);
+  std::atomic<int> next{0};
+  run_threads(threads, [&](int) {
+    for (;;) {
+      const int task = next.fetch_add(1);
+      if (task >= 6 * bands) break;
+      const int f = task / bands, bd = task % bands;
+      raster_band(tris, by_band[task], f, bd * kBandRows, std::min(R, (bd + 1) * kBandRows), R, delta, rmax, lit_ok,
+                  out.tex.data());
+    }
+  });
+  out.R = R;
+  for (int k = 0; k < 3; ++k) out.pos[k] = light[k];
+  out.seconds = std::chrono::duration<double>(std::chrono::steady_clock::now() - t0).count();
+  return RT_OK;
+}
+
+}
+
+extern "C" long long rt_debug_light_map(const rt_scene_soa* soa, const double* light, int R, int build_threads,
+                                        void* out, long long bytes) {
+  if (!soa || !light || build_threads < 0) return RT_ERR_INVALID;
+  if (R == 0) R = rtk::kLightMapDefaultR;
+  if (R < rtk::kLightMapMinR || R > rtk::kLightMapMaxR) return RT_ERR_INVALID;
+  const long long need = 6LL * R * R * (long long)sizeof(rtk::LightTexel);
+  if (!out) return need;
+  if (bytes < need) return RT_ERR_INVALID;
+  rtk::LightMap m;
+  const int rc = rtk::build_light_map(soa, light, R, build_threads, m);
+  if (rc != RT_OK) return rc;
+  std::copy(m.tex.begin(), m.tex.end(), static_cast<rtk::LightTexel*>(out));
+  return need;
+}
+
+extern "C" int rt_debug_light_map_certify(const void* map, int R, const double* light, long long n,
+                                          const double* points, const int* slots, unsigned char* out) {
+  if (!map || !light || !points || !slots || !out || n < 0) return RT_ERR_INVALID;
+  if (R < rtk::kLightMapMinR || R > rtk::kLightMapMaxR) return RT_ERR_INVALID;
+  const rtk::LightTexel* tex = static_cast<const rtk::LightTexel*>(map);
+  for (long long i = 0; i < n; ++i) {
+    const double* p = points + 3 * i;
+    const double to[3] = {light[0] - p[0], light[1] - p[1], light[2] - p[2]};
+    const double nl = std::sqrt(to[0] * to[0] + to[1] * to[1] + to[2] * to[2]);
+    const double l[3] = {to[0] / nl, to[1] / nl, to[2] / nl};
+    out[i] = (unsigned char)rtk::light_map_certify(tex, R, l, nl, slots[i]);
+  }
+  return RT_OK;
+}
diff --git a/my-raytracer_amd/csrc/host/light_map.hpp b/my-raytracer_amd/csrc/host/light_map.hpp
--- /dev/null
+++ b/my-raytracer_amd/csrc/host/light_map.hpp
@@ -0,0 +1,57 @@
+#pragma once
+#include <cmath>
+#include <cstdint>
+#include <vector>
+
+#include "../../../include/rt_hip.h"
+
+namespace rtk {
+
+struct LightTexel {
+  int32_t id1;
+  float d2;
+  float occ;
+  uint32_t pad_;
+};
+static_assert(sizeof(LightTexel) == 16, "one 16-byte load per lookup");
+
+constexpr int kLightMapDefaultR = 512;
+constexpr int kLightMapMinR = 16, kLightMapMaxR = 2048;
+constexpr double kLightMapDilation = 0.125;
+constexpr float kLightMapM = 1.00001f;
+constexpr float kLightMapA = 1e-3f;
+constexpr double kLightMapMaxExtent = 1e4;
+
+struct LightMap {
+  int R = 0;
+  double pos[3] = {0, 0, 0};
+  std::vector<LightTexel> tex;
+  double seconds = 0.0;
+};
+
+int build_light_map(const rt_scene_soa* s, const double light[3], int R, int threads, LightMap& out);
+
+enum { kCertNone = 0, kCertLit = 1, kCertOccluded = 2, kCertClamped = 4, kCertForeign = 8 };
+
+inline int light_map_certify(const LightTexel* tex, int R, const double l[3], double nl, int slot) {
+  const float d[3] = {(float)-l[0], (float)-l[1], (float)-l[2]};
+  const float ax = std::fabs(d[0]), ay = std::fabs(d[1]), az = std::fabs(d[2]);
+  const int axis = (ax >= ay && ax >= az) ? 0 : (ay >= az ? 1 : 2);
+  const float m = std::fabs(d[axis]);
+  if (!(m > 0.0f)) return kCertNone;
+  const int f = 2 * axis + (d[axis] < 0.0f);
+  const float u = d[(axis + 1) % 3] / m, v = d[(axis + 2) % 3] / m;
+  const float half = 0.5f * (float)R;
+  int i = (int)std::floor((u + 1.0f) * half), j = (int)std::floor((v + 1.0f) * half);
+  int flags = 0;
+  if (i < 0 || i >= R || j < 0 || j >= R) flags = kCertClamped;
+  i = i < 0 ? 0 : (i >= R ? R - 1 : i);
+  j = j < 0 ? 0 : (j >= R ? R - 1 : j);
+  const LightTexel t = tex[((size_t)f * R + j) * R + i];
+  const float n = (float)nl;
+  if (n * kLightMapM < t.d2) return kCertLit | flags | ((slot >= 0 && slot != t.id1) ? kCertForeign : 0);
+  if (n > t.occ * kLightMapM + kLightMapA) return kCertOccluded | flags;
+  return flags;
+}
+
+}
diff --git a/my-raytracer_amd/rtamd/__init__.py b/my-raytracer_amd/rtamd/__init__.py
--- a/my-raytracer_amd/rtamd/__init__.py
+++ b/my-raytracer_amd/rtamd/__init__.py
@@ -820,15 +820,16 @@
         return img.reshape(rows_in_shard(params), params.camera.width, 3)
 
     def debug_counters(self):
-        buf = (C.c_ulonglong * 40)()
-        n = hip_lib().rt_debug_counters(self._h, buf, 40)
+        buf = (C.c_ulonglong * 43)()
+        n = hip_lib().rt_debug_counters(self._h, buf, 43)
         if n < 0:
             _check_hip(n, "rt_debug_counters")
         names = {16: "node_iters", 17: "node_lanes", 18: "leaf_iters", 19: "leaf_lanes", 20: "trav_cycles",
                  21: "shade_cycles", 22: "fetch_cycles", 23: "outer_iters", 24: "trav_rounds", 25: "trav_round_lanes",
                  26: "stack_spills", 27: "node_lines", 28: "leaf_lines", 29: "big_leaf_tests",
                  30: "node_lds_iters", 32: "gnode_uniform_iters", 33: "gnode_distinct", 34: "leaf_uniform_iters",
-                 35: "anyhit_tri_tests", 36: "anyhit_own_record_tests", 37: "shadow_rays_skipped"}
+                 35: "anyhit_tri_tests", 36: "anyhit_own_record_tests", 37: "shadow_rays_skipped",
+                 38: "shadow_rays_certified_lit", 42: "shadow_rays_certified_occluded"}
         return {v: int(buf[k]) for k, v in names.items()}
 
     def wave_log(self, max_waves=1 << 16):
diff --git a/my-raytracer_amd/rtamd/abi.py b/my-raytracer_amd/rtamd/abi.py
--- a/my-raytracer_amd/rtamd/abi.py
+++ b/my-raytracer_amd/rtamd/abi.py
@@ -200,10 +200,11 @@
                 ("verbose", C.c_int), ("sbvh_alpha", C.c_double), ("sbvh_budget", C.c_double),
                 ("sbvh_c_trav", C.c_double), ("collapse_c_tri", C.c_double), ("reserve_cus", C.c_int),
                 ("order_window", C.c_int), ("spp_lanes", C.c_int), ("tree_opt", C.c_int),
-                ("reserved_", C.c_int * 4)]
+                ("light_map", C.c_int), ("reserved_", C.c_int * 3)]
 
 
 RT_TREE_OPT_PASSES, RT_TREE_OPT_MAX = 3, 64
+RT_LIGHT_MAP_MIN, RT_LIGHT_MAP_MAX, RT_LIGHT_MAPS = 16, 2048, 4
 RT_TREE_BAD_UNION, RT_TREE_BAD_LEAF, RT_TREE_BAD_RECORDS, RT_TREE_BAD_IDS, RT_TREE_BAD_FIXPOINT = 1, 2, 4, 8, 16
 
 
@@ -299,6 +300,10 @@
     "rt_debug_corrupt_hierarchy": (C.c_int, [C.c_void_p]),
     "rt_debug_tree_report": (C.c_int, [C.POINTER(SceneSoA), C.POINTER(BvhSoA), C.POINTER(UploadOptions),
                                        C.POINTER(TreeReport)]),
+    "rt_debug_light_map": (C.c_longlong, [C.POINTER(SceneSoA), C.POINTER(C.c_double), C.c_int, C.c_int, C.c_void_p,
+                                          C.c_longlong]),
+    "rt_debug_light_map_certify": (C.c_int, [C.c_void_p, C.c_int, C.POINTER(C.c_double), C.c_longlong,
+                                             C.POINTER(C.c_double), C.POINTER(C.c_int), C.POINTER(C.c_ubyte)]),
     "rt_scene_status": (C.c_int, [C.c_void_p]),
     "rt_scene_free": (None, [C.c_void_p]),
     "rt_last_error": (C.c_char_p, []),
```

Measured after the change: 29150 Mrays/s (median of 6 runs). 1.03x the previous value.
